# mvanveen/hyperopt

Measured on AMD Instinct MI355X. Metric: TPE candidate x component lpdf evals/sec (10k-trial history), higher is better.
Workload: dtype f32+f64

## Files before the change

hyperopt_amd/_lib.py:

```python
import ctypes
import os

HERE = os.path.dirname(os.path.abspath(__file__))
LIB_PATH = os.path.join(HERE, 'libhyperopt_tpe.so')
HEADER = os.path.join(os.path.dirname(HERE), 'include', 'hyperopt_tpe.h')

ABI_VERSION = 4

TPE_OK = 0
TPE_ERR_VALUE = -1
TPE_ERR_TYPE = -2
TPE_ERR_ARG = -3
TPE_STATUS_VALUE_ONLY = 1
TPE_ERR_HIP = -4
TPE_ERR_SAMPLE = -5

TPE_F64 = 0
TPE_F32 = 1

TPE_GMM1 = 0
TPE_LGMM1 = 1
TPE_CATEGORICAL = 2

TPE_HAS_LOW = 1
TPE_HAS_HIGH = 2
TPE_HAS_Q = 4
TPE_HAS_STREAM = 8

TPE_OPT_SCREEN = 1
TPE_OPT_SPLITK = 2
TPE_OPT_DEDUP = 3
TPE_OPT_CHUNKS = 4
TPE_OPT_WHOLE_N = 5
TPE_OPT_WHOLE_ROUNDS = 6
TPE_OPT_TIMING = 7
TPE_OPT_WINDOW = 8
TPE_OPT_WIN_T = 9
TPE_OPT_WIN_GROUPS = 10
TPE_OPT_EXPAND = 11
TPE_OPT_HOT = 12
TPE_OPT_EARLY = 13
TPE_OPT_HOT_DIV = 14
TPE_OPT_ZERO_WIN = 15
TPE_OPT_VALUE_ONLY = 16
TPE_OPT_RESCORE_CAP = 17
TPE_OPT_MODE_MASK = 18
TPE_OPT_AUX_FAMILIES = 19
TPE_OPT_BX_SPLIT = 21
TPE_OPT_BX_T = 22
TPE_OPT_PK_SLICED = 23
TPE_OPT_DEFER_REPORT = 24
TPE_OPT_LABEL_SHARDS = 25

TPE_JOINT_STREAM = 0x7FFFFFFF

TPE_OBS_IDENTITY = 0
TPE_OBS_LOG = 1
TPE_OBS_LOG_FLOOR = 2


class LabelDesc(ctypes.Structure):
    _fields_ = [('kind', ctypes.c_int32), ('flags', ctypes.c_int32),
                ('low', ctypes.c_double), ('high', ctypes.c_double), ('q', ctypes.c_double),
                ('below_off', ctypes.c_int64), ('above_off', ctypes.c_int64),
                ('n_below', ctypes.c_int32), ('n_above', ctypes.c_int32)]


class LabelSpec(ctypes.Structure):
    _fields_ = [('kind', ctypes.c_int32), ('flags', ctypes.c_int32),
                ('low', ctypes.c_double), ('high', ctypes.c_double), ('q', ctypes.c_double),
                ('prior_mu', ctypes.c_double), ('prior_sigma', ctypes.c_double),
                ('upper', ctypes.c_int32), ('randint', ctypes.c_int32), ('p_off', ctypes.c_int64),
                ('stream', ctypes.c_int32), ('reserved', ctypes.c_int32)]


class LabelResult(ctypes.Structure):
    _fields_ = [('value', ctypes.c_double), ('score', ctypes.c_double),
                ('lpdf_below', ctypes.c_double), ('lpdf_above', ctypes.c_double),
                ('index', ctypes.c_int64), ('label', ctypes.c_int32), ('status', ctypes.c_int32)]


class JointDim(ctypes.Structure):
    _fields_ = [('kind', ctypes.c_int32), ('flags', ctypes.c_int32),
                ('low', ctypes.c_double), ('high', ctypes.c_double),
                ('stream', ctypes.c_int32)]


assert ctypes.sizeof(JointDim) == 32
assert ctypes.sizeof(LabelDesc) == 56
assert ctypes.sizeof(LabelResult) == 48
assert ctypes.sizeof(LabelSpec) == 72

_P = ctypes.c_void_p
_I32, _I64, _U32, _U64, _D = (ctypes.c_int32, ctypes.c_int64, ctypes.c_uint32,
                              ctypes.c_uint64, ctypes.c_double)
_PD = ctypes.POINTER(ctypes.c_double)

SIGNATURES = {
    'tpe_abi_version': (ctypes.c_int, []),
    'tpe_source_hash': (ctypes.c_char_p, []),
    'tpe_ctx_create': (ctypes.c_int, [ctypes.c_int, ctypes.c_int, ctypes.POINTER(_P)]),
    'tpe_ctx_create_multi': (ctypes.c_int, [_P, _I32, ctypes.c_int, ctypes.POINTER(_P)]),
    'tpe_ctx_devices': (ctypes.c_int32, [_P, _P, _I32]),
    'tpe_label_device': (ctypes.c_int32, [_P, _I32]),
    'tpe_ctx_destroy': (None, [_P]),
    'tpe_last_error': (ctypes.c_char_p, [_P]),
    'tpe_gmm1_lpdf': (ctypes.c_int, [_P, _P, _I64, _P, _P, _P, _I32, _I32, _D, _D, _D, _P]),
    'tpe_lgmm1_lpdf': (ctypes.c_int, [_P, _P, _I64, _P, _P, _P, _I32, _I32, _D, _D, _D, _P]),
    'tpe_categorical_lpdf': (ctypes.c_int, [_P, _P, _I64, _P, _I32, _P]),
    'tpe_broadcast_best': (ctypes.c_int, [_P, _P, _P, _I64, _P]),
    'tpe_gmm1_sample': (ctypes.c_int, [_P, _P, _P, _P, _I32, _I32, _D, _D, _D, _U64, _U32, _U32,
                                       _I64, _I64, _P]),
    'tpe_lgmm1_sample': (ctypes.c_int, [_P, _P, _P, _P, _I32, _I32, _D, _D, _D, _U64, _U32, _U32,
                                        _I64, _I64, _P]),
    'tpe_categorical_sample': (ctypes.c_int, [_P, _P, _I32, _U64, _U32, _U32, _I64, _I64, _P]),
    'tpe_set_posterior': (ctypes.c_int, [_P, _P, _I32, _P, _P, _P, _I64]),
    'tpe_suggest': (ctypes.c_int, [_P, _U64, _U32, _I64, _I64, _P]),
    'tpe_suggest_batch': (ctypes.c_int, [_P, _U64, _P, _I32, _I64, _I64, _P]),
    'tpe_score': (ctypes.c_int, [_P, _I32, _P, _I64, _P, _P, _P]),
    'tpe_merge_results': (ctypes.c_int, [_P, _I32, _I32, _P]),
    'tpe_suggest_batch_device': (ctypes.c_int, [_P, _U64, _P, _I32, _I64, _I64, _P, _P]),
    'tpe_merge_results_device': (ctypes.c_int, [_P, _P, _I32, _I32, _P]),
    'tpe_last_timing': (ctypes.c_int, [_P, ctypes.POINTER(ctypes.c_float),
                                       ctypes.POINTER(ctypes.c_float)]),
    'tpe_last_evals': (ctypes.c_int64, [_P]),
    'tpe_last_mode_stats': (ctypes.c_int, [_P, _P, _P]),
    'tpe_build_posterior': (ctypes.c_int, [_P, _P, _I32, _P, _I64, _P, _I64, _P, _P, _P, _D, _D,
                                           _I32, _P]),
    'tpe_get_mixture': (ctypes.c_int, [_P, _I32, _I32, _P, _P, _P, _I32, _P]),
    'tpe_resident_labels': (ctypes.c_int32, [_P]),
    'tpe_history_reset': (ctypes.c_int, [_P, _P, _I32, _P, _I64]),
    'tpe_history_append': (ctypes.c_int, [_P, _P, _P, _P]),
    'tpe_build_posterior_resident': (ctypes.c_int, [_P, _P, _I64, _I64, _D, _D, _I32, _P]),
    'tpe_build_posterior_resident_ordered': (ctypes.c_int, [_P, _P, _I64, _I64, _D, _D, _I32, _P, _P, _P,
                                                            _P, _P]),
    'tpe_rebuild_labels': (ctypes.c_int, [_P, _P, _I64, _I64, _D, _D, _I32, _P, _P, _P, _I32, _P, _P]),
    'tpe_last_build_ms': (ctypes.c_int, [_P, ctypes.POINTER(ctypes.c_float)]),
    'tpe_build_report': (ctypes.c_int, [_P, ctypes.POINTER(ctypes.c_int32), ctypes.c_void_p]),
    'tpe_last_screen': (ctypes.c_int, [_P, _P, _P, ctypes.POINTER(ctypes.c_float)]),
    'tpe_set_option': (ctypes.c_int, [_P, _I32, _I64]),
    'tpe_last_screen_terms': (ctypes.c_int, [_P, _P]),
    'tpe_last_rescore_terms': (ctypes.c_int, [_P, _P]),
    'tpe_last_drawn': (ctypes.c_int, [_P, _P, _P]),
    'tpe_device_bytes': (ctypes.c_int64, []),
    'tpe_prepare': (ctypes.c_int, [_P, ctypes.c_int64, ctypes.c_int32]),
    'tpe_arm_prepare': (ctypes.c_int, [_P, ctypes.c_int64, ctypes.c_int32]),
    'tpe_last_screen_mode': (ctypes.c_int32, [_P]),
    'tpe_last_hot': (ctypes.c_int, [_P, _P, _P]),
    'tpe_last_prepare': (ctypes.c_int, [_P, _P]),
    'tpe_hot_probe': (ctypes.c_int, [_P, ctypes.c_int32, _P, ctypes.c_int64, _P, _P, _P]),
    'tpe_screen_probe': (ctypes.c_int, [_P, _I32, _P, _I64, _P, _P]),
    'tpe_export_posterior': (ctypes.c_int, [_P, _P, _I64, _P]),
    'tpe_import_posterior': (ctypes.c_int, [_P, _P, _I64, _P, _I32, _P, _P]),
    'tpe_joint_set_posterior': (ctypes.c_int, [_P, _P, _I32, _I32, _P, _P, _P, _I32, _P, _P, _P]),
    'tpe_joint_draw': (ctypes.c_int, [_P, _U64, _U32, _I64, _I64, _P, _P]),
    'tpe_joint_score': (ctypes.c_int, [_P, _P, _I64, _P, _P]),
    'tpe_joint_suggest': (ctypes.c_int, [_P, _U64, _U32, _I64, _P, _P, _PD, _PD]),
}

_lib = None


def load():
    global _lib
    if _lib is not None:
        return _lib
    try:
        import torch
    except Exception:
        pass
    variant = os.environ.get('HYPEROPT_AMD_VARIANT')
    path = LIB_PATH
    if variant:
        import sys
        path = os.path.abspath(variant)
        sys.stderr.write('hyperopt_amd: loading the experiment variant %s, not the product '
                         'library\n' % path)
    if not os.path.exists(path):
        raise OSError('hyperopt_amd native library not built: %s (run '
                      '`python -m hyperopt_amd._build` or __graft_entry__.build())' % path)
    lib = ctypes.CDLL(path)
    for name, (res, args) in SIGNATURES.items():
        if variant and not hasattr(lib, name):
            continue
        fn = getattr(lib, name)
        fn.restype = res
        fn.argtypes = args
    if lib.tpe_abi_version() != ABI_VERSION:
        raise OSError('ABI version mismatch')
    if variant:
        if not lib.tpe_source_hash().decode().startswith('v:'):
            raise OSError('%s is not a variant build (tools/build_variant.py)' % path)
    else:
        check_stamp(lib)
    _lib = lib
    return lib


def check_stamp(lib):
    from . import _build
    want = _build.source_hash()
    got = lib.tpe_source_hash().decode()
    if got != want:
        raise OSError('hyperopt_amd native library %s is stale: built from sources %s, tree '
                      'has %s (run `python -m hyperopt_amd._build`)' % (LIB_PATH, got, want))


def header_functions(path=HEADER):
    import re
    txt = open(path).read()
    txt = re.sub(r'/\*.*?\*/', '', txt, flags=re.S)
    return sorted(set(re.findall(r'\b(tpe_[a-z0-9_]+)\s*\(', txt)))
```

hyperopt_amd/csrc/tpe_build.hip:

```cpp
#include <hip/hip_runtime.h>

#include <hipcub/hipcub.hpp>

#include <cmath>
#include <cstring>
#include <string>
#include <vector>

#include "../../include/hyperopt_tpe.h"
#include "tpe_ctx.h"
#include "tpe_device.h"

using namespace tpe;
using namespace tpe_rt;

namespace {

constexpr int kSplitBlock = 1024;
constexpr int kPartBlock = 1024;
constexpr int kPartU = 4;
constexpr int kParzenBlock = 1024;
constexpr int kFoldU = 4;
constexpr int kMaxLF = 64;
constexpr int kCatChunk = 8192;
// ... 1304 lines not shown
        for (int32_t l = 0; l < L; ++l) mx = std::max(mx, B.cnt_h[l]);
        if (mx > 0 && B.pool_cap > 0)
            hipLaunchKernelGGL(k_hist_regrow, dim3((unsigned)std::min<int64_t>((mx + kBlock - 1) / kBlock, 1024), L),
                               dim3(kBlock), 0, sm, B.p_off.p, o2.p, B.cnt.p, B.p_trial.p, B.p_val.p,
                               B.s_key.p, B.s_idx.p, t2.p, v2.p, k2.p, i2.p);
        HIPCHK(ctx, hipGetLastError());
        HIPCHK(ctx, hipStreamSynchronize(sm));
        std::swap(B.p_trial, t2);
        std::swap(B.p_val, v2);
        std::swap(B.s_key, k2);
        std::swap(B.s_idx, i2);
        std::swap(B.p_off, o2);
        t2.release();
        v2.release();
        k2.release();
        i2.release();
        o2.release();
        HIPCHK(ctx, B.s_key2.reserve(pc));
        HIPCHK(ctx, B.s_idx2.reserve(pc));
        HIPCHK(ctx, B.arank.reserve(pc));
        HIPCHK(ctx, B.keys.reserve(pc));
        HIPCHK(ctx, B.idx.reserve(pc));
        B.cap_h = cap;
        B.off_h = off;
        B.pool_cap = pc;
    }
    HIPCHK(ctx, B.st_off.reserve(L + 1));
    HIPCHK(ctx, B.st_trial.reserve(total));
    HIPCHK(ctx, B.st_val.reserve(total));
    HIPCHK(ctx, B.st_idx.reserve(total));
    HIPCHK(ctx, B.st_idx_sorted.reserve(total));
    HIPCHK(ctx, B.st_key_sorted.reserve(total));
    HIPCHK(ctx, B.seg_begin.reserve(L));
    HIPCHK(ctx, B.seg_end.reserve(L));
    auto al = [](int64_t v) { return (v + 15) / 16 * 16; };
    const int64_t o_off = 0, o_val = al((L + 1) * 8), o_trial = o_val + al(total * 8),
                  o_seg = o_trial + al(total * 4), o_cnt = o_seg + al(2 * (int64_t)L * 4),
                  o_end = o_cnt + al((int64_t)L * 4);
    HIPCHK(ctx, B.h_stage.resize(o_end));
    HIPCHK(ctx, B.d_stage.reserve(o_end));
    uint8_t* hs = B.h_stage.data();
    std::memcpy(hs + o_off, st.data(), (L + 1) * sizeof(int64_t));
    int32_t* seg = (int32_t*)(hs + o_seg);
    for (int32_t l = 0; l < L; ++l) {
        seg[l] = (int32_t)st[l];
        seg[L + l] = (int32_t)(B.specs_h[l].kind == TPE_CATEGORICAL ? st[l] : st[l + 1]);
    }
    std::memcpy(hs + o_trial, obs_trial, total * sizeof(int32_t));
    std::memcpy(hs + o_val, obs_val, total * sizeof(double));
    int32_t* cnt_new = (int32_t*)(hs + o_cnt);
    for (int32_t l = 0; l < L; ++l) cnt_new[l] = B.cnt_h[l] + (int32_t)n_new[l];
    HIPCHK(ctx, hipMemcpyAsync(B.d_stage.p, hs, o_end, hipMemcpyHostToDevice, sm));
    {
        const uint8_t* ds = B.d_stage.p;
        const CopySpec cs[5] = {{B.st_off.p, ds + o_off, (L + 1) * 8},
                                {B.st_trial.p, ds + o_trial, total * 4},
                                {B.st_val.p, ds + o_val, total * 8},
                                {B.seg_begin.p, ds + o_seg, (int64_t)L * 4},
                                {B.seg_end.p, ds + o_seg + (int64_t)L * 4, (int64_t)L * 4}};
        const int rc = tpe_rt::copy_batch(ctx, sm, cs, 5);
        if (rc) return rc;
    }
    int64_t mx_new = 0, mx_all = 0;
    for (int32_t l = 0; l < L; ++l) {
        mx_new = std::max(mx_new, n_new[l]);
        mx_all = std::max<int64_t>(mx_all, B.cnt_h[l] + n_new[l]);
    }
    hipLaunchKernelGGL(k_hist_append, dim3((unsigned)std::min<int64_t>((mx_new + kBlock - 1) / kBlock, 1024), L),
                       dim3(kBlock), 0, sm, B.st_off.p, B.st_trial.p, B.st_val.p, B.p_off.p, B.cnt.p,
                       B.p_trial.p, B.p_val.p, B.st_idx.p);
    HIPCHK(ctx, hipGetLastError());
    if (total >= kGlobalSortMin) {
        HIPCHK(ctx, B.gs_a.reserve(total));
        HIPCHK(ctx, B.gs_b.reserve(total));
        HIPCHK(ctx, B.gs_lab.reserve(total));
        HIPCHK(ctx, B.gs_lab2.reserve(total));
        int lab_bits = 1;
        while ((1LL << lab_bits) < (int64_t)L) ++lab_bits;
        const unsigned gb = (unsigned)std::min<int64_t>((total + kBlock - 1) / kBlock, 2048);
        hipLaunchKernelGGL(k_iota, dim3(gb), dim3(kBlock), 0, sm, B.gs_a.p, total);
        HIPCHK(ctx, hipGetLastError());
        size_t b1 = 0, b2 = 0;
        HIPCHK(ctx, hipcub::DeviceRadixSort::SortPairs(nullptr, b1, B.st_val.p, B.st_key_sorted.p, B.gs_a.p,
                                                         B.gs_b.p, (int)total, 0, 64, sm));
        HIPCHK(ctx, hipcub::DeviceRadixSort::SortPairs(nullptr, b2, B.gs_lab.p, B.gs_lab2.p, B.gs_b.p,
                                                         B.gs_a.p, (int)total, 0, lab_bits, sm));
        HIPCHK(ctx, B.sort_tmp.reserve(std::max<size_t>(std::max(b1, b2), 1)));
        HIPCHK(ctx, hipcub::DeviceRadixSort::SortPairs(B.sort_tmp.p, b1, B.st_val.p, B.st_key_sorted.p,
                                                         B.gs_a.p, B.gs_b.p, (int)total, 0, 64, sm));
        hipLaunchKernelGGL(k_label_of, dim3(gb), dim3(kBlock), 0, sm, B.st_off.p, L, B.gs_b.p, B.gs_lab.p, total);
        HIPCHK(ctx, hipGetLastError());
        HIPCHK(ctx, hipcub::DeviceRadixSort::SortPairs(B.sort_tmp.p, b2, B.gs_lab.p, B.gs_lab2.p, B.gs_b.p,
                                                         B.gs_a.p, (int)total, 0, lab_bits, sm));
        hipLaunchKernelGGL(k_sorted_gather, dim3(gb), dim3(kBlock), 0, sm, B.gs_a.p, B.st_val.p, B.st_idx.p,
                           B.st_key_sorted.p, B.st_idx_sorted.p, total);
        HIPCHK(ctx, hipGetLastError());
    } else {
        size_t bytes = 0;
        HIPCHK(ctx, hipcub::DeviceSegmentedRadixSort::SortPairs(
                        nullptr, bytes, B.st_val.p, B.st_key_sorted.p, B.st_idx.p, B.st_idx_sorted.p,
                        (int)total, L, B.seg_begin.p, B.seg_end.p, 0, 64, sm));
        HIPCHK(ctx, B.sort_tmp.reserve(std::max<size_t>(bytes, 1)));
        HIPCHK(ctx, hipcub::DeviceSegmentedRadixSort::SortPairs(
                        B.sort_tmp.p, bytes, B.st_val.p, B.st_key_sorted.p, B.st_idx.p, B.st_idx_sorted.p,
                        (int)total, L, B.seg_begin.p, B.seg_end.p, 0, 64, sm));
    }
    hipLaunchKernelGGL(k_hist_merge, dim3((unsigned)std::min<int64_t>((mx_all + kBlock - 1) / kBlock, 1024), L),
                       dim3(kBlock), 0, sm, B.specs.p, B.p_off.p, B.cnt.p, B.st_off.p, B.s_key.p,
                       B.s_idx.p, B.st_key_sorted.p, B.st_idx_sorted.p, B.s_key2.p, B.s_idx2.p);
    HIPCHK(ctx, hipGetLastError());
    std::swap(B.s_key, B.s_key2);
    std::swap(B.s_idx, B.s_idx2);
    for (int32_t l = 0; l < L; ++l) B.cnt_h[l] += (int32_t)n_new[l];
    {
        const CopySpec cs{B.cnt.p, B.d_stage.p + o_cnt, (int64_t)L * 4};
        const int rc = tpe_rt::copy_batch(ctx, sm, &cs, 1);
        if (rc) return rc;
    }
    HIPCHK(ctx, hipEventRecord(B.ev_staged, sm));
    B.staged_pending = true;
    return TPE_OK;
}

constexpr int32_t kGammaCap = 25;

uint64_t loss_fingerprint(const double* losses, int64_t n) {
    uint64_t h = 0x9e3779b97f4a7c15ull ^ (uint64_t)n;
    for (int64_t t = 0; t < n; ++t) {
        uint64_t v;
        std::memcpy(&v, losses + t, sizeof(v));
        h = (h ^ v) * 0xff51afd7ed558ccdull;
        h ^= h >> 29;
    }
    return h;
}

int finish_build(tpe_ctx* ctx, BuildTail& t, int32_t* ties_out, int32_t* n_below_out) {
    auto& B = ctx->build;
    Posterior& P = ctx->resident;
    const int32_t n_labels = t.n_labels;
    const int64_t rep_dl = t.rep_dl;
    std::vector<DLabel>& dl = t.dl;
    const std::vector<int32_t>* grp = t.grp;
    const bool beside = t.beside, subset = t.subset;
    HIPCHK(ctx, hipStreamSynchronize(t.st));
    P.qc_ready = false;
    int32_t errh;
    std::memcpy(&errh, B.h_rep.data() + rep_dl, sizeof(int32_t));
    std::memcpy(dl.data(), B.h_rep.data(), rep_dl);
    B.last_ties.resize(n_labels + 1);
    std::memcpy(B.last_ties.data(), B.h_rep.data() + rep_dl + 16, (n_labels + 1) * sizeof(int32_t));
    B.last_n_below = t.n_below;
    if (ties_out) std::memcpy(ties_out, B.last_ties.data(), (n_labels + 1) * sizeof(int32_t));
    if (t.deferred) ctx->build_ms = -1.f;
    else HIPCHK(ctx, hipEventElapsedTime(&ctx->build_ms, ctx->ev0, ctx->ev1));
    if (errh & 1) return ctx->fail(TPE_ERR_ARG, "observation trial position out of range");
    if (errh & 2) return ctx->fail(TPE_ERR_ARG, "more below observations than the below set (duplicate trial in a label?)");
    if (errh & 4) return ctx->fail(TPE_ERR_VALUE, "below weights sum to zero");
    if (errh & 8) return ctx->fail(TPE_ERR_ARG, "supplied observation order does not fit the above set");

    std::vector<int32_t> cat;
    for (int m = 0; m < kNumModes; ++m) {
        P.group_off[m] = (int32_t)cat.size();
        cat.insert(cat.end(), grp[m].begin(), grp[m].end());
        P.h_group[m] = grp[m];
    }
    const bool groups_changed = cat != P.groups_h || !P.groups.p;
    if (groups_changed) {
        HIPCHK(ctx, P.groups.reserve(std::max<size_t>(cat.size(), 1)));
        HIPCHK(ctx, hipMemcpy(P.groups.p, cat.data(), cat.size() * sizeof(int32_t), hipMemcpyHostToDevice));
        P.groups_h = cat;
    }
    P.h_labels = dl;
    P.win_ready = false;
    P.zw_ready = false;
    P.qc_ready = t.qc_queued;
    if (!beside) P.bx_ready = tpe_rt::bx_keep_after(ctx, groups_changed);
    P.n_labels = n_labels;
    B.n_labels = n_labels;
    B.mix_h = t.mix;
    B.built_ok = true;
    B.built_gen = B.hist_gen;
    B.built_T = t.n_trials;
    B.built_valid = t.n_valid;
    B.built_gamma = t.gamma;
    B.built_pw = t.pw;
    B.built_lf = t.lf;
    if (!subset) B.built_loss_hash = t.loss_hash;
    if (n_below_out) *n_below_out = t.n_below;
    P.bx_prescan_ok = t.prescan && !P.bx_ready;
    if (t.arm_c > 0) return tpe1_prepare(ctx, t.arm_c, t.arm_r);
    return TPE_OK;
}

int build_resident(tpe_ctx* ctx, const double* losses, int64_t n_trials, int64_t n_valid,
                   double gamma, double prior_weight, int32_t lf, int32_t* n_below_out,
                   const uint8_t* below_h = nullptr, const int64_t* order_off_h = nullptr,
                   const int32_t* order_h = nullptr, int32_t* ties_out = nullptr,
                   const int32_t* only_h = nullptr, int32_t n_only = 0) {
    auto& B = ctx->build;
    const bool defer_report = B.defer;
    B.defer = false;
    if (!B.hist_ready) return ctx->fail(TPE_ERR_ARG, "no resident history (tpe_history_reset)");
    const bool subset = only_h != nullptr && n_only > 0;
    const int64_t arm_c = subset ? 0 : ctx->arm_c;
    const int32_t arm_r = subset ? 0 : ctx->arm_r;
    if (!subset) ctx->arm_c = ctx->arm_r = 0;
    if (subset) {
        if (below_h)
            return ctx->fail(TPE_ERR_ARG, "a label-subset rebuild keeps the previous build's below set");
        if (!B.built_ok || B.built_gen != B.hist_gen || B.built_T != n_trials || B.built_valid != n_valid ||
            B.built_gamma != gamma || B.built_pw != prior_weight || B.built_lf != lf ||
            B.n_labels != (int32_t)B.specs_h.size())
            return ctx->fail(TPE_ERR_ARG, "a label-subset rebuild must follow a build of the same history");
        if (n_trials > 0 && !losses) return ctx->fail(TPE_ERR_ARG, "tpe_build_posterior: bad trial arguments");
        if (loss_fingerprint(losses, n_trials) != B.built_loss_hash)
            return ctx->fail(TPE_ERR_ARG, "a label-subset rebuild must be given the previous build's losses");
        for (int32_t i = 0; i < n_only; ++i)
            if (only_h[i] < 0 || only_h[i] >= B.n_labels || (i && only_h[i] <= only_h[i - 1]))
                return ctx->fail(TPE_ERR_ARG, "subset labels must be increasing label indices");
    }
    B.built_ok = false;
    ctx->resident.bx_prescan_ok = false;
    if (lf < 1 || lf >= kMaxLF) return ctx->fail(TPE_ERR_ARG, "linear forgetting must be in [1, 63]");
    if (n_trials < 0 || n_trials >= INT32_MAX || (n_trials > 0 && !losses) || n_valid < 0 ||
        n_valid > n_trials)
        return ctx->fail(TPE_ERR_ARG, "tpe_build_posterior: bad trial arguments");
    HIPCHK(ctx, hipSetDevice(ctx->device));
    const int32_t n_labels = (int32_t)B.specs_h.size();
    Posterior& P = ctx->resident;
    ctx->P = &ctx->resident;
    bool beside = subset;
    for (int32_t i = 0; beside && i < n_only; ++i) {
        const tpe_label_spec& s = B.specs_h[only_h[i]];
        beside = s.kind == TPE_CATEGORICAL || (s.flags & TPE_HAS_Q) != 0;
    }
    hipStream_t st = beside ? ctx->aux : ctx->stream;

    const double nbd = std::ceil(gamma * std::sqrt((double)n_valid));
    const int32_t n_below = (int32_t)std::min<double>(nbd, (double)kGammaCap);
    if (below_h) {
        int64_t nb = 0;
        for (int64_t t = 0; t < n_trials; ++t)
            if (below_h[t]) {
                if (!(losses[t] == losses[t])) return ctx->fail(TPE_ERR_ARG, "below set holds a trial without a loss");
                ++nb;
            }
        if (nb != n_below) return ctx->fail(TPE_ERR_ARG, "below set size differs from n_below");
    }

    std::vector<DLabel> dl(n_labels);
    std::vector<int64_t> mix(2 * (size_t)n_labels);
    std::vector<int32_t> grp[kNumModes];
    int64_t total = 0, samp_total = 0, max_cap = 1;
    for (int32_t l = 0; l < n_labels; ++l) {
        const tpe_label_spec& s = B.specs_h[l];
        DLabel& o = dl[l];
        std::memset(&o, 0, sizeof(o));
        const bool quant = (s.flags & TPE_HAS_Q) != 0;
        int64_t cap_b, cap_a;
        if (s.kind == TPE_CATEGORICAL) {
            o.mode = CAT;
            cap_b = cap_a = s.upper;
        } else {
            o.mode = s.kind == TPE_GMM1 ? (quant ? QUANT_GMM : DENSE_GMM) : (quant ? QUANT_LGMM : DENSE_LGMM);
            cap_b = lf + 1;
            cap_a = (int64_t)B.cnt_h[l] + 1;
        }
        o.flags = s.kind == TPE_CATEGORICAL ? 0 : (s.flags & (TPE_HAS_LOW | TPE_HAS_HIGH | TPE_HAS_Q));
        o.low = s.low;
        o.high = s.high;
        o.q = s.q;
        o.exp_low = std::exp(s.low);
        o.exp_high = std::exp(s.high);
        o.stream = (s.flags & TPE_HAS_STREAM) ? s.stream : l;
        o.comp_b = mix[2 * l] = total;
        total += cap_b;
        o.comp_a = mix[2 * l + 1] = total;
        total += cap_a;
        max_cap = std::max(max_cap, std::max(cap_b, cap_a));
        o.samp_off = samp_total;
        samp_total += cap_b;
        grp[o.mode].push_back(l);
    }
    const int64_t T = n_trials;
    HIPCHK(ctx, B.losses.reserve(std::max<int64_t>(T, 1)));
    HIPCHK(ctx, B.below.reserve(std::max<int64_t>(T, 1)));
    HIPCHK(ctx, B.below_val.reserve((size_t)n_labels * kMaxLF));
    HIPCHK(ctx, B.counts.reserve(2 * (size_t)n_labels));
    HIPCHK(ctx, B.kcount.reserve(2 * (size_t)n_labels));
    HIPCHK(ctx, B.keys.reserve(std::max<int64_t>(B.pool_cap, 1)));
    HIPCHK(ctx, B.idx.reserve(std::max<int64_t>(B.pool_cap, 1)));
    HIPCHK(ctx, B.arank.reserve(std::max<int64_t>(B.pool_cap, 1)));
    HIPCHK(ctx, B.w.reserve(total));
    HIPCHK(ctx, B.mu.reserve(total));
    HIPCHK(ctx, B.sigma.reserve(total));
    HIPCHK(ctx, B.mix_off.reserve(2 * (size_t)n_labels));
    HIPCHK(ctx, B.scratch.reserve(4 * (size_t)total));
    HIPCHK(ctx, P.labels.reserve(n_labels));
    HIPCHK(ctx, P.comps64.reserve(total));
    HIPCHK(ctx, P.comps32.reserve(total));
    HIPCHK(ctx, P.samp.reserve(samp_total));
    HIPCHK(ctx, ctx->build_err.reserve(1));
    HIPCHK(ctx, B.ties.reserve(n_labels + 1));
    const int64_t* order_off_d = nullptr;
    const int32_t* order_d = nullptr;
    std::vector<UpTask> up;
    std::vector<const void*> up_src;
    auto put = [&](const void* src, int64_t bytes, void* dst) {
        if (bytes <= 0) return;
        up.push_back(UpTask{0, (uint8_t*)dst, bytes, 0});
        up_src.push_back(src);
    };
    put(nullptr, (n_labels + 1) * (int64_t)sizeof(int32_t), B.ties.p);
    if (order_off_h && order_h && order_off_h[n_labels] > 0) {
        for (int32_t l = 0; l < n_labels; ++l)
            if (order_off_h[l + 1] < order_off_h[l] || order_off_h[l] < 0)
                return ctx->fail(TPE_ERR_ARG, "order offsets must not decrease");
        HIPCHK(ctx, B.order_off.reserve(n_labels + 1));
        HIPCHK(ctx, B.order.reserve(order_off_h[n_labels]));
        put(order_off_h, (n_labels + 1) * (int64_t)sizeof(int64_t), B.order_off.p);
        put(order_h, order_off_h[n_labels] * (int64_t)sizeof(int32_t), B.order.p);
        order_off_d = B.order_off.p;
        order_d = B.order.p;
    }
    const int32_t* only_d = nullptr;
    const int32_t nl_run = subset ? n_only : n_labels;
    if (subset) {
        HIPCHK(ctx, B.only.reserve(n_only));
        put(only_h, n_only * (int64_t)sizeof(int32_t), B.only.p);
        only_d = B.only.p;
    } else {
        put(losses, T * (int64_t)sizeof(double), B.losses.p);
        if (below_h) put(below_h, T, B.below.p);
        put(mix.data(), (int64_t)mix.size() * (int64_t)sizeof(int64_t), B.mix_off.p);
        put(dl.data(), n_labels * (int64_t)sizeof(DLabel), P.labels.p);
    }
    put(nullptr, sizeof(int32_t), ctx->build_err.p);
    {
        const int64_t head = ((int64_t)up.size() * (int64_t)sizeof(UpTask) + 255) / 256 * 256;
        int64_t o = head;
        for (UpTask& u : up) {
            u.src = up_src[&u - up.data()] ? o : -1;
            if (u.src >= 0) o += (u.bytes + 15) / 16 * 16;
        }
        if (B.up_pending) {
            HIPCHK(ctx, hipEventSynchronize(B.ev_up));
            B.up_pending = false;
        }
        HIPCHK(ctx, B.h_up.resize(o));
        HIPCHK(ctx, B.d_up.reserve(o));
        std::memcpy(B.h_up.data(), up.data(), up.size() * sizeof(UpTask));
        for (size_t i = 0; i < up.size(); ++i)
            if (up[i].src >= 0) std::memcpy(B.h_up.data() + up[i].src, up_src[i], up[i].bytes);
        HIPCHK(ctx, hipMemcpyAsync(B.d_up.p, B.h_up.data(), o, hipMemcpyHostToDevice, st));
        if (!B.ev_up) HIPCHK(ctx, hipEventCreateWithFlags(&B.ev_up, hipEventDisableTiming));
        HIPCHK(ctx, hipEventRecord(B.ev_up, st));
        B.up_pending = true;
        int64_t mx = 1;
        for (const UpTask& u : up) mx = std::max(mx, u.bytes);
        hipLaunchKernelGGL(k_build_inputs, dim3((unsigned)std::min<int64_t>((mx + 4 * kUpBlock - 1) / (4 * kUpBlock), 32),
                                                (unsigned)up.size()),
                           dim3(kUpBlock), 0, st, (const UpTask*)B.d_up.p, B.d_up.p);
        HIPCHK(ctx, hipGetLastError());
    }

    HIPCHK(ctx, hipEventRecord(ctx->ev0, st));
    if (T > 0 && !below_h && !subset) {
        const int rc = launch_split(ctx, st, B.losses.p, T, n_below, B.below.p, B.ties.p + n_labels);
        if (rc) return rc;
    }
    hipLaunchKernelGGL(k_partition, dim3(nl_run), dim3(kPartBlock), 0, st, B.specs.p, B.p_off.p, B.cnt.p,
                       B.p_trial.p, B.p_val.p, B.s_key.p, B.s_idx.p, B.below.p, B.losses.p, T,
                       B.below_val.p, B.arank.p, B.keys.p, B.idx.p, B.counts.p, ctx->build_err.p, only_d);
    hipLaunchKernelGGL(k_parzen, dim3(nl_run, 2), dim3(kParzenBlock), 0, st, B.specs.p, B.cat_p.p,
                       B.p_off.p, B.counts.p, B.below_val.p, B.keys.p, B.keys.p, B.idx.p, B.mix_off.p,
                       prior_weight, lf, B.w.p, B.mu.p, B.sigma.p, B.kcount.p, B.scratch.p + total, order_off_d,
                       order_d, B.ties.p, ctx->build_err.p, only_d);
    hipLaunchKernelGGL(k_fold_terms, dim3((unsigned)((max_cap + kTermBlock - 1) / kTermBlock), nl_run, 2),
                       dim3(kTermBlock), 0, st, P.labels.p, B.kcount.p, B.mix_off.p, B.w.p, B.mu.p,
                       B.sigma.p, B.scratch.p, B.scratch.p + 2 * total, B.scratch.p + 3 * total, only_d);
    hipLaunchKernelGGL(k_fold, dim3(nl_run), dim3(kParzenBlock), 0, st, P.labels.p, B.kcount.p,
                       B.mix_off.p, B.w.p, B.mu.p, B.sigma.p, P.comps64.p, P.comps32.p, P.samp.p,
                       B.scratch.p, B.scratch.p + 2 * total, B.scratch.p + 3 * total, B.scratch.p + total,
                       ctx->build_err.p, only_d);
    HIPCHK(ctx, hipGetLastError());
    HIPCHK(ctx, hipEventRecord(ctx->ev1, st));
    const int64_t rep_dl = (int64_t)n_labels * (int64_t)sizeof(DLabel);
    const int64_t rep_bytes = rep_dl + 16 + (int64_t)(n_labels + 1) * (int64_t)sizeof(int32_t);
    HIPCHK(ctx, B.d_rep.reserve(rep_bytes));
    HIPCHK(ctx, B.h_rep.resize(rep_bytes));
    hipLaunchKernelGGL(k_build_report, dim3(1), dim3(kUpBlock), 0, st, (const uint32_t*)P.labels.p,
                       (int32_t)(rep_dl / 4), ctx->build_err.p, B.ties.p, n_labels + 1, (uint32_t*)B.d_rep.p);
    HIPCHK(ctx, hipGetLastError());
    HIPCHK(ctx, hipMemcpyAsync(B.h_rep.data(), B.d_rep.p, rep_bytes, hipMemcpyDeviceToHost, st));
    if (!beside) {
        const int rc = tpe_rt::bx_keep_check(ctx);
        if (rc) return rc;
    }
    bool prescan = false;
    if (!subset && arm_c > 0 && P.groups.p) {
        std::vector<int32_t> cat_now;
        for (int m = 0; m < kNumModes; ++m) cat_now.insert(cat_now.end(), grp[m].begin(), grp[m].end());
        bool same = cat_now == P.groups_h;
        for (int m = 0; same && m < kNumModes; ++m) same = grp[m] == P.h_group[m];
        if (same) {
            const int rc = tpe_rt::bx_prescan(ctx, st, &prescan);
            if (rc) return rc;
        }
    }
    bool qc_queued = false;
    if (beside && P.groups.p) {
        std::vector<int32_t> cat_now;
        for (int m = 0; m < kNumModes; ++m) cat_now.insert(cat_now.end(), grp[m].begin(), grp[m].end());
        if (cat_now == P.groups_h) {
            const int rc = tpe_rt::qc_launch(ctx, st);
            if (rc) return rc;
            qc_queued = true;
        }
    }
    BuildTail t;
    t.st = st;
    t.rep_dl = rep_dl;
    t.n_labels = n_labels;
    t.lf = lf;
    t.n_below = n_below;
    t.dl = std::move(dl);
    for (int m = 0; m < kNumModes; ++m) t.grp[m] = std::move(grp[m]);
    t.mix = std::move(mix);
    t.beside = beside;
    t.qc_queued = qc_queued;
    t.subset = subset;
    t.n_trials = n_trials;
    t.n_valid = n_valid;
    t.arm_c = arm_c;
    t.arm_r = arm_r;
    t.prescan = prescan;
    t.gamma = gamma;
    t.pw = prior_weight;
    if (!subset) t.loss_hash = loss_fingerprint(losses, n_trials);
    if (beside && subset && qc_queued && defer_report) {
        t.deferred = true;
        B.pending.reset(new BuildTail(std::move(t)));
        if (ties_out) std::memset(ties_out, 0, (n_labels + 1) * sizeof(int32_t));
        if (n_below_out) *n_below_out = n_below;
        return TPE_OK;
    }
    return finish_build(ctx, t, ties_out, n_below_out);
}

}

int tpe_rt::settle_build(tpe_ctx* ctx) {
    if (!ctx) return TPE_OK;
    auto& B = ctx->build;
    if (!B.pending) return TPE_OK;
    std::unique_ptr<BuildTail> t = std::move(B.pending);
    return finish_build(ctx, *t, nullptr, nullptr);
}

extern "C" {

TPE_DEV int tpe1_history_reset(tpe_ctx* ctx, const tpe_label_spec* specs, int32_t n_labels,
                      const double* cat_p, int64_t n_cat_p) {
    if (!ctx) return TPE_ERR_ARG;
    TPE_SETTLE(ctx);
    return history_reset(ctx, specs, n_labels, cat_p, n_cat_p);
}

TPE_DEV int tpe1_history_append(tpe_ctx* ctx, const int64_t* n_new, const int32_t* obs_trial,
                       const double* obs_val) {
    if (!ctx || !n_new) return TPE_ERR_ARG;
    TPE_SETTLE(ctx);
    return history_append(ctx, n_new, obs_trial, obs_val);
}

TPE_DEV int tpe1_build_posterior_resident(tpe_ctx* ctx, const double* losses, int64_t n_trials,
                                 int64_t n_valid, double gamma, double prior_weight, int32_t lf,
                                 int32_t* n_below_out) {
    if (!ctx) return TPE_ERR_ARG;
    TPE_SETTLE(ctx);
    return build_resident(ctx, losses, n_trials, n_valid, gamma, prior_weight, lf, n_below_out);
}

TPE_DEV int tpe1_build_posterior_resident_ordered(tpe_ctx* ctx, const double* losses, int64_t n_trials,
                                                  int64_t n_valid, double gamma, double prior_weight,
                                                  int32_t lf, const uint8_t* below, const int64_t* order_off,
                                                  const int32_t* order, int32_t* n_below_out, int32_t* ties) {
    if (!ctx) return TPE_ERR_ARG;
    TPE_SETTLE(ctx);
    return build_resident(ctx, losses, n_trials, n_valid, gamma, prior_weight, lf, n_below_out, below,
                          order_off, order, ties);
}

TPE_DEV int tpe1_rebuild_labels(tpe_ctx* ctx, const double* losses, int64_t n_trials, int64_t n_valid,
                                double gamma, double prior_weight, int32_t lf, const int64_t* order_off,
                                const int32_t* order, const int32_t* labels, int32_t n_only,
                                int32_t* n_below_out, int32_t* ties) {
    if (!ctx) return TPE_ERR_ARG;
    TPE_SETTLE(ctx);
    if (!labels || n_only <= 0) return ctx->fail(TPE_ERR_ARG, "tpe_rebuild_labels: no labels");
    return build_resident(ctx, losses, n_trials, n_valid, gamma, prior_weight, lf, n_below_out, nullptr,
                          order_off, order, ties, labels, n_only);
}

TPE_DEV int tpe1_build_posterior(tpe_ctx* ctx, const tpe_label_spec* specs, int32_t n_labels,
                        const double* cat_p, int64_t n_cat_p, const double* losses,
                        int64_t n_trials, const int64_t* obs_off, const int32_t* obs_trial,
                        const double* obs_val, double gamma, double prior_weight, int32_t lf,
                        int32_t* n_below_out) {
    if (!ctx) return TPE_ERR_ARG;
    TPE_SETTLE(ctx);
    if (n_labels <= 0 || !specs || !obs_off || n_trials < 0 || (n_trials > 0 && !losses))
        return ctx->fail(TPE_ERR_ARG, "tpe_build_posterior: bad arguments");
    if (obs_off[0] != 0 || obs_off[n_labels] < 0 || obs_off[n_labels] >= INT32_MAX)
        return ctx->fail(TPE_ERR_ARG, "observation offsets");
    std::vector<int64_t> n_new(n_labels);
    for (int32_t l = 0; l < n_labels; ++l) {
        n_new[l] = obs_off[l + 1] - obs_off[l];
        if (n_new[l] < 0) return ctx->fail(TPE_ERR_ARG, "observation offsets must not decrease");
    }
    int64_t n_valid = 0;
    for (int64_t t = 0; t < n_trials; ++t) n_valid += losses[t] == losses[t];
    int rc = history_reset(ctx, specs, n_labels, cat_p, n_cat_p);
    if (!rc) rc = history_append(ctx, n_new.data(), obs_trial, obs_val);
    if (!rc) rc = build_resident(ctx, losses, n_trials, n_valid, gamma, prior_weight, lf, n_below_out);
    if (rc) ctx->build.hist_ready = false;
    return rc;
}

TPE_DEV int tpe1_get_mixture(tpe_ctx* ctx, int32_t label, int32_t side, double* weights, double* mus,
                             double* sigmas, int32_t cap, int32_t* n) {
    if (!ctx) return TPE_ERR_ARG;
    TPE_SETTLE(ctx);
    auto& B = ctx->build;
    if (label < 0 || label >= B.n_labels || side < 0 || side > 1 || ctx->resident.n_labels != B.n_labels)
        return ctx->fail(TPE_ERR_ARG, "tpe_get_mixture: no such built mixture");
    const DLabel& d = ctx->resident.h_labels[label];
    const int32_t K = side ? d.na : d.nb;
    if (n) *n = K;
    const int32_t m = std::min(K, std::max(cap, 0));
    const int64_t o = B.mix_h[2 * (size_t)label + side];
    HIPCHK(ctx, hipSetDevice(ctx->device));
    if (m > 0) {
        if (weights) HIPCHK(ctx, hipMemcpy(weights, B.w.p + o, m * sizeof(double), hipMemcpyDeviceToHost));
        if (mus) HIPCHK(ctx, hipMemcpy(mus, B.mu.p + o, m * sizeof(double), hipMemcpyDeviceToHost));
        if (sigmas) HIPCHK(ctx, hipMemcpy(sigmas, B.sigma.p + o, m * sizeof(double), hipMemcpyDeviceToHost));
    }
    return TPE_OK;
}

TPE_DEV int32_t tpe1_resident_labels(const tpe_ctx* ctx) { return ctx ? ctx->resident.n_labels : 0; }

TPE_DEV int tpe1_last_build_ms(const tpe_ctx* ctx, float* ms) {
    if (!ctx || !ms) return TPE_ERR_ARG;
    TPE_SETTLE(const_cast<tpe_ctx*>(ctx));
    *ms = ctx->build_ms;
    return TPE_OK;
}

TPE_DEV int tpe1_build_report(tpe_ctx* ctx, int32_t* n_below, int32_t* ties) {
    if (!ctx) return TPE_ERR_ARG;
    TPE_SETTLE(ctx);
    if (n_below) *n_below = ctx->build.last_n_below;
    if (ties) {
        const auto& t = ctx->build.last_ties;
        if (t.empty()) return ctx->fail(TPE_ERR_ARG, "tpe_build_report: no build");
        std::memcpy(ties, t.data(), t.size() * sizeof(int32_t));
    }
    return TPE_OK;
}

}
```

hyperopt_amd/csrc/tpe_ctx.h:

```cpp
#pragma once

#include <hip/hip_runtime.h>
#include <stdint.h>

#include <algorithm>
#include <atomic>
#include <memory>
#include <string>
#include <vector>

#include "../../include/hyperopt_tpe.h"
#include "tpe_device.h"

struct tpe_ctx;

namespace tpe_rt {

struct RescoreChunkH {
    int32_t cell, j;
};
struct RescorePlanH {
    int64_t total;
    int32_t ne, sliced, overflow, pad;
};
// ... 86 lines not shown
            if (e != hipSuccess) {
                p = nullptr;
                return e;
            }
            cap = c;
        }
        n = m;
        return hipSuccess;
    }
    T* data() { return p; }
    const T* data() const { return p; }
    size_t size() const { return n; }
    T& operator[](size_t i) { return p[i]; }
    const T& operator[](size_t i) const { return p[i]; }
    PinVec() = default;
    PinVec(const PinVec&) = delete;
    PinVec& operator=(const PinVec&) = delete;
    ~PinVec() {
        if (p) (void)hipHostFree(p);
    }
};

struct PinScalars {
    int32_t err = 0, hot_flag = 0, bx_diff = 1, pad = 0;
    unsigned long long screen_exec = 0, xdrawn[2] = {0, 0};
    RescorePlanH plan{};
};

struct Posterior {
    std::vector<DLabel> h_labels;
    std::vector<int32_t> h_group[kNumModes];
    int32_t n_labels = 0;
    DevBuf<DLabel> labels;
    DevBuf<Comp<double>> comps64;
    DevBuf<Comp<float>> comps32;
    DevBuf<SampRec> samp;
    DevBuf<int32_t> groups;
    std::vector<int32_t> groups_h;
    int32_t group_off[kNumModes] = {};
    bool win_ready = false;
    bool zw_ready = false;
    DevBuf<double> zw_hi, zw_lo;
    DevBuf<int32_t> zw_wide, zw_n;
    bool qc_ready = false;
    DevBuf<Comp<double>> qcomp;
    DevBuf<int32_t> qc_n;
    int32_t win_t = 0;
    DevBuf<tpe::WinLabel> win;
    DevBuf<double> win_p, win_q;
    DevBuf<Comp<float>> win_wide;
    DevBuf<int2> win_bins;
    DevBuf<double> win_seg;
    DevBuf<int32_t> win_hist;
    DevBuf<uint8_t> win_flag;
    DevBuf<double> win_skip;
    DevBuf<double> win_skip_part;
    bool bx_ready = false, bx_ok = false;
    bool bx_prescan_ok = false;
    PinVec<double> bx_scan_h;
    DevBuf<tpe::BxLabel> bx;
    std::vector<tpe::BxLabel> bx_h;
    PinVec<tpe::BxLabel> bx_up_h;
    DevBuf<double> bx_tab;
    DevBuf<int32_t> bx_nc;
    DevBuf<tpe::BxTerm> bx_terms;
    DevBuf<int32_t> bx_loff;
    DevBuf<int32_t> bx_list;
    DevBuf<double> bx_scan;
    DevBuf<float2> bx_sb;
    DevBuf<float> bx_sbp;
    DevBuf<double> bx_part;
    DevBuf<int2> bx_blocks;
    PinVec<int2> bx_blocks_h;
    int64_t bx_sb_max = 0;
    uint64_t bx_gen = 0;
    DevBuf<tpe::DLabel> bx_snap_l;
    DevBuf<tpe::Comp<double>> bx_snap_c;
    DevBuf<tpe::SampRec> bx_snap_s;
    DevBuf<int32_t> bx_snap_g;
    DevBuf<int32_t> bx_diff;
    int32_t bx_snap_nl = 0;
    void release() {
        labels.release();
        comps64.release();
        comps32.release();
        samp.release();
        groups.release();
        groups_h.clear();
        win.release();
        win_p.release();
        win_q.release();
        win_wide.release();
        win_bins.release();
        win_seg.release();
        win_hist.release();
        win_flag.release();
        win_skip.release();
        win_skip_part.release();
        win_ready = false;
        zw_ready = false;
        qc_ready = false;
        qcomp.release();
        qc_n.release();
        zw_hi.release();
        zw_lo.release();
        zw_wide.release();
        zw_n.release();
        bx.release();
        bx_h.clear();
        bx_tab.release();
        bx_nc.release();
        bx_terms.release();
        bx_loff.release();
        bx_list.release();
        bx_scan.release();
        bx_sb.release();
        bx_sbp.release();
        bx_part.release();
        bx_blocks.release();
        bx_snap_l.release();
        bx_snap_c.release();
        bx_snap_s.release();
        bx_snap_g.release();
        bx_diff.release();
        bx_snap_nl = 0;
        bx_ready = bx_ok = false;
        n_labels = 0;
    }
};

struct CopySpec {
    void* dst;
    const void* src;
    int64_t bytes;
};
constexpr int kCopyBatch = 8;
int copy_batch(tpe_ctx* ctx, hipStream_t st, const CopySpec* specs, int n);

struct UpTask {
    int64_t src;
    uint8_t* dst;
    int64_t bytes;
    int64_t pad;
};

struct BuildTail {
    hipStream_t st = nullptr;
    int64_t rep_dl = 0;
    int32_t n_labels = 0, lf = 0, n_below = 0;
    std::vector<DLabel> dl;
    std::vector<int32_t> grp[kNumModes];
    std::vector<int64_t> mix;
    bool beside = false, qc_queued = false, subset = false, deferred = false;
    int64_t n_trials = 0, n_valid = 0, arm_c = 0;
    int32_t arm_r = 0;
    bool prescan = false;
    double gamma = 0.0, pw = 0.0;
    uint64_t loss_hash = 0;
};
int settle_build(tpe_ctx* ctx);

struct BuildBufs {
    std::vector<tpe_label_spec> specs_h;
    std::vector<int64_t> cap_h, off_h;
    std::vector<int32_t> cnt_h;
    int64_t pool_cap = 0;
    bool hist_ready = false;
    DevBuf<tpe_label_spec> specs;
    DevBuf<double> cat_p;
    DevBuf<int64_t> p_off;
    DevBuf<int32_t> cnt;
    DevBuf<int32_t> p_trial;
    DevBuf<double> p_val;
    DevBuf<double> s_key, s_key2;
    DevBuf<int32_t> s_idx, s_idx2;
    DevBuf<int32_t> arank;
    DevBuf<int64_t> st_off;
    DevBuf<int32_t> st_trial, st_idx, st_idx_sorted;
    DevBuf<double> st_val, st_key_sorted;
    DevBuf<int32_t> seg_begin, seg_end;
    DevBuf<uint8_t> sort_tmp;
    DevBuf<int32_t> gs_a, gs_b;
    DevBuf<uint32_t> gs_lab, gs_lab2;
    PinVec<uint8_t> h_stage;
    DevBuf<uint8_t> d_stage;
    hipEvent_t ev_staged = nullptr;
    bool staged_pending = false;
    DevBuf<double> losses;
    DevBuf<uint8_t> below;
    DevBuf<double> keys;
    DevBuf<int32_t> idx;
    DevBuf<double> below_val;
    DevBuf<int32_t> counts;
    DevBuf<int32_t> kcount;
    DevBuf<double> w, mu, sigma;
    DevBuf<int64_t> mix_off;
    DevBuf<double> scratch;
    DevBuf<int32_t> ties;
    DevBuf<int64_t> order_off;
    DevBuf<int32_t> order;
    int32_t n_labels = 0;
    std::vector<int64_t> mix_h;
    uint64_t hist_gen = 0, built_gen = 0;
    bool built_ok = false;
    int64_t built_T = -1, built_valid = -1;
    double built_gamma = 0.0, built_pw = 0.0;
    int32_t built_lf = 0;
    uint64_t built_loss_hash = 0;
    DevBuf<int32_t> only;
    DevBuf<uint64_t> split_key;
    DevBuf<int64_t> split_pos;
    bool defer = false;
    std::unique_ptr<BuildTail> pending;
    std::vector<int32_t> last_ties;
    int32_t last_n_below = 0;
    PinVec<uint8_t> h_up, h_rep;
    DevBuf<uint8_t> d_up, d_rep;
    hipEvent_t ev_up = nullptr;
    bool up_pending = false;
    void release() {
        specs.release(); cat_p.release(); p_off.release(); cnt.release(); p_trial.release();
        p_val.release(); s_key.release(); s_key2.release(); s_idx.release(); s_idx2.release();
        arank.release(); st_off.release(); st_trial.release(); st_idx.release();
        st_idx_sorted.release(); st_val.release(); st_key_sorted.release(); seg_begin.release();
        seg_end.release(); sort_tmp.release(); gs_a.release(); gs_b.release(); gs_lab.release();
        gs_lab2.release(); losses.release(); below.release(); keys.release();
        idx.release(); below_val.release(); counts.release(); kcount.release(); w.release();
        mu.release(); sigma.release(); mix_off.release(); scratch.release(); ties.release();
        order_off.release(); order.release(); only.release(); split_key.release(); split_pos.release();
        d_up.release(); d_rep.release(); d_stage.release();
        if (ev_up) (void)hipEventDestroy(ev_up);
        ev_up = nullptr;
        up_pending = false;
        if (ev_staged) (void)hipEventDestroy(ev_staged);
        ev_staged = nullptr;
        staged_pending = false;
        built_ok = false;
        n_labels = 0;
        hist_ready = false;
        pool_cap = 0;
    }
};

double np_pairwise_sum(const double* a, size_t n);

struct QExchange {
    virtual int exchange(tpe_ctx* ctx, std::vector<unsigned long long>& mm) = 0;
    virtual ~QExchange() {}
};

}

struct tpe_ctx {
    using Partial = tpe::Partial;
    using QInfo = tpe_rt::QInfo;
    template <typename T>
    using DevBuf = tpe_rt::DevBuf<T>;
    using Posterior = tpe_rt::Posterior;
    static constexpr int kNumModes = tpe_rt::kNumModes;

    int device = 0;
    int precision = TPE_F64;
    hipStream_t stream = nullptr;
    hipEvent_t ev0 = nullptr, ev1 = nullptr, ev2 = nullptr;
    hipEvent_t evm[kNumModes][2] = {};
    bool mode_ran[kNumModes] = {};
    float mode_ms[kNumModes] = {};
    int64_t mode_evals[kNumModes] = {};
    std::string err;
    float score_ms = 0.f, round_ms = 0.f;
    int64_t evals = 0;
    bool dedup = true;
    bool timing = true;

    Posterior resident, single;
    Posterior* P = &resident;

    DevBuf<Partial> partials;
    DevBuf<tpe_label_result> results;
    DevBuf<uint32_t> rounds;
    DevBuf<int32_t> errflag;
    DevBuf<int32_t> build_err;
    DevBuf<double> cand, out_lb, out_la;
    DevBuf<int32_t> one_group;
    DevBuf<int64_t> qj;
    DevBuf<unsigned long long> qmm;
    DevBuf<QInfo> qinfo;
    DevBuf<double2> qtab;
    DevBuf<unsigned long long> qkmax;
    DevBuf<int64_t> xfound;
    DevBuf<unsigned long long> xdrawn;
    unsigned long long xdrawn_h[2] = {0, 0};
    bool cat_early = false;
    DevBuf<double> xs, slice_part;
    bool splitk = true;
    DevBuf<double> chunk_part;
    int32_t chunks_forced = 0;
    bool screen = true;
    DevBuf<float> scr_hi;
    DevBuf<double> scr_hid;
    DevBuf<double2> bx_lohi;
    bool expand = true;
    int32_t hot = 1;
    bool early = true;
    bool zero_win = true;
    bool zw_pending = false;
    double hot_cap_div = 16.0;
    DevBuf<double> hot_x;
    DevBuf<uint32_t> rs_done;
    bool dense_one = false;
    DevBuf<int32_t> hot_pc;
    DevBuf<uint32_t> hot_ucell;
    DevBuf<uint4> samp_img;
    int32_t bx_split = 0;
    int64_t pk_sliced = 8192;
    int32_t bx_t_force = 0;
    double bx_t_next = 64.0;
    DevBuf<int32_t> hot_i, hot_cnt;
    DevBuf<int32_t> hot_mi, hot_mcnt;
    DevBuf<unsigned long long> hot_t, hot_tau0;
    DevBuf<uint32_t> hot_bits;
    DevBuf<int32_t> hot_flag;
    DevBuf<int32_t> hot_items;
    tpe_rt::PinVec<int32_t> hot_cnt_h;
    int64_t hot_listed = 0;
    int32_t hot_fallback = 0;
    bool hot_ran = false;
    int64_t hot_cells = 0;
    bool hot_redo = false;
    DevBuf<int64_t> rs_plan;
    bool value_only = false;
    int32_t mode_mask = 31;
    int64_t pk_cap = 1 << 16;
    bool pk_plan_pending = false;
    bool pk_redo = false;
    tpe_label_result* dev_out = nullptr;
    float prep_ms = 0.f;
    hipEvent_t ev_prep[2] = {};
    bool prep_pending = false;
    uint64_t hot_tau0_gen = 0;
    int64_t hot_tau0_n = 0;
    int64_t arm_c = 0;
    int32_t arm_r = 0;
    DevBuf<int32_t> scr_idx;
    DevBuf<unsigned long long> scr_lb;
    DevBuf<int32_t> scr_cnt;
    tpe_rt::PinVec<int32_t> scr_cnt_h;
    tpe_rt::PinVec<tpe_rt::PinScalars> pin;
    struct RepTask {
        const void* src;
        void* dst;
        int64_t bytes;
    };
    std::vector<RepTask> rep;
    tpe_rt::DevBuf<uint8_t> rep_d;
    tpe_rt::PinVec<uint8_t> rep_h;
    tpe_rt::PinVec<tpe_label_result> res_h;
    static constexpr int kResPieces = 4;
    hipEvent_t ev_res[kResPieces] = {};
    tpe_rt::PinVec<tpe::DLabel> dl_h;
    tpe_rt::PinVec<int32_t> ties_h;
    DevBuf<int64_t> scr_chunks;
    DevBuf<int64_t> scr_list;
    DevBuf<Partial> scr_res;
    DevBuf<int64_t> scr_rsel;
    DevBuf<int64_t> scr_off;
    DevBuf<int64_t> scr_range;
    DevBuf<double> scr_planes;
    DevBuf<double> rs_x, rs_part;
    DevBuf<int32_t> rs_win;
    DevBuf<int64_t> rs_g;
    std::vector<tpe_rt::RescoreChunkH> scr_chunks_h;
    int64_t screen_total = 0, screen_rescored = 0;
    int32_t screen_mode = 0;
    bool screen_pending = false;
    bool window = true;
    int32_t win_t = tpe::kWinTDefault;
    int32_t win_groups = 0;
    DevBuf<uint32_t> win_keys[2], win_keys2[2];
    DevBuf<uint8_t> win_keys8[2], win_keys8b[2];
    DevBuf<uint64_t> win_vals[2], win_vals2[2];
    DevBuf<uint8_t> win_tmp[2];
    hipStream_t aux = nullptr;
    hipEvent_t ev_fork = nullptr, ev_sorted[2] = {}, ev_done[2] = {};
    hipEvent_t ev_cat[2] = {};
    bool aux_families = false;
    std::vector<hipEvent_t> evw;
    int32_t evw_used = 0;
    DevBuf<unsigned long long> win_evals;
    DevBuf<float2> win_lohi;
    int64_t screen_exec = 0;
    int64_t screen_rescore_terms = 0;
    bool screen_exec_pending = false;
    unsigned long long screen_exec_h = 0;
    hipEvent_t evs[2] = {};
    float screen_ms = 0.f;
    tpe_rt::BuildBufs build;
    int64_t built_n_trials = 0;
    int32_t built_n_below = 0;
    float build_ms = 0.f;

    std::vector<tpe_ctx*> peers;
    std::shared_ptr<void> workers;
    std::shared_ptr<void> share;
    int64_t hint_n = 0;
    int32_t hint_rounds = 0;
    int64_t opt_whole_n = 0;
    int32_t opt_whole_rounds = 0;
    tpe_rt::QExchange* qx = nullptr;
    int32_t shard_id = 0;
    std::vector<std::vector<int32_t>> lsh_ids;
    std::vector<int32_t> lsh_dev, lsh_local;
    int32_t lsh_L = 0;
    bool lsh_enable = true;

    std::shared_ptr<void> joint;

    int fail(int code, const std::string& m) {
        err = m;
        return code;
    }
    int hip(hipError_t e, const char* what) {
        if (e == hipSuccess) return TPE_OK;
        err = std::string(what) + ": " + hipGetErrorString(e);
        return TPE_ERR_HIP;
    }
};

namespace tpe_rt {
struct WinScreenArgs {
    const int32_t* grp;
    int32_t nl;
    int64_t n, cand_offset;
    uint64_t seed;
    int32_t z0, nz;
    const double* cand_in;
    float* hi;
    unsigned long long* lbkey;
    double *s_out, *e_out;
    int32_t cpack = 0;
    float2* lohi = nullptr;
    int32_t y0 = 0, nl_all = 0;
    int slot = 0;
};
int win_prepare(tpe_ctx* ctx);
int win_screen(tpe_ctx* ctx, const WinScreenArgs& a, const uint64_t** sorted_vals);
int win_reserve(tpe_ctx* ctx, size_t total, int64_t cells, int nslots);
int win_sort(tpe_ctx* ctx, const WinScreenArgs& a, hipStream_t st, const uint64_t** sorted);
int win_tiles(tpe_ctx* ctx, const WinScreenArgs& a, const uint64_t* sorted, hipStream_t st);
int64_t win_rounds_per_batch(int64_t n, int32_t nl);

int bx_prepare(tpe_ctx* ctx);
uint64_t next_bx_gen();
int bx_build(tpe_ctx* ctx);
int bx_keep_check(tpe_ctx* ctx);
bool bx_keep_after(tpe_ctx* ctx, bool groups_changed);
int bx_prescan(tpe_ctx* ctx, hipStream_t st, bool* queued);
int qc_launch(tpe_ctx* ctx, hipStream_t st);
}

#define TPE_SETTLE(ctx)                                   \
    do {                                                  \
        const int settle_rc_ = tpe_rt::settle_build(ctx); \
        if (settle_rc_) return settle_rc_;                \
    } while (0)

#define TPE_DEV __attribute__((visibility("hidden")))
extern "C" {
TPE_DEV int tpe1_set_posterior(tpe_ctx* ctx, const tpe_label_desc* labels, int32_t n_labels,
                               const double* weights, const double* mus, const double* sigmas,
                               int64_t n_components);
TPE_DEV int tpe1_suggest(tpe_ctx* ctx, uint64_t seed, uint32_t round, int64_t n_candidates,
                         int64_t cand_offset, tpe_label_result* out);
TPE_DEV int tpe1_suggest_batch(tpe_ctx* ctx, uint64_t seed, const uint32_t* rounds,
                               int32_t n_rounds, int64_t n_candidates, int64_t cand_offset,
                               tpe_label_result* out);
TPE_DEV int tpe1_set_option(tpe_ctx* ctx, int32_t option, int64_t value);
TPE_DEV int tpe1_prepare(tpe_ctx* ctx, int64_t n_candidates, int32_t n_rounds);
TPE_DEV int tpe1_arm_prepare(tpe_ctx* ctx, int64_t n_candidates, int32_t n_rounds);
TPE_DEV int tpe1_history_reset(tpe_ctx* ctx, const tpe_label_spec* specs, int32_t n_labels,
                               const double* cat_p, int64_t n_cat_p);
TPE_DEV int tpe1_history_append(tpe_ctx* ctx, const int64_t* n_new, const int32_t* obs_trial,
                                const double* obs_val);
TPE_DEV int tpe1_build_posterior_resident(tpe_ctx* ctx, const double* losses, int64_t n_trials,
                                          int64_t n_valid, double gamma, double prior_weight,
                                          int32_t lf, int32_t* n_below_out);
TPE_DEV int tpe1_build_posterior_resident_ordered(tpe_ctx* ctx, const double* losses, int64_t n_trials,
                                                  int64_t n_valid, double gamma, double prior_weight,
                                                  int32_t lf, const uint8_t* below, const int64_t* order_off,
                                                  const int32_t* order, int32_t* n_below_out, int32_t* ties);
TPE_DEV int tpe1_rebuild_labels(tpe_ctx* ctx, const double* losses, int64_t n_trials, int64_t n_valid,
                                double gamma, double prior_weight, int32_t lf, const int64_t* order_off,
                                const int32_t* order, const int32_t* labels, int32_t n_only,
                                int32_t* n_below_out, int32_t* ties);
TPE_DEV int tpe1_build_posterior(tpe_ctx* ctx, const tpe_label_spec* specs, int32_t n_labels,
                                 const double* cat_p, int64_t n_cat_p, const double* losses,
                                 int64_t n_trials, const int64_t* obs_off, const int32_t* obs_trial,
                                 const double* obs_val, double gamma, double prior_weight,
                                 int32_t lf, int32_t* n_below_out);
TPE_DEV void tpe1_ctx_destroy(tpe_ctx* ctx);
TPE_DEV int tpe1_get_mixture(tpe_ctx* ctx, int32_t label, int32_t side, double* weights, double* mus,
                             double* sigmas, int32_t cap, int32_t* n);
TPE_DEV int32_t tpe1_resident_labels(const tpe_ctx* ctx);
TPE_DEV int tpe1_last_build_ms(const tpe_ctx* ctx, float* ms);
TPE_DEV int tpe1_build_report(tpe_ctx* ctx, int32_t* n_below, int32_t* ties);
TPE_DEV int tpe1_score(tpe_ctx* ctx, int32_t label, const double* cand, int64_t n, double* lpdf_below,
                       double* lpdf_above, tpe_label_result* out);
}

#define TPE_NOT_LSHARD(ctx)                                                                        \
    do {                                                                                         \
        if (!(ctx)->lsh_ids.empty())                                                             \
            return (ctx)->fail(TPE_ERR_ARG, "not available on a label-sharded multi-device context"); \
    } while (0)

#define HIPCHK(ctx, call)                                  \
    do {                                                   \
        int _rc = (ctx)->hip((call), #call);               \
        if (_rc != TPE_OK) return _rc;                     \
    } while (0)
```

hyperopt_amd/csrc/tpe_engine.hip:

```cpp
#include <hip/hip_runtime.h>

#include <algorithm>
#include <type_traits>
#include <cmath>
#include <cstdio>
#include <cstring>
#include <string>
#include <thread>
#include <vector>

#include "../../include/hyperopt_tpe.h"
#include "tpe_ctx.h"
#include "tpe_device.h"

using namespace tpe;
using namespace tpe_rt;

namespace {

constexpr int kR = 4;
constexpr int kRGroup = 3;
constexpr int kTile = kBlock * kR;

thread_local std::string g_create_error;
// ... 3838 lines not shown
                       a.cand_offset, a.seed, ctx->rounds.p, qbase, ctx->P->n_labels, a.tiles,          \
                       ctx->partials.p, ctx->errflag.p, a.S)
                const unsigned qgx = (unsigned)std::max<int64_t>(
                    1, std::min<int64_t>({(int64_t)a.gx, (a.n + kQR * kBlock - 1) / (kQR * kBlock),
                                          kHotWgs / std::max<int64_t>(1, (int64_t)cnt * a.gz)}));
#define TPE_QTILES(M)                                                                                   \
    do {                                                                                                \
    for (const EarlyPhase& ph : early_phases(a, (int64_t)kQR * kBlock, qgx, found != nullptr,           \
                                             (int64_t)cnt * a.gz))                                     \
        hipLaunchKernelGGL((k_qfused_tiles<M, kQR>), dim3(ph.grid, cnt, a.gz), dim3(kBlock), 0,         \
                           ctx->stream, ctx->P->labels.p, g.dev[mode], ctx->P->comps64.p, ctx->P->samp.p, \
                           ctx->qinfo.p, ctx->qtab.p, ph.n, a.cand_offset, a.seed, ctx->rounds.p, qbase,  \
                           ctx->P->n_labels, a.tiles, ctx->partials.p, ctx->errflag.p, ctx->qkmax.p, found, \
                           ph.i0, ph.slot_base, ph.empty_from, nullptr);                                \
    launch_early_drawn(ctx, g.dev[mode], cnt, a, found, (int64_t)kQR * kBlock, ctx->xdrawn.p);          \
    } while (0)
                if (fam) {
                    if (a.S.cpack == 0) TPE_QTILES(QUANT_LGMM);
                    else if (narrow(a.S)) TPE_QFUSED(QUANT_LGMM, kRGroup);
                    else TPE_QFUSED(QUANT_LGMM, kR);
                } else {
                    if (a.S.cpack == 0) TPE_QTILES(QUANT_GMM);
                    else if (narrow(a.S)) TPE_QFUSED(QUANT_GMM, kRGroup);
                    else TPE_QFUSED(QUANT_GMM, kR);
                }
#undef TPE_QTILES
#undef TPE_QFUSED
                bracket(ctx, mode, 1);
            }
            return ctx->hip(hipGetLastError(), "fused quantized launch");
        }
        evals_q[0] = evals_q[1] = 0;
    }
    const size_t slots = (size_t)a.n_rounds * nq;
    HIPCHK(ctx, ctx->qj.reserve(slots * (size_t)a.n));
    HIPCHK(ctx, ctx->qmm.reserve(2 * (size_t)nq));
    HIPCHK(ctx, ctx->qinfo.reserve(nq));
    const int first_mode = nqg ? QUANT_GMM : QUANT_LGMM;
    bracket(ctx, first_mode, 0);
    HIPCHK(ctx, hipMemsetAsync(ctx->qmm.p, 0xFF, nq * sizeof(unsigned long long), ctx->stream));
    HIPCHK(ctx, hipMemsetAsync(ctx->qmm.p + nq, 0, nq * sizeof(unsigned long long), ctx->stream));
#define TPE_QSAMPLE(M, CNT, BASE, RR)                                                         \
    hipLaunchKernelGGL((k_qsample<M, RR>), dim3(a.gx, CNT, a.gz), dim3(kBlock), 0, ctx->stream, \
                       ctx->P->labels.p, g.dev[M], ctx->P->samp.p, a.n, a.cand_offset, a.seed,      \
                       ctx->rounds.p, nq, BASE, ctx->qj.p, ctx->qmm.p, ctx->qmm.p + nq,        \
                       ctx->errflag.p, a.S)
    if (nqg) {
        if (narrow(a.S)) TPE_QSAMPLE(QUANT_GMM, nqg, 0, kRGroup);
        else TPE_QSAMPLE(QUANT_GMM, nqg, 0, kR);
    }
    if (nql) {
        if (narrow(a.S)) TPE_QSAMPLE(QUANT_LGMM, nql, nqg, kRGroup);
        else TPE_QSAMPLE(QUANT_LGMM, nql, nqg, kR);
    }
#undef TPE_QSAMPLE
    HIPCHK(ctx, hipGetLastError());
    std::vector<unsigned long long> mm(2 * (size_t)nq);
    HIPCHK(ctx, hipMemcpyAsync(mm.data(), ctx->qmm.p, 2 * nq * sizeof(unsigned long long),
                               hipMemcpyDeviceToHost, ctx->stream));
    HIPCHK(ctx, hipStreamSynchronize(ctx->stream));
    if (ctx->qx) {
        int rc = ctx->qx->exchange(ctx, mm);
        if (rc) return rc;
    }
    std::vector<QInfo> qi(nq);
    int64_t tab = 0, maxG = 0;
    const int64_t total = a.total_slots;
    for (int qpos = 0; qpos < nq; ++qpos) {
        const int64_t jmin = (int64_t)(mm[qpos] ^ 0x8000000000000000ull);
        const int64_t jmax = (int64_t)(mm[nq + qpos] ^ 0x8000000000000000ull);
        const int64_t G = (mm[qpos] <= mm[nq + qpos]) ? jmax - jmin + 1 : 0;
        qi[qpos] = QInfo{jmin, (ctx->dedup && G > 0 && 2 * G <= total) ? G : 0, tab, 1, 0, 0};
        tab += qi[qpos].G;
        maxG = std::max(maxG, qi[qpos].G);
        const int li = qpos < nqg ? ctx->P->h_group[QUANT_GMM][qpos] : ctx->P->h_group[QUANT_LGMM][qpos - nqg];
        const DLabel& d = ctx->P->h_labels[li];
        evals_q[qpos < nqg ? 0 : 1] += (qi[qpos].G ? qi[qpos].G : total) * (int64_t)(d.nb + d.na);
    }
    HIPCHK(ctx, ctx->qtab.reserve(std::max<int64_t>(tab, 1)));
    HIPCHK(ctx, hipMemcpyAsync(ctx->qinfo.p, qi.data(), nq * sizeof(QInfo),
                               hipMemcpyHostToDevice, ctx->stream));
    for (int fam = 0; fam < 2; ++fam) {
        const int mode = fam ? QUANT_LGMM : QUANT_GMM;
        const int cnt = fam ? nql : nqg;
        const int qbase = fam ? nqg : 0;
        if (!cnt) continue;
        if (mode != first_mode) bracket(ctx, mode, 0);
        if (maxG > 0) {
            dim3 tg((unsigned)maxG, cnt, 1);
            if (fam)
                hipLaunchKernelGGL(k_qtable<QUANT_LGMM>, tg, dim3(kBlock), 0, ctx->stream,
                                   ctx->P->labels.p, g.dev[mode], ctx->P->comps64.p, ctx->qinfo.p, nq,
                                   qbase, ctx->qtab.p, nullptr, ctx->P->qcomp.p, ctx->P->qc_n.p);
            else
                hipLaunchKernelGGL(k_qtable<QUANT_GMM>, tg, dim3(kBlock), 0, ctx->stream,
                                   ctx->P->labels.p, g.dev[mode], ctx->P->comps64.p, ctx->qinfo.p, nq,
                                   qbase, ctx->qtab.p, nullptr, ctx->P->qcomp.p, ctx->P->qc_n.p);
        }
        dim3 sg(a.gx, cnt, a.gz);
#define TPE_QSCAN(M, RR)                                                                      \
    hipLaunchKernelGGL((k_qscan<M, RR>), sg, dim3(kBlock), 0, ctx->stream, ctx->P->labels.p,     \
                       g.dev[mode], ctx->P->comps64.p, ctx->qj.p, ctx->qinfo.p, ctx->qtab.p, a.n, \
                       a.cand_offset, nq, qbase, ctx->P->n_labels, a.tiles, ctx->partials.p, a.S)
        if (fam) {
            if (narrow(a.S)) TPE_QSCAN(QUANT_LGMM, kRGroup);
            else TPE_QSCAN(QUANT_LGMM, kR);
        } else {
            if (narrow(a.S)) TPE_QSCAN(QUANT_GMM, kRGroup);
            else TPE_QSCAN(QUANT_GMM, kR);
        }
#undef TPE_QSCAN
        bracket(ctx, mode, 1);
    }
    HIPCHK(ctx, hipGetLastError());
    return TPE_OK;
}

constexpr int64_t kSplitKMaxSlots = 2048;

inline int slices_of(const DLabel& d) {
    const int S = slice_len(d.mode);
    return (d.nb + S - 1) / S + (d.na + S - 1) / S;
}

template <typename T, int MODE>
int launch_splitk(tpe_ctx* ctx, const Groups& g, const RoundArgs& a, int32_t s_max) {
    constexpr bool kAny = MODE == DENSE_ANY;
    const int nl = kAny ? g.count[DENSE_GMM] + g.count[DENSE_LGMM] : g.count[MODE];
    if (nl == 0) return TPE_OK;
    const int32_t* grp = kAny ? ctx->P->groups.p + ctx->P->group_off[DENSE_GMM] : g.dev[MODE];
    int32_t s_mode = 0;
    for (int m : {kAny ? DENSE_GMM : MODE, kAny ? DENSE_LGMM : MODE})
        for (int li : ctx->P->h_group[m]) s_mode = std::max(s_mode, slices_of(ctx->P->h_labels[li]));
    const Comp<T>* comps;
    if constexpr (sizeof(T) == 8) comps = ctx->P->comps64.p; else comps = ctx->P->comps32.p;
    const int32_t L = ctx->P->n_labels;
    const int slot = kAny ? DENSE_GMM : MODE;
    bracket(ctx, slot, 0);
    const unsigned sb = (unsigned)((a.n * a.n_rounds + kBlock - 1) / kBlock);
    hipLaunchKernelGGL(k_sample_small<MODE>, dim3(sb, nl), dim3(kBlock), 0, ctx->stream,
                       ctx->P->labels.p, grp, ctx->P->samp.p, a.n, a.cand_offset, a.seed,
                       ctx->rounds.p, a.n_rounds, L, ctx->xs.p, ctx->errflag.p);
    hipLaunchKernelGGL((k_score_slices<T, MODE>),
                       dim3((unsigned)((s_mode + kSliceWaves - 1) / kSliceWaves), nl, a.n_rounds),
                       dim3(kBlock), 0, ctx->stream, ctx->P->labels.p, grp, comps,
                       ctx->P->comps64.p, a.n, L, s_max, ctx->xs.p, ctx->slice_part.p);
    hipLaunchKernelGGL((k_finish_slices<T, MODE>), dim3(nl, a.n_rounds), dim3(kBlock), 0,
                       ctx->stream, ctx->P->labels.p, grp, comps, a.n, a.cand_offset, L, s_max,
                       ctx->xs.p, ctx->slice_part.p, ctx->partials.p, ctx->errflag.p);
    bracket(ctx, slot, 1);
    return ctx->hip(hipGetLastError(), "split-K launch");
}

int run_round(tpe_ctx* ctx, uint64_t seed, const uint32_t* rounds_h, int32_t n_rounds, int64_t n,
              int64_t cand_offset, const double* cand_in_dev, double* olb, double* ola,
              tpe_label_result* out, int32_t only_label) {
    if (ctx->P->n_labels == 0) return ctx->fail(TPE_ERR_ARG, "no posterior set (tpe_set_posterior)");
    if (n < 0 || n_rounds <= 0) return ctx->fail(TPE_ERR_ARG, "bad candidate/round count");
    if (cand_offset < 0 || cand_offset + n > (int64_t)UINT32_MAX)
        return ctx->fail(TPE_ERR_ARG, "candidate indices must stay below 2^32");
    if (!(ctx->build.pending && only_label < 0 && cand_in_dev == nullptr && n > 0 && ctx->aux_families &&
          ctx->aux && !ctx->qx))
        TPE_SETTLE(ctx);
    Slots S{0, 0, n_rounds};
    int32_t tiles;
    uint32_t gx, gz;
    if (n > 0 && n < kTile) {
        const int per_block = n <= kBlock * kRGroup ? kBlock * kRGroup : kTile;
        S.cpack = (int32_t)n;
        S.rpb = per_block / (int32_t)n;
        tiles = 1;
        gx = (uint32_t)((n_rounds + S.rpb - 1) / S.rpb);
        gz = 1;
    } else {
        tiles = (int32_t)((n + kTile - 1) / kTile);
        gx = (uint32_t)tiles;
        gz = (uint32_t)n_rounds;
    }
    const int32_t L = ctx->P->n_labels;
    ctx->rep.clear();
    HIPCHK(ctx, ctx->partials.reserve((size_t)n_rounds * L * std::max(tiles, 1)));
    HIPCHK(ctx, ctx->results.reserve((size_t)n_rounds * L));
    HIPCHK(ctx, ctx->rounds.reserve(n_rounds));
    HIPCHK(ctx, ctx->errflag.reserve(1));
    HIPCHK(ctx, hipMemcpyAsync(ctx->rounds.p, rounds_h, n_rounds * sizeof(uint32_t),
                               hipMemcpyHostToDevice, ctx->stream));
    HIPCHK(ctx, ctx->xdrawn.reserve(2));
    {
        FillSet f{};
        add_fill(f, ctx->errflag.p, sizeof(int32_t), 0);
        add_fill(f, ctx->xdrawn.p, 2 * sizeof(unsigned long long), 0);
        if (ctx->early && S.cpack == 0 && cand_in_dev == nullptr) {
            HIPCHK(ctx, ctx->xfound.reserve((size_t)n_rounds * L));
            add_fill(f, ctx->xfound.p, (size_t)n_rounds * L * sizeof(int64_t), 0x7f7f7f7fu);
        }
        const int rc = run_fills(ctx, f);
        if (rc) return rc;
    }
    const int32_t fam = only_label >= 0 ? 31 : ctx->mode_mask;
    const bool dense_on = (fam & 3) != 0;
    Groups g;
    for (int m = 0; m < kNumModes; ++m) {
        g.dev[m] = ctx->P->groups.p + ctx->P->group_off[m];
        g.count[m] = (fam >> m) & 1 ? (int32_t)ctx->P->h_group[m].size() : 0;
        if (!((fam >> m) & 1)) continue;
        ctx->mode_ran[m] = false;
        ctx->mode_ms[m] = 0.f;
        ctx->mode_evals[m] = 0;
    }
    if (only_label >= 0) {
        HIPCHK(ctx, ctx->one_group.reserve(1));
        HIPCHK(ctx, hipMemcpyAsync(ctx->one_group.p, &only_label, sizeof(int32_t),
                                   hipMemcpyHostToDevice, ctx->stream));
        for (int m = 0; m < kNumModes; ++m) g.count[m] = 0;
        const int m = ctx->P->h_labels[only_label].mode;
        g.dev[m] = ctx->one_group.p;
        g.count[m] = 1;
    }
    const int64_t n_whole =
        ctx->hint_n > 0 ? ctx->hint_n : (ctx->opt_whole_n > 0 ? ctx->opt_whole_n : n);
    const int32_t rounds_whole = ctx->hint_rounds > 0
                                     ? ctx->hint_rounds
                                     : (ctx->opt_whole_rounds > 0 ? ctx->opt_whole_rounds : n_rounds);
    const uint32_t gx_whole =
        S.cpack ? (uint32_t)((rounds_whole + S.rpb - 1) / S.rpb) : gx;
    RoundArgs a{n, cand_offset, seed, n_rounds, tiles, cand_in_dev, olb, ola, S, gx, gz,
                n_whole * rounds_whole, gx_whole};
    if (dense_on) {
        ctx->screen_total = ctx->screen_rescored = 0;
        ctx->hot_ran = false;
        ctx->hot_listed = 0;
        ctx->hot_fallback = 0;
        ctx->screen_mode = 0;
        ctx->screen_exec = 0;
        ctx->screen_rescore_terms = 0;
    }
    if (fam & (1 << CAT)) ctx->cat_early = false;
    ctx->dense_one = false;
    ctx->pk_plan_pending = false;
    ctx->zw_pending = false;
    ctx->evw_used = 0;
    ctx->screen_pending = false;
    ctx->screen_exec_pending = false;
    const bool sample = cand_in_dev == nullptr;
    int64_t evals_q[2] = {0, 0};
    if (ctx->timing) HIPCHK(ctx, hipEventRecord(ctx->ev0, ctx->stream));
    const bool splitk = sample && ctx->splitk && n > 0 && S.cpack != 0 &&
                        a.total_slots <= kSplitKMaxSlots;
    if (splitk) {
        TPE_SETTLE(ctx);
        int32_t s_max = 1;
        for (int m = 0; m < CAT; ++m)
            for (int li : ctx->P->h_group[m]) s_max = std::max(s_max, slices_of(ctx->P->h_labels[li]));
        HIPCHK(ctx, ctx->xs.reserve((size_t)n_rounds * L * n));
        HIPCHK(ctx, ctx->slice_part.reserve((size_t)n_rounds * L * s_max * n));
        int rc;
        if (ctx->precision == TPE_F32) {
            if ((rc = launch_splitk<float, DENSE_ANY>(ctx, g, a, s_max))) return rc;
        } else {
            if ((rc = launch_splitk<double, DENSE_ANY>(ctx, g, a, s_max))) return rc;
        }
        if ((rc = launch_splitk<double, QUANT_GMM>(ctx, g, a, s_max))) return rc;
        if ((rc = launch_splitk<double, QUANT_LGMM>(ctx, g, a, s_max))) return rc;
        for (int q = 0; q < 2; ++q)
            for (int li : ctx->P->h_group[q ? QUANT_LGMM : QUANT_GMM]) {
                const DLabel& d = ctx->P->h_labels[li];
                evals_q[q] += n * (int64_t)n_rounds * (d.nb + d.na);
            }
        launch_round<double, CAT, true>(ctx, g, a);
    } else if (sample) {
        const bool side = ctx->aux_families && ctx->aux && !ctx->qx && a.tiles > 0 &&
                          g.count[CAT] + g.count[QUANT_GMM] + g.count[QUANT_LGMM] > 0;
        int rc = TPE_OK;
        bool dense_done = false;
        if (side) {
            HIPCHK(ctx, hipEventRecord(ctx->ev_cat[0], ctx->stream));
            if (ctx->build.pending) {
                rc = ctx->precision == TPE_F32 ? launch_dense<float>(ctx, g, a) : launch_dense<double>(ctx, g, a);
                if (rc) return rc;
                dense_done = true;
                TPE_SETTLE(ctx);
            }
            HIPCHK(ctx, hipStreamWaitEvent(ctx->aux, ctx->ev_cat[0], 0));
            std::swap(ctx->stream, ctx->aux);
            rc = launch_quantized(ctx, g, a, evals_q);
            if (rc == TPE_OK) launch_round<double, CAT, true>(ctx, g, a);
            std::swap(ctx->stream, ctx->aux);
            const hipError_t e = hipEventRecord(ctx->ev_cat[1], ctx->aux);
            if (rc == TPE_OK && e != hipSuccess) rc = ctx->hip(e, "second-stream join");
        } else {
            TPE_SETTLE(ctx);
            rc = launch_quantized(ctx, g, a, evals_q);
        }
        if (rc == TPE_OK && !dense_done)
            rc = ctx->precision == TPE_F32 ? launch_dense<float>(ctx, g, a) : launch_dense<double>(ctx, g, a);
        if (side) HIPCHK(ctx, hipStreamWaitEvent(ctx->stream, ctx->ev_cat[1], 0));
        if (rc) return rc;
        if (!side) launch_round<double, CAT, true>(ctx, g, a);
    } else {
        launch_round<double, QUANT_GMM, false>(ctx, g, a);
        launch_round<double, QUANT_LGMM, false>(ctx, g, a);
        if (ctx->precision == TPE_F32) {
            launch_round<float, DENSE_GMM, false>(ctx, g, a);
            launch_round<float, DENSE_LGMM, false>(ctx, g, a);
        } else {
            launch_round<double, DENSE_GMM, false>(ctx, g, a);
            launch_round<double, DENSE_LGMM, false>(ctx, g, a);
        }
        launch_round<double, CAT, false>(ctx, g, a);
    }
    HIPCHK(ctx, hipGetLastError());
    TPE_SETTLE(ctx);
    if (ctx->timing) HIPCHK(ctx, hipEventRecord(ctx->ev1, ctx->stream));
    if (tiles == 1) {
        const int64_t nr = (int64_t)n_rounds * L;
        hipLaunchKernelGGL(k_emit, dim3((unsigned)((nr + kBlock - 1) / kBlock)), dim3(kBlock), 0,
                           ctx->stream, ctx->partials.p, nr, L, ctx->results.p);
        HIPCHK(ctx, hipGetLastError());
    } else if (tiles > 1) {
        hipLaunchKernelGGL(k_reduce, dim3(L, n_rounds), dim3(kReduceBlock), 0, ctx->stream,
                           ctx->partials.p, tiles, L, ctx->results.p, ctx->P->labels.p, ctx->dense_one ? 1 : 0);
        HIPCHK(ctx, hipGetLastError());
    }
    if (ctx->timing) HIPCHK(ctx, hipEventRecord(ctx->ev2, ctx->stream));
    PinScalars& pin = ctx->pin[0];
    const size_t n_res = (size_t)n_rounds * L;
    if (tiles > 0 && ctx->dev_out)
        HIPCHK(ctx, hipMemcpyAsync(ctx->dev_out, ctx->results.p, n_res * sizeof(tpe_label_result),
                                   hipMemcpyDeviceToDevice, ctx->stream));
    const size_t res_bytes = n_res * sizeof(tpe_label_result);
    const int pieces = (tiles > 0 && out && res_bytes >= ((size_t)8 << 20)) ? tpe_ctx::kResPieces : 0;
    const size_t piece = ((res_bytes + std::max(pieces, 1) - 1) / std::max(pieces, 1) + 4095) & ~(size_t)4095;
    {
        int rc = defer_read(ctx, &pin.err, ctx->errflag.p, sizeof(int32_t));
        if (!rc) rc = defer_read(ctx, pin.xdrawn, ctx->xdrawn.p, 2 * sizeof(unsigned long long));
        if (!rc && tiles > 0 && out) HIPCHK(ctx, ctx->res_h.resize(n_res));
        if (!rc && pieces) {
            for (int k = 0; k < pieces; ++k) {
                const size_t a0 = std::min(res_bytes, k * piece), a1 = std::min(res_bytes, a0 + piece);
                if (!ctx->ev_res[k])
                    HIPCHK(ctx, hipEventCreateWithFlags(&ctx->ev_res[k], hipEventDisableTiming));
                if (a1 > a0)
                    HIPCHK(ctx, hipMemcpyAsync((char*)ctx->res_h.data() + a0, (const char*)ctx->results.p + a0,
                                               a1 - a0, hipMemcpyDeviceToHost, ctx->stream));
                HIPCHK(ctx, hipEventRecord(ctx->ev_res[k], ctx->stream));
            }
        } else if (!rc && tiles > 0 && out) {
            rc = defer_read(ctx, ctx->res_h.data(), ctx->results.p, res_bytes);
        }
        if (!rc) rc = flush_reads(ctx);
        if (rc) return rc;
    }
    for (int k = 0; k < pieces; ++k) {
        const size_t a0 = std::min(res_bytes, k * piece), a1 = std::min(res_bytes, a0 + piece);
        HIPCHK(ctx, hipEventSynchronize(ctx->ev_res[k]));
        if (a1 > a0) copy_out((char*)out + a0, (const char*)ctx->res_h.data() + a0, a1 - a0);
    }
    HIPCHK(ctx, hipStreamSynchronize(ctx->stream));
    unpack_reads(ctx);
    if (tiles > 0 && out && !pieces) copy_out(out, ctx->res_h.data(), res_bytes);
    if (tiles == 0 && out) std::memset(out, 0, res_bytes);
    if (ctx->zw_pending) {
        ctx->P->zw_ready = pin.plan.total > 0 && !pin.plan.sliced;
        ctx->zw_pending = false;
    }
    if (ctx->pk_plan_pending && pin.plan.overflow && !ctx->pk_redo) {
        ctx->pk_cap = pin.plan.total + pin.plan.total / 4 + 1024;
        ctx->pk_redo = true;
        const int rc = run_round(ctx, seed, rounds_h, n_rounds, n, cand_offset, cand_in_dev, olb, ola, out,
                                 only_label);
        ctx->pk_redo = false;
        return rc;
    }
    const int32_t errh = pin.err;
    ctx->xdrawn_h[0] = pin.xdrawn[0];
    ctx->xdrawn_h[1] = pin.xdrawn[1];
    if (dense_on) ctx->screen_ms = 0.f;
    if (ctx->screen_exec_pending) {
        ctx->screen_exec += (int64_t)ctx->pin[0].screen_exec;
        ctx->screen_exec_pending = false;
    }
    if (ctx->screen_pending) {
        const std::vector<int32_t>& gg = ctx->P->h_group[DENSE_GMM];
        const std::vector<int32_t>& gl = ctx->P->h_group[DENSE_LGMM];
        const size_t nld = gg.size() + gl.size();
        for (size_t c = 0; c < ctx->scr_cnt_h.size(); ++c) {
            const int32_t cnt = ctx->scr_cnt_h[c];
            const size_t y = c % nld;
            const DLabel& d = ctx->P->h_labels[y < gg.size() ? gg[y] : gl[y - gg.size()]];
            ctx->screen_rescored += cnt;
            ctx->screen_rescore_terms += (int64_t)cnt * (d.nb + d.na);
        }
        ctx->screen_pending = false;
        if (ctx->timing && ctx->evw_used > 0) {
            for (int32_t u = 0; u < ctx->evw_used; ++u) {
                float ms = 0.f;
                HIPCHK(ctx, hipEventElapsedTime(&ms, ctx->evw[2 * u], ctx->evw[2 * u + 1]));
                ctx->screen_ms += ms;
            }
        } else if (ctx->timing) {
            HIPCHK(ctx, hipEventElapsedTime(&ctx->screen_ms, ctx->evs[0], ctx->evs[1]));
        }
    }
    if (ctx->timing) {
        HIPCHK(ctx, hipEventElapsedTime(&ctx->score_ms, ctx->ev0, ctx->ev1));
        HIPCHK(ctx, hipEventElapsedTime(&ctx->round_ms, ctx->ev0, ctx->ev2));
    } else {
        ctx->score_ms = ctx->round_ms = 0.f;
    }
    for (int m = 0; m < kNumModes; ++m)
        if (ctx->mode_ran[m])
            if (ctx->timing)
                HIPCHK(ctx, hipEventElapsedTime(&ctx->mode_ms[m], ctx->evm[m][0], ctx->evm[m][1]));
    int64_t evals = 0;
    for (int32_t l = 0; l < L; ++l) {
        if (only_label >= 0 && l != only_label) continue;
        const DLabel& d = ctx->P->h_labels[l];
        if (!((fam >> d.mode) & 1)) continue;
        if (sample && (d.mode == QUANT_GMM || d.mode == QUANT_LGMM)) continue;
        if (d.mode == CAT && ctx->cat_early) continue;
        const int64_t e = ((d.mode == CAT) ? 2 * n : n * (int64_t)(d.nb + d.na)) * n_rounds;
        evals += e;
        const bool merged = sample && d.mode == DENSE_LGMM;
        ctx->mode_evals[merged ? DENSE_GMM : d.mode] += e;
    }
    ctx->mode_evals[QUANT_GMM] += evals_q[0];
    ctx->mode_evals[QUANT_LGMM] += evals_q[1];
    if (ctx->cat_early) {
        ctx->mode_evals[CAT] += 2 * (int64_t)ctx->xdrawn_h[1];
        evals += 2 * (int64_t)ctx->xdrawn_h[1];
    }
    ctx->evals = evals + evals_q[0] + evals_q[1];
    if (tiles == 0 && out) {
        for (int32_t j = 0; j < n_rounds * L; ++j)
            out[j] = tpe_label_result{NAN, NAN, NAN, NAN, -1, j % L, 0};
    }
    if (dense_on && ctx->hot_ran) {
        for (int64_t c = 0; c < ctx->hot_cells; ++c) ctx->hot_listed += ctx->hot_cnt_h[c];
        const int32_t hf = pin.hot_flag;
        if (hf && !ctx->hot_redo && errh == 0) {
            if ((hf & 2) && ctx->hot_cap_div > 1.0) ctx->hot_cap_div = std::max(1.0, ctx->hot_cap_div / 4.0);
            const int64_t listed = ctx->hot_listed;
            int64_t side_evals = 0;
            for (int m = QUANT_GMM; m <= CAT; ++m)
                if ((fam >> m) & 1) side_evals += ctx->mode_evals[m];
            const unsigned long long drawn0 = ctx->xdrawn_h[0], drawn1 = ctx->xdrawn_h[1];
            const bool cat_early = ctx->cat_early;
            const int32_t mask = ctx->mode_mask;
            ctx->mode_mask = fam & ((1 << DENSE_GMM) | (1 << DENSE_LGMM));
            ctx->hot_redo = true;
            const int rc = run_round(ctx, seed, rounds_h, n_rounds, n, cand_offset, cand_in_dev, olb, ola, out,
                                     only_label);
            ctx->hot_redo = false;
            ctx->mode_mask = mask;
            ctx->hot_ran = true;
            ctx->hot_fallback = hf;
            ctx->hot_listed = listed;
            ctx->evals += side_evals;
            ctx->xdrawn_h[0] = drawn0;
            ctx->xdrawn_h[1] = drawn1;
            ctx->cat_early = cat_early;
            return rc;
        }
    }
    if (errh & 1) return ctx->fail(TPE_ERR_SAMPLE, "truncated sampler: interval [low, high) not reached");
    if (errh & 2) return ctx->fail(TPE_ERR_VALUE, "negative arg to lognormal_cdf");
    if (errh & 4) return ctx->fail(TPE_ERR_VALUE, "categorical sample out of range");
    if (errh & 8) return ctx->fail(TPE_ERR_VALUE, "quantized sample beyond 2^52 grid steps");
    return TPE_OK;
}

__global__ __launch_bounds__(64) void k_samp_fold(const DLabel* __restrict__ labels, SampRec* __restrict__ samp) {
    const DLabel L = labels[blockIdx.x];
    (void)samp_fold_block(L, samp + L.samp_off, L.ns);
}

void launch_sample_only(tpe_ctx* ctx, int mode, int64_t n, int64_t offset, uint64_t seed,
                        double* out) {
    const int blocks = (int)((n + kBlock - 1) / kBlock);
#define TPE_SO(M)                                                                             \
    hipLaunchKernelGGL(k_sample_only<M>, dim3(blocks), dim3(kBlock), 0, ctx->stream,         \
                       ctx->P->labels.p, ctx->P->samp.p, n, offset, seed, ctx->rounds.p, out,       \
                       ctx->errflag.p)
    switch (mode) {
        case DENSE_GMM: TPE_SO(DENSE_GMM); break;
        case DENSE_LGMM: TPE_SO(DENSE_LGMM); break;
        case QUANT_GMM: TPE_SO(QUANT_GMM); break;
        case QUANT_LGMM: TPE_SO(QUANT_LGMM); break;
        default: TPE_SO(CAT); break;
    }
#undef TPE_SO
}

int set_posterior_impl(tpe_ctx* ctx, const tpe_label_desc* labels, int32_t n_labels,
                       const double* weights, const double* mus, const double* sigmas,
                       int64_t n_components, bool sampler_checks) {
    if (!ctx) return TPE_ERR_ARG;
    if (ctx->P == &ctx->resident) ctx->build.n_labels = 0;
    ctx->P->bx_prescan_ok = false;
    if (n_labels <= 0 || !labels || !weights) return ctx->fail(TPE_ERR_ARG, "empty posterior");
    HIPCHK(ctx, hipSetDevice(ctx->device));
    std::vector<DLabel> dl(n_labels);
    std::vector<Comp<double>> c64;
    std::vector<Comp<float>> c32;
    std::vector<SampRec> sr;
    std::vector<int32_t> grp[kNumModes];
    for (int32_t l = 0; l < n_labels; ++l) {
        const tpe_label_desc& d = labels[l];
        DLabel& o = dl[l];
        std::memset(&o, 0, sizeof(o));
        const bool quant = (d.flags & TPE_HAS_Q) != 0;
        if (d.kind == TPE_CATEGORICAL) o.mode = CAT;
        else if (d.kind == TPE_GMM1) o.mode = quant ? QUANT_GMM : DENSE_GMM;
        else if (d.kind == TPE_LGMM1) o.mode = quant ? QUANT_LGMM : DENSE_LGMM;
        else return ctx->fail(TPE_ERR_ARG, "label " + std::to_string(l) + ": unknown kind");
        if (d.n_below <= 0 || d.n_above <= 0 || d.below_off < 0 || d.above_off < 0 ||
            d.below_off + d.n_below > n_components || d.above_off + d.n_above > n_components)
            return ctx->fail(TPE_ERR_ARG, "label " + std::to_string(l) + ": component range");
        if (d.kind == TPE_CATEGORICAL && d.n_below != d.n_above)
            return ctx->fail(TPE_ERR_ARG, "categorical: below/above sizes differ");
        if (d.kind != TPE_CATEGORICAL) {
            if (!mus || !sigmas) return ctx->fail(TPE_ERR_ARG, "mus/sigmas required");
            int rc = validate_mixture(ctx, d.n_below, d.flags, d.low, d.high, sampler_checks);
            if (rc) return rc;
            if (quant && !(d.q > 0) && !(d.q < 0)) return ctx->fail(TPE_ERR_VALUE, "q must be non-zero");
        }
        o.flags = d.flags;
        o.low = d.low;
        o.high = d.high;
        o.q = d.q;
        o.exp_low = std::exp(d.low);
        o.exp_high = std::exp(d.high);
        o.nb = d.n_below;
        o.na = d.n_above;
        o.stream = l;
        if (d.kind != TPE_CATEGORICAL && !quant) {
            double lo = INFINITY, hi = -INFINITY;
            for (int side = 0; side < 2; ++side) {
                const int64_t off = side ? d.above_off : d.below_off;
                const int32_t n = side ? d.n_above : d.n_below;
                for (int k = 0; k < n; ++k) {
                    lo = std::min(lo, mus[off + k]);
                    hi = std::max(hi, mus[off + k]);
                }
            }
            o.centre = (std::isfinite(lo) && std::isfinite(hi)) ? 0.5 * lo + 0.5 * hi : 0.0;
        }
        for (int side = 0; side < 2; ++side) {
            const int64_t off = side ? d.above_off : d.below_off;
            const int32_t n = side ? d.n_above : d.n_below;
            const int64_t at = (int64_t)c64.size();
            c64.resize(at + n);
            c32.resize(at + n);
            if (d.kind == TPE_CATEGORICAL) {
                for (int k = 0; k < n; ++k) {
                    const double lp = std::log(weights[off + k]);
                    c64[at + k] = Comp<double>{0.0, 0.0, lp, weights[off + k]};
                    c32[at + k] = Comp<float>{0.f, 0.f, (float)lp, (float)weights[off + k]};
                }
            } else {
                Folded f = fold_mixture(d.kind, quant, d.flags, d.low, d.high, o.centre, weights + off,
                                        mus + off, sigmas + off, n, c64.data() + at, c32.data() + at);
                (side ? o.shift_a : o.shift_b) = f.shift;
                (side ? o.logpacc_a : o.logpacc_b) = f.logpacc;
                (side ? o.amax_a : o.amax_b) = (float)f.amax;
            }
            (side ? o.comp_a : o.comp_b) = at;
        }
        o.samp_off = (int64_t)sr.size();
        o.ns = d.n_below;
        double tot = 0.0;
        for (int k = 0; k < d.n_below; ++k) tot += weights[d.below_off + k];
        if (!(tot > 0) && sampler_checks) return ctx->fail(TPE_ERR_VALUE, "below weights sum to zero");
        for (int k = 0; k < d.n_below; ++k) {
            SampRec s{};
            s.mu = d.kind == TPE_CATEGORICAL ? 0.0 : mus[d.below_off + k];
            s.sigma = d.kind == TPE_CATEGORICAL ? 0.0 : sigmas[d.below_off + k];
            s.wd = weights[d.below_off + k];
            sr.push_back(s);
        }
        grp[o.mode].push_back(l);
    }
    std::vector<int32_t> cat;
    for (int m = 0; m < kNumModes; ++m) {
        ctx->P->group_off[m] = (int32_t)cat.size();
        cat.insert(cat.end(), grp[m].begin(), grp[m].end());
        ctx->P->h_group[m] = grp[m];
    }
    HIPCHK(ctx, ctx->P->labels.reserve(n_labels));
    HIPCHK(ctx, ctx->P->comps64.reserve(c64.size()));
    HIPCHK(ctx, ctx->P->comps32.reserve(c32.size()));
    HIPCHK(ctx, ctx->P->samp.reserve(sr.size()));
    HIPCHK(ctx, ctx->P->groups.reserve(cat.size()));
    HIPCHK(ctx, hipMemcpy(ctx->P->labels.p, dl.data(), dl.size() * sizeof(DLabel), hipMemcpyHostToDevice));
    HIPCHK(ctx, hipMemcpy(ctx->P->comps64.p, c64.data(), c64.size() * sizeof(Comp<double>), hipMemcpyHostToDevice));
    HIPCHK(ctx, hipMemcpy(ctx->P->comps32.p, c32.data(), c32.size() * sizeof(Comp<float>), hipMemcpyHostToDevice));
    HIPCHK(ctx, hipMemcpy(ctx->P->samp.p, sr.data(), sr.size() * sizeof(SampRec), hipMemcpyHostToDevice));
    HIPCHK(ctx, hipMemcpy(ctx->P->groups.p, cat.data(), cat.size() * sizeof(int32_t), hipMemcpyHostToDevice));
    hipLaunchKernelGGL(k_samp_fold, dim3((unsigned)n_labels), dim3(64), 0, ctx->stream, ctx->P->labels.p,
                       ctx->P->samp.p);
    HIPCHK(ctx, hipGetLastError());
    HIPCHK(ctx, hipStreamSynchronize(ctx->stream));
    ctx->P->groups_h = cat;
    ctx->P->h_labels = dl;
    ctx->P->win_ready = false;
    ctx->P->zw_ready = false;
    ctx->P->qc_ready = false;
    ctx->P->bx_ready = false;
    ctx->P->n_labels = n_labels;
    return TPE_OK;
}

}

double tpe_rt::np_pairwise_sum(const double* a, size_t n) {
    double r = 0.0;
    for (size_t c = 0; c < n; c += 8192) r += np_pairwise_sum_impl(a + c, std::min<size_t>(8192, n - c));
    return r;
}

int tpe_rt::qc_launch(tpe_ctx* ctx, hipStream_t st) {
    tpe_rt::Posterior& P = *ctx->P;
    const int nall = (int)(P.h_group[QUANT_GMM].size() + P.h_group[QUANT_LGMM].size());
    if (nall > 0) {
        HIPCHK(ctx, P.qcomp.reserve(P.comps64.cap));
        HIPCHK(ctx, P.qc_n.reserve(std::max(P.n_labels, 1)));
        hipLaunchKernelGGL(k_qcompress, dim3((unsigned)nall), dim3(kQcBlock), 0, st, P.labels.p,
                           P.groups.p + P.group_off[QUANT_GMM], P.comps64.p, P.qcomp.p, P.qc_n.p);
        HIPCHK(ctx, hipGetLastError());
    }
    P.qc_ready = true;
    return TPE_OK;
}

namespace {
__global__ __launch_bounds__(kBlock) void k_merge_results(const tpe_label_result* __restrict__ parts,
                                                          int32_t n_parts, int32_t n,
                                                          tpe_label_result* __restrict__ out,
                                                          int32_t* __restrict__ err) {
    const int32_t j = blockIdx.x * kBlock + threadIdx.x;
    if (j >= n) return;
    for (int32_t p = 0; p < n_parts; ++p) {
        const tpe_label_result* c = parts + (size_t)p * n + j;
        if (c->index >= 0 && c->status == TPE_STATUS_VALUE_ONLY) *err = 1;
    }
    int32_t bp = 0;
    int64_t bi = parts[j].index;
    uint64_t bk = order_key(parts[j].score);
    for (int32_t p = 1; p < n_parts; ++p) {
        const tpe_label_result* c = parts + (size_t)p * n + j;
        const int64_t ci = c->index;
        if (ci < 0) continue;
        const uint64_t ck = order_key(c->score);
        if (bi < 0 || better(ck, ci, bk, bi)) {
            bp = p;
            bi = ci;
            bk = ck;
        }
    }
    out[j] = parts[(size_t)bp * n + j];
}

}

extern "C" {

int tpe_abi_version(void) { return TPE_ABI_VERSION; }

#ifndef TPE_SOURCE_HASH
#define TPE_SOURCE_HASH "unstamped000000"
#endif
static const char kSourceStamp[] __attribute__((used)) = "TPE_SOURCE_HASH=" TPE_SOURCE_HASH;
const char* tpe_source_hash(void) { return kSourceStamp + 16; }

int tpe_ctx_create(int device, int precision, tpe_ctx** out) {
    if (!out) return TPE_ERR_ARG;
    *out = nullptr;
    if (precision != TPE_F64 && precision != TPE_F32) {
        g_create_error = "precision must be TPE_F64 or TPE_F32";
        return TPE_ERR_ARG;
    }
    int ndev = 0;
    hipError_t e = hipGetDeviceCount(&ndev);
    if (e != hipSuccess || device < 0 || device >= ndev) {
        g_create_error = std::string("no HIP device ") + std::to_string(device) + " (" +
                         (e == hipSuccess ? "count " + std::to_string(ndev) : hipGetErrorString(e)) + ")";
        return TPE_ERR_HIP;
    }
    e = hipSetDevice(device);
    if (e != hipSuccess) {
        g_create_error = hipGetErrorString(e);
        return TPE_ERR_HIP;
    }
    tpe_ctx* c = new tpe_ctx();
    c->device = device;
    c->precision = precision;
    bool ok = hipStreamCreateWithFlags(&c->stream, hipStreamNonBlocking) == hipSuccess &&
              hipEventCreate(&c->ev0) == hipSuccess && hipEventCreate(&c->ev1) == hipSuccess &&
              hipEventCreate(&c->ev2) == hipSuccess;
    for (int m = 0; m < kNumModes; ++m)
        ok = ok && hipEventCreate(&c->evm[m][0]) == hipSuccess &&
             hipEventCreate(&c->evm[m][1]) == hipSuccess;
    ok = ok && hipEventCreate(&c->evs[0]) == hipSuccess && hipEventCreate(&c->evs[1]) == hipSuccess;
    ok = ok && hipEventCreate(&c->ev_prep[0]) == hipSuccess && hipEventCreate(&c->ev_prep[1]) == hipSuccess;
    int prio_lo = 0, prio_hi = 0;
    (void)hipDeviceGetStreamPriorityRange(&prio_lo, &prio_hi);
    ok = ok && hipStreamCreateWithPriority(&c->aux, hipStreamNonBlocking, prio_hi) == hipSuccess &&
         hipEventCreateWithFlags(&c->ev_fork, hipEventDisableTiming) == hipSuccess &&
         hipEventCreateWithFlags(&c->ev_cat[0], hipEventDisableTiming) == hipSuccess &&
         hipEventCreateWithFlags(&c->ev_cat[1], hipEventDisableTiming) == hipSuccess;
    for (int j = 0; j < 2; ++j)
        ok = ok && hipEventCreateWithFlags(&c->ev_sorted[j], hipEventDisableTiming) == hipSuccess &&
             hipEventCreateWithFlags(&c->ev_done[j], hipEventDisableTiming) == hipSuccess;
    ok = ok && c->pin.resize(1) == hipSuccess;
    if (ok) c->pin[0] = PinScalars{};
    if (!ok) {
        g_create_error = "stream/event creation failed";
        tpe_ctx_destroy(c);
        return TPE_ERR_HIP;
    }
    *out = c;
    return TPE_OK;
}

TPE_DEV void tpe1_ctx_destroy(tpe_ctx* c) {
    if (!c) return;
    (void)hipSetDevice(c->device);
    if (c->stream) (void)hipStreamSynchronize(c->stream);
    if (c->aux) (void)hipStreamSynchronize(c->aux);
    c->resident.release();
    c->single.release();
    c->partials.release();
    c->results.release();
    c->rounds.release();
    c->errflag.release();
    c->build_err.release();
    c->cand.release();
    c->out_lb.release();
    c->out_la.release();
    c->one_group.release();
    c->qj.release();
    c->qmm.release();
    c->qinfo.release();
    c->qtab.release();
    c->xs.release();
    c->slice_part.release();
    c->build.release();
    if (c->ev0) (void)hipEventDestroy(c->ev0);
    if (c->ev1) (void)hipEventDestroy(c->ev1);
    if (c->ev2) (void)hipEventDestroy(c->ev2);
    for (int m = 0; m < kNumModes; ++m)
        for (int j = 0; j < 2; ++j)
            if (c->evm[m][j]) (void)hipEventDestroy(c->evm[m][j]);
    for (int j = 0; j < 2; ++j) {
        if (c->evs[j]) (void)hipEventDestroy(c->evs[j]);
        if (c->ev_prep[j]) (void)hipEventDestroy(c->ev_prep[j]);
    }
    for (hipEvent_t& e : c->ev_res)
        if (e) (void)hipEventDestroy(e);
    c->scr_hi.release();
    c->scr_idx.release();
    c->scr_range.release();
    c->rs_plan.release();
    c->scr_lb.release();
    c->scr_cnt.release();
    c->scr_chunks.release();
    c->scr_list.release();
    c->scr_res.release();
    c->scr_rsel.release();
    c->scr_off.release();
    c->scr_planes.release();
    c->chunk_part.release();
    for (int j = 0; j < 2; ++j) {
        c->win_keys[j].release();
        c->win_keys2[j].release();
        c->win_keys8[j].release();
        c->win_keys8b[j].release();
        c->win_vals[j].release();
        c->win_vals2[j].release();
        c->win_tmp[j].release();
        if (c->ev_sorted[j]) (void)hipEventDestroy(c->ev_sorted[j]);
        if (c->ev_done[j]) (void)hipEventDestroy(c->ev_done[j]);
    }
    c->win_evals.release();
    c->win_lohi.release();
    for (hipEvent_t e : c->evw) (void)hipEventDestroy(e);
    if (c->ev_fork) (void)hipEventDestroy(c->ev_fork);
    for (hipEvent_t e : c->ev_cat)
        if (e) (void)hipEventDestroy(e);
    if (c->aux) (void)hipStreamDestroy(c->aux);
    if (c->stream) (void)hipStreamDestroy(c->stream);
    delete c;
}

const char* tpe_last_error(const tpe_ctx* c) {
    return c ? c->err.c_str() : g_create_error.c_str();
}

TPE_DEV int tpe1_set_posterior(tpe_ctx* ctx, const tpe_label_desc* labels, int32_t n_labels,
                      const double* weights, const double* mus, const double* sigmas,
                      int64_t n_components) {
    TPE_SETTLE(ctx);
    return set_posterior_impl(ctx, labels, n_labels, weights, mus, sigmas, n_components, true);
}

TPE_DEV int tpe1_suggest(tpe_ctx* ctx, uint64_t seed, uint32_t round, int64_t n_candidates,
                int64_t cand_offset, tpe_label_result* out) {
    if (!ctx || !out) return TPE_ERR_ARG;
    HIPCHK(ctx, hipSetDevice(ctx->device));
    return run_round(ctx, seed, &round, 1, n_candidates, cand_offset, nullptr, nullptr, nullptr,
                     out, -1);
}

TPE_DEV int tpe1_suggest_batch(tpe_ctx* ctx, uint64_t seed, const uint32_t* rounds, int32_t n_rounds,
                      int64_t n_candidates, int64_t cand_offset, tpe_label_result* out) {
    if (!ctx || !out || !rounds) return TPE_ERR_ARG;
    HIPCHK(ctx, hipSetDevice(ctx->device));
    return run_round(ctx, seed, rounds, n_rounds, n_candidates, cand_offset, nullptr, nullptr,
                     nullptr, out, -1);
}

TPE_DEV int tpe1_score(tpe_ctx* ctx, int32_t label, const double* cand, int64_t n, double* lpdf_below,
                       double* lpdf_above, tpe_label_result* out) {
    if (!ctx || (!cand && n > 0)) return TPE_ERR_ARG;
    TPE_SETTLE(ctx);
    if (label < 0 || label >= ctx->P->n_labels) return ctx->fail(TPE_ERR_ARG, "label out of range");
    HIPCHK(ctx, hipSetDevice(ctx->device));
    const DLabel& d = ctx->P->h_labels[label];
    if (d.mode == QUANT_LGMM) {
        for (int64_t i = 0; i < n; ++i) {
            double ub = cand[i] + d.q / 2.0;
            if ((d.flags & 2) && ub > d.exp_high) ub = d.exp_high;
            if (ub < 0) return ctx->fail(TPE_ERR_VALUE, "negative arg to lognormal_cdf");
        }
    }
    if (d.mode == CAT) {
        for (int64_t i = 0; i < n; ++i)
            if (!(cand[i] >= 0 && cand[i] < d.nb) || cand[i] != std::floor(cand[i]))
                return ctx->fail(TPE_ERR_VALUE, "categorical sample out of range");
    }
    const size_t rows = (size_t)ctx->P->n_labels * std::max<int64_t>(n, 1);
    HIPCHK(ctx, ctx->cand.reserve(std::max<int64_t>(n, 1)));
    HIPCHK(ctx, ctx->out_lb.reserve(rows));
    HIPCHK(ctx, ctx->out_la.reserve(rows));
    if (n > 0)
        HIPCHK(ctx, hipMemcpyAsync(ctx->cand.p, cand, n * sizeof(double), hipMemcpyHostToDevice,
                                   ctx->stream));
    std::vector<tpe_label_result> all(ctx->P->n_labels);
    uint32_t round = 0;
    int rc = run_round(ctx, 0, &round, 1, n, 0, ctx->cand.p, ctx->out_lb.p, ctx->out_la.p,
                       all.data(), label);
    if (rc) return rc;
    const size_t row = (size_t)label * n;
    if (lpdf_below && n > 0)
        HIPCHK(ctx, hipMemcpy(lpdf_below, ctx->out_lb.p + row, n * sizeof(double), hipMemcpyDeviceToHost));
    if (lpdf_above && n > 0)
        HIPCHK(ctx, hipMemcpy(lpdf_above, ctx->out_la.p + row, n * sizeof(double), hipMemcpyDeviceToHost));
    if (out) {
        *out = all[label];
        if (n == 0) *out = tpe_label_result{NAN, NAN, NAN, NAN, -1, label, 0};
    }
    return TPE_OK;
}

int tpe_hot_probe(tpe_ctx* ctx, int32_t label, const double* cand, int64_t n, double* upper, double* lower,
                  double* mass) {
    if (!ctx || (n > 0 && (!cand || !upper || !lower || !mass))) return TPE_ERR_ARG;
    TPE_NOT_LSHARD(ctx);
    TPE_SETTLE(ctx);
    if (label < 0 || label >= ctx->P->n_labels) return ctx->fail(TPE_ERR_ARG, "label out of range");
    const DLabel& d = ctx->P->h_labels[label];
    if (d.mode != DENSE_GMM && d.mode != DENSE_LGMM)
        return ctx->fail(TPE_ERR_ARG, "hot probe: label is not a dense GMM1/LGMM1 label");
    HIPCHK(ctx, hipSetDevice(ctx->device));
    ctx->bx_t_next = kBxTTile;
    int rc = tpe_rt::bx_prepare(ctx);
    if (rc) return rc;
    tpe_rt::Posterior& P = *ctx->P;
    if (!P.bx_ok) return ctx->fail(TPE_ERR_ARG, "hot probe: the posterior has no expansion index");
    if (n == 0) return TPE_OK;
    HIPCHK(ctx, ctx->cand.reserve(n));
    HIPCHK(ctx, ctx->out_lb.reserve(n));
    HIPCHK(ctx, ctx->out_la.reserve(n));
    HIPCHK(ctx, ctx->xs.reserve(n));
    HIPCHK(ctx, hipMemcpyAsync(ctx->cand.p, cand, n * sizeof(double), hipMemcpyHostToDevice, ctx->stream));
    hipLaunchKernelGGL(k_hot_probe, dim3((unsigned)((n + kBlock - 1) / kBlock)), dim3(kBlock), 0, ctx->stream,
                       P.labels.p, P.bx.p, P.bx_sb.p, P.bx_sbp.p, label, ctx->cand.p, n, ctx->out_lb.p,
                       ctx->out_la.p, ctx->xs.p);
    HIPCHK(ctx, hipGetLastError());
    HIPCHK(ctx, hipMemcpyAsync(upper, ctx->out_lb.p, n * sizeof(double), hipMemcpyDeviceToHost, ctx->stream));
    HIPCHK(ctx, hipMemcpyAsync(lower, ctx->out_la.p, n * sizeof(double), hipMemcpyDeviceToHost, ctx->stream));
    HIPCHK(ctx, hipMemcpyAsync(mass, ctx->xs.p, n * sizeof(double), hipMemcpyDeviceToHost, ctx->stream));
    HIPCHK(ctx, hipStreamSynchronize(ctx->stream));
    return TPE_OK;
}

int tpe_screen_probe(tpe_ctx* ctx, int32_t label, const double* cand, int64_t n, double* score32,
                     double* err_bound) {
    if (!ctx || (n > 0 && (!cand || !score32 || !err_bound))) return TPE_ERR_ARG;
    TPE_NOT_LSHARD(ctx);
    TPE_SETTLE(ctx);
    if (label < 0 || label >= ctx->P->n_labels) return ctx->fail(TPE_ERR_ARG, "label out of range");
    const DLabel& d = ctx->P->h_labels[label];
    if (d.mode != DENSE_GMM && d.mode != DENSE_LGMM)
        return ctx->fail(TPE_ERR_ARG, "screen probe: label is not a dense GMM1/LGMM1 label");
    if (n == 0) return TPE_OK;
    HIPCHK(ctx, hipSetDevice(ctx->device));
    HIPCHK(ctx, ctx->cand.reserve(n));
    HIPCHK(ctx, ctx->out_lb.reserve(n));
    HIPCHK(ctx, ctx->out_la.reserve(n));
    HIPCHK(ctx, ctx->one_group.reserve(1));
    HIPCHK(ctx, ctx->rounds.reserve(1));
    HIPCHK(ctx, ctx->errflag.reserve(1));
    HIPCHK(ctx, hipMemcpyAsync(ctx->one_group.p, &label, sizeof(int32_t), hipMemcpyHostToDevice, ctx->stream));
    HIPCHK(ctx, hipMemcpyAsync(ctx->cand.p, cand, n * sizeof(double), hipMemcpyHostToDevice, ctx->stream));
    bool use_bx = false;
    if (ctx->expand && n >= 2048) {
        ctx->bx_t_next = kBxTTile;
        int rc = tpe_rt::bx_prepare(ctx);
        if (rc) return rc;
        use_bx = ctx->P->bx_ok;
    }
    if (use_bx) {
        tpe_rt::Posterior& P = *ctx->P;
        const unsigned bgx = (unsigned)((n + kBxR * kBlock - 1) / (kBxR * kBlock));
        hipLaunchKernelGGL((k_screen_bx<kBxR, false>), dim3(bgx, 1, 1), dim3(kBlock), 0, ctx->stream,
                           P.labels.p, ctx->one_group.p, P.comps64.p, P.samp.p, P.bx.p, P.bx_tab.p,
                           P.bx_loff.p, P.bx_list.p, n, 0, 0, ctx->rounds.p, 1, nullptr, nullptr, nullptr,
                           nullptr, nullptr, ctx->errflag.p, Slots{0, 0, 1}, ctx->cand.p, ctx->out_lb.p,
                           ctx->out_la.p, nullptr, (int64_t)0);
    } else if (ctx->window && n >= 2048) {
        int rc = tpe_rt::win_prepare(ctx);
        if (rc) return rc;
        if (n > ((int64_t)1 << 30)) return ctx->fail(TPE_ERR_ARG, "screen probe: too many candidates");
        const uint64_t* sorted = nullptr;
        tpe_rt::WinScreenArgs wa{ctx->one_group.p, 1, n, 0, 0, 0, 1, ctx->cand.p,
                                 nullptr, nullptr, ctx->out_lb.p, ctx->out_la.p};
        if ((rc = tpe_rt::win_screen(ctx, wa, &sorted))) return rc;
    } else {
        const uint32_t tiles = (uint32_t)((n + kTile - 1) / kTile);
        hipLaunchKernelGGL((k_screen<kR, false>), dim3(tiles, 1, 1), dim3(kBlock), 0, ctx->stream,
                           ctx->P->labels.p, ctx->one_group.p, ctx->P->comps32.p, ctx->P->samp.p, n, 0,
                           0, ctx->rounds.p, 1, nullptr, nullptr, ctx->errflag.p, Slots{0, 0, 1},
                           ctx->cand.p, ctx->out_lb.p, ctx->out_la.p);
    }
    HIPCHK(ctx, hipGetLastError());
    HIPCHK(ctx, hipMemcpyAsync(score32, ctx->out_lb.p, n * sizeof(double), hipMemcpyDeviceToHost, ctx->stream));
    HIPCHK(ctx, hipMemcpyAsync(err_bound, ctx->out_la.p, n * sizeof(double), hipMemcpyDeviceToHost, ctx->stream));
    HIPCHK(ctx, hipStreamSynchronize(ctx->stream));
    return TPE_OK;
}

int tpe_suggest_batch_device(tpe_ctx* ctx, uint64_t seed, const uint32_t* rounds, int32_t n_rounds,
                             int64_t n_candidates, int64_t cand_offset, tpe_label_result* d_out,
                             tpe_label_result* out) {
    if (!ctx || !d_out || !rounds) return TPE_ERR_ARG;
    TPE_NOT_LSHARD(ctx);
    if (!ctx->peers.empty()) return ctx->fail(TPE_ERR_ARG, "device results: single-device contexts only");
    HIPCHK(ctx, hipSetDevice(ctx->device));
    if (n_candidates <= 0) return ctx->fail(TPE_ERR_ARG, "device results need candidates");
    ctx->dev_out = d_out;
    const int rc = run_round(ctx, seed, rounds, n_rounds, n_candidates, cand_offset, nullptr, nullptr, nullptr, out,
                             -1);
    ctx->dev_out = nullptr;
    return rc;
}

int tpe_merge_results_device(tpe_ctx* ctx, const tpe_label_result* d_parts, int32_t n_parts, int32_t n,
                             tpe_label_result* d_out) {
    if (!ctx || !d_parts || !d_out || n_parts <= 0 || n < 0) return TPE_ERR_ARG;
    TPE_SETTLE(ctx);
    HIPCHK(ctx, hipSetDevice(ctx->device));
    if (n == 0) return TPE_OK;
    HIPCHK(ctx, ctx->errflag.reserve(1));
    HIPCHK(ctx, ctx->pin.resize(1));
    ctx->pin[0].err = 0;
    HIPCHK(ctx, hipMemsetAsync(ctx->errflag.p, 0, sizeof(int32_t), ctx->stream));
    hipLaunchKernelGGL(k_merge_results, dim3((unsigned)((n + kBlock - 1) / kBlock)), dim3(kBlock), 0, ctx->stream,
                       d_parts, n_parts, n, d_out, ctx->errflag.p);
    HIPCHK(ctx, hipGetLastError());
    HIPCHK(ctx, hipMemcpyAsync(&ctx->pin[0].err, ctx->errflag.p, sizeof(int32_t), hipMemcpyDeviceToHost,
                               ctx->stream));
    HIPCHK(ctx, hipStreamSynchronize(ctx->stream));
    if (ctx->pin[0].err)
        return ctx->fail(TPE_ERR_ARG, "tpe_merge_results_device: a part holds a value-only record "
                                      "(TPE_OPT_VALUE_ONLY): it has no score to merge by");
    return TPE_OK;
}

int tpe_merge_results(const tpe_label_result* parts, int32_t n_parts, int32_t n,
                      tpe_label_result* out) {
    if (!parts || !out || n_parts <= 0 || n < 0) return TPE_ERR_ARG;
    for (int64_t j = 0; j < (int64_t)n_parts * n; ++j)
        if (parts[j].index >= 0 && parts[j].status == TPE_STATUS_VALUE_ONLY) return TPE_ERR_ARG;
    for (int32_t j = 0; j < n; ++j) {
        tpe_label_result best = parts[j];
        for (int32_t p = 1; p < n_parts; ++p) {
            const tpe_label_result& c = parts[(size_t)p * n + j];
            if (c.index < 0) continue;
            if (best.index < 0 ||
                host_better(order_key(c.score), c.index, order_key(best.score), best.index))
                best = c;
        }
        out[j] = best;
    }
    return TPE_OK;
}

int tpe_last_timing(const tpe_ctx* ctx, float* score_ms, float* round_ms) {
    if (!ctx) return TPE_ERR_ARG;
    if (score_ms) *score_ms = ctx->score_ms;
    if (round_ms) *round_ms = ctx->round_ms;
    return TPE_OK;
}

int64_t tpe_last_evals(const tpe_ctx* ctx) { return ctx ? ctx->evals : -1; }

int tpe_last_screen(const tpe_ctx* ctx, int64_t* screened, int64_t* rescored, float* screen_ms) {
    if (!ctx) return TPE_ERR_ARG;
    if (screened) *screened = ctx->screen_total;
    if (rescored) *rescored = ctx->screen_rescored;
    if (screen_ms) *screen_ms = ctx->screen_ms;
    return TPE_OK;
}

int tpe_last_screen_terms(const tpe_ctx* ctx, int64_t* terms) {
    if (!ctx) return TPE_ERR_ARG;
    if (terms) *terms = ctx->screen_exec;
    return TPE_OK;
}

int32_t tpe_last_screen_mode(const tpe_ctx* ctx) { return ctx ? ctx->screen_mode : -1; }

int tpe_last_prepare(tpe_ctx* ctx, float* ms) {
    if (!ctx) return TPE_ERR_ARG;
    if (ctx->prep_pending) {
        HIPCHK(ctx, hipEventSynchronize(ctx->ev_prep[1]));
        HIPCHK(ctx, hipEventElapsedTime(&ctx->prep_ms, ctx->ev_prep[0], ctx->ev_prep[1]));
        ctx->prep_pending = false;
    }
    if (ms) *ms = ctx->prep_ms;
    return TPE_OK;
}

int tpe_last_hot(const tpe_ctx* ctx, int64_t* listed, int32_t* fallback) {
    if (!ctx) return TPE_ERR_ARG;
    if (listed) *listed = ctx->hot_ran ? ctx->hot_listed : -1;
    if (fallback) *fallback = ctx->hot_fallback;
    return TPE_OK;
}

int tpe_last_drawn(const tpe_ctx* ctx, int64_t* quantized, int64_t* categorical) {
    if (!ctx) return TPE_ERR_ARG;
    if (quantized) *quantized = (int64_t)ctx->xdrawn_h[0];
    if (categorical) *categorical = (int64_t)ctx->xdrawn_h[1];
    return TPE_OK;
}

int64_t tpe_device_bytes(void) { return tpe_rt::device_bytes_held().load(std::memory_order_relaxed); }

int tpe_last_rescore_terms(const tpe_ctx* ctx, int64_t* terms) {
    if (!ctx) return TPE_ERR_ARG;
    if (terms) *terms = ctx->screen_rescore_terms;
    return TPE_OK;
}

TPE_DEV int tpe1_prepare(tpe_ctx* ctx, int64_t n_candidates, int32_t n_rounds) {
    if (!ctx) return TPE_ERR_ARG;
    TPE_SETTLE(ctx);
    if (!ctx->P || ctx->P->n_labels <= 0) return ctx->fail(TPE_ERR_ARG, "no resident posterior");
    if (n_candidates < 0 || n_rounds < 1) return ctx->fail(TPE_ERR_ARG, "bad candidate/round count");
    if (ctx->precision != TPE_F64 || !ctx->screen || !ctx->expand || n_candidates * n_rounds < kWinMinN)
        return TPE_OK;
    HIPCHK(ctx, hipSetDevice(ctx->device));
    ctx->bx_t_next = n_candidates >= kTile ? kBxTTile : kBxT;
    int rc = tpe_rt::bx_prepare(ctx);
    if (rc == TPE_OK && ctx->hot && n_candidates >= kWinMinN) rc = hot_tau_prepare(ctx, n_candidates);
    return rc;
}

TPE_DEV int tpe1_arm_prepare(tpe_ctx* ctx, int64_t n_candidates, int32_t n_rounds) {
    if (!ctx) return TPE_ERR_ARG;
    TPE_SETTLE(ctx);
    if (n_candidates < 0 || (n_candidates > 0 && n_rounds < 1))
        return ctx->fail(TPE_ERR_ARG, "bad candidate/round count");
    ctx->arm_c = n_candidates;
    ctx->arm_r = n_candidates > 0 ? n_rounds : 0;
    return TPE_OK;
}

TPE_DEV int tpe1_set_option(tpe_ctx* ctx, int32_t option, int64_t value) {
    if (!ctx) return TPE_ERR_ARG;
    TPE_SETTLE(ctx);
    switch (option) {
        case TPE_OPT_SCREEN: ctx->screen = value != 0; break;
        case TPE_OPT_SPLITK: ctx->splitk = value != 0; break;
        case TPE_OPT_DEDUP: ctx->dedup = value != 0; break;
        case TPE_OPT_CHUNKS:
            if (value < 0 || value > 4096) return ctx->fail(TPE_ERR_ARG, "chunks must be in [0, 4096]");
            ctx->chunks_forced = (int32_t)value;
            break;
        case TPE_OPT_TIMING: ctx->timing = value != 0; break;
        case TPE_OPT_WINDOW: ctx->window = value != 0; break;
        case TPE_OPT_EXPAND: ctx->expand = value != 0; break;
        case TPE_OPT_EARLY: ctx->early = value != 0; break;
        case TPE_OPT_ZERO_WIN: ctx->zero_win = value != 0; break;
        case TPE_OPT_VALUE_ONLY: ctx->value_only = value != 0; break;
        case TPE_OPT_BX_T:
            if (value != 0 && (value < 32 || value > 128)) return ctx->fail(TPE_ERR_ARG, "index cut T must be 0 or in [32, 128]");
            ctx->bx_t_force = (int32_t)value;
            break;
        case TPE_OPT_PK_SLICED:
            if (value < 0 || value > kSlicedRescoreMax)
                return ctx->fail(TPE_ERR_ARG, "packed sliced re-score limit must be in [0, 65536]");
            ctx->pk_sliced = value;
            break;
        case TPE_OPT_DEFER_REPORT:
            if (!ctx->peers.empty() && value) return ctx->fail(TPE_ERR_ARG, "deferred reports: single-device contexts only");
            ctx->build.defer = value != 0;
            break;
        case TPE_OPT_BX_SPLIT:
            if (value < 0 || value > 8) return ctx->fail(TPE_ERR_ARG, "index window split must be in [0, 8]");
            ctx->bx_split = (int32_t)value;
            break;
        case TPE_OPT_MODE_MASK:
            if (value < 1 || value > 31) return ctx->fail(TPE_ERR_ARG, "family mask must be in [1, 31]");
            ctx->mode_mask = (int32_t)value;
            break;
        case TPE_OPT_AUX_FAMILIES: ctx->aux_families = value != 0; break;
        case TPE_OPT_RESCORE_CAP:
            if (value < 1) return ctx->fail(TPE_ERR_ARG, "re-score capacity must be positive");
            ctx->pk_cap = value;
            break;
        case TPE_OPT_HOT_DIV:
            if (value < 1 || value > (1 << 20)) return ctx->fail(TPE_ERR_ARG, "hot list divisor must be in [1, 2^20]");
            ctx->hot_cap_div = (double)value;
            break;
        case TPE_OPT_HOT:
            if (value < 0 || value > 2) return ctx->fail(TPE_ERR_ARG, "hot must be 0, 1 or 2");
            ctx->hot = (int32_t)value;
            break;
        case TPE_OPT_WIN_GROUPS:
            if (value < 0 || value > 64) return ctx->fail(TPE_ERR_ARG, "window groups must be in [0, 64]");
            ctx->win_groups = (int32_t)value;
            break;
        case TPE_OPT_WIN_T:
            if (value < 8 || value > 62) return ctx->fail(TPE_ERR_ARG, "window cut must be in [8, 62]");
            ctx->win_t = (int32_t)value;
            break;
        case TPE_OPT_WHOLE_N:
            if (value < 0) return ctx->fail(TPE_ERR_ARG, "whole candidate count must be >= 0");
            ctx->opt_whole_n = value;
            break;
        case TPE_OPT_WHOLE_ROUNDS:
            if (value < 0 || value > INT32_MAX) return ctx->fail(TPE_ERR_ARG, "whole round count");
            ctx->opt_whole_rounds = (int32_t)value;
            break;
        default: return ctx->fail(TPE_ERR_ARG, "unknown option " + std::to_string(option));
    }
    return TPE_OK;
}

int tpe_last_mode_stats(const tpe_ctx* ctx, float* ms, int64_t* evals) {
    if (!ctx) return TPE_ERR_ARG;
    for (int m = 0; m < kNumModes; ++m) {
        if (ms) ms[m] = ctx->mode_ms[m];
        if (evals) evals[m] = ctx->mode_evals[m];
    }
    return TPE_OK;
}


namespace {
struct SingleSlot {
    tpe_ctx* ctx;
    explicit SingleSlot(tpe_ctx* c) : ctx(c) { ctx->P = &ctx->single; }
    ~SingleSlot() { ctx->P = &ctx->resident; }
};
}

static int one_label_lpdf(tpe_ctx* ctx, int kind, const double* samples, int64_t n,
                          const double* w, const double* mu, const double* sg, int32_t k,
                          int32_t flags, double low, double high, double q, double* out) {
    if (!ctx) return TPE_ERR_ARG;
    SingleSlot slot(ctx);
    if (n == 0) return TPE_OK;
    if (!samples || !out || !w || !mu || !sg) return ctx->fail(TPE_ERR_ARG, "null pointer");
    tpe_label_desc d{};
    d.kind = kind;
    d.flags = flags;
    d.low = low;
    d.high = high;
    d.q = q;
    d.n_below = d.n_above = k;
    int rc = set_posterior_impl(ctx, &d, 1, w, mu, sg, k, false);
    if (rc) return rc;
    tpe_label_result r;
    return tpe_score(ctx, 0, samples, n, out, nullptr, &r);
}

int tpe_gmm1_lpdf(tpe_ctx* ctx, const double* samples, int64_t n, const double* weights,
                  const double* mus, const double* sigmas, int32_t k, int32_t flags, double low,
                  double high, double q, double* out) {
    TPE_SETTLE(ctx);
    return one_label_lpdf(ctx, TPE_GMM1, samples, n, weights, mus, sigmas, k, flags, low, high, q, out);
}

int tpe_lgmm1_lpdf(tpe_ctx* ctx, const double* samples, int64_t n, const double* weights,
                   const double* mus, const double* sigmas, int32_t k, int32_t flags, double low,
                   double high, double q, double* out) {
    TPE_SETTLE(ctx);
    return one_label_lpdf(ctx, TPE_LGMM1, samples, n, weights, mus, sigmas, k, flags, low, high, q, out);
}

int tpe_categorical_lpdf(tpe_ctx* ctx, const int64_t* samples, int64_t n, const double* p,
                         int32_t upper, double* out) {
    if (!ctx) return TPE_ERR_ARG;
    TPE_SETTLE(ctx);
    SingleSlot slot(ctx);
    if (n == 0) return TPE_OK;
    if (!samples || !p || !out || upper <= 0) return ctx->fail(TPE_ERR_ARG, "bad arguments");
    tpe_label_desc d{};
    d.kind = TPE_CATEGORICAL;
    d.n_below = d.n_above = upper;
    int rc = set_posterior_impl(ctx, &d, 1, p, nullptr, nullptr, upper, false);
    if (rc) return rc;
    std::vector<double> c(n);
    for (int64_t i = 0; i < n; ++i) c[i] = (double)samples[i];
    tpe_label_result r;
    return tpe_score(ctx, 0, c.data(), n, out, nullptr, &r);
}

int tpe_broadcast_best(tpe_ctx* ctx, const double* below, const double* above, int64_t n,
                       int64_t* best) {
    if (!ctx || !best) return TPE_ERR_ARG;
    if (n <= 0) {
        *best = -1;
        return TPE_OK;
    }
    HIPCHK(ctx, hipSetDevice(ctx->device));
    HIPCHK(ctx, ctx->out_lb.reserve(n));
    HIPCHK(ctx, ctx->out_la.reserve(n));
    const int blocks = (int)std::min<int64_t>((n + kBlock - 1) / kBlock, 1024);
    HIPCHK(ctx, ctx->partials.reserve(blocks));
    HIPCHK(ctx, hipMemcpyAsync(ctx->out_lb.p, below, n * sizeof(double), hipMemcpyHostToDevice, ctx->stream));
    HIPCHK(ctx, hipMemcpyAsync(ctx->out_la.p, above, n * sizeof(double), hipMemcpyHostToDevice, ctx->stream));
// ... 87 lines not shown
```

hyperopt_amd/csrc/tpe_multi.hip:

```cpp
#include <hip/hip_runtime.h>

#include <condition_variable>
#include <algorithm>
#include <functional>
#include <mutex>
#include <string>
#include <thread>
#include <vector>

#include "../../include/hyperopt_tpe.h"
#include "tpe_ctx.h"

namespace {

constexpr int64_t kMinShard = 1024;

int ndev(const tpe_ctx* c) { return 1 + (int)c->peers.size(); }

tpe_ctx* dev(tpe_ctx* c, int d) { return d == 0 ? c : c->peers[d - 1]; }

struct Workers {
    std::mutex mu;
    std::condition_variable cv_job, cv_done;
    const std::function<int(tpe_ctx*, int)>* job = nullptr;
// ... 476 lines not shown
        std::fill(ties, ties + L + 1, 0);
        for (int d = 0; d < nd; ++d) lsh_ties_merge(ctx->lsh_ids[d], td[d], L, ties);
    }
    return TPE_OK;
}

int tpe_rebuild_labels(tpe_ctx* ctx, const double* losses, int64_t n_trials, int64_t n_valid, double gamma,
                       double prior_weight, int32_t lf, const int64_t* order_off, const int32_t* order,
                       const int32_t* labels, int32_t n_only, int32_t* n_below_out, int32_t* ties) {
    if (!ctx) return TPE_ERR_ARG;
    if (!lsharded(ctx))
        return for_all(ctx, [&](tpe_ctx* x, int d) {
            return tpe1_rebuild_labels(x, losses, n_trials, n_valid, gamma, prior_weight, lf, order_off, order,
                                       labels, n_only, d == 0 ? n_below_out : nullptr, d == 0 ? ties : nullptr);
        });
    if (!labels || n_only <= 0 || !order_off) return ctx->fail(TPE_ERR_ARG, "tpe_rebuild_labels: no labels");
    const int nd = ndev(ctx);
    const int32_t L = ctx->lsh_L;
    std::vector<std::vector<int32_t>> td(nd);
    std::vector<int32_t> nbd(nd, -1);
    const int rc = for_all(ctx, [&](tpe_ctx* x, int d) {
        const std::vector<int32_t>& ids = ctx->lsh_ids[d];
        td[d].assign(ids.size() + 1, 0);
        std::vector<int32_t> mine;
        for (int32_t i = 0; i < n_only; ++i) {
            const int32_t g = labels[i];
            if (g < 0 || g >= L) return x->fail(TPE_ERR_ARG, "tpe_rebuild_labels: label out of range");
            if (ctx->lsh_dev[g] == d) mine.push_back(ctx->lsh_local[g]);
        }
        if (mine.empty()) return TPE_OK;
        std::vector<int64_t> off;
        std::vector<int32_t> ord;
        lsh_orders(ids, order_off, order, off, ord);
        return tpe1_rebuild_labels(x, losses, n_trials, n_valid, gamma, prior_weight, lf, off.data(), ord.data(),
                                   mine.data(), (int32_t)mine.size(), &nbd[d], td[d].data());
    });
    if (rc) return rc;
    if (n_below_out) {
        *n_below_out = 0;
        for (int d = 0; d < nd; ++d)
            if (nbd[d] >= 0) {
                *n_below_out = nbd[d];
                break;
            }
    }
    if (ties) {
        std::fill(ties, ties + L + 1, 0);
        for (int d = 0; d < nd; ++d) lsh_ties_merge(ctx->lsh_ids[d], td[d], L, ties);
    }
    return TPE_OK;
}

int tpe_build_report(tpe_ctx* ctx, int32_t* n_below, int32_t* ties) {
    if (!ctx) return TPE_ERR_ARG;
    if (!lsharded(ctx)) return tpe1_build_report(ctx, n_below, ties);
    const int nd = ndev(ctx);
    const int32_t L = ctx->lsh_L;
    std::vector<std::vector<int32_t>> td(nd);
    int32_t nb0 = 0;
    const int rc = for_all(ctx, [&](tpe_ctx* x, int d) {
        td[d].assign(ctx->lsh_ids[d].size() + 1, 0);
        return tpe1_build_report(x, d == 0 ? &nb0 : nullptr, td[d].data());
    });
    if (rc) return rc;
    if (n_below) *n_below = nb0;
    if (ties) {
        std::fill(ties, ties + L + 1, 0);
        for (int d = 0; d < nd; ++d) lsh_ties_merge(ctx->lsh_ids[d], td[d], L, ties);
    }
    return TPE_OK;
}

int tpe_get_mixture(tpe_ctx* ctx, int32_t label, int32_t side, double* weights, double* mus, double* sigmas,
                    int32_t cap, int32_t* n) {
    if (!ctx) return TPE_ERR_ARG;
    if (!lsharded(ctx)) return tpe1_get_mixture(ctx, label, side, weights, mus, sigmas, cap, n);
    if (label < 0 || label >= ctx->lsh_L) return ctx->fail(TPE_ERR_ARG, "tpe_get_mixture: no such built mixture");
    tpe_ctx* x = dev(ctx, ctx->lsh_dev[label]);
    HIPCHK(ctx, hipSetDevice(x->device));
    const int rc = tpe1_get_mixture(x, ctx->lsh_local[label], side, weights, mus, sigmas, cap, n);
    if (rc) ctx->err = x->err;
    return rc;
}

int32_t tpe_label_device(const tpe_ctx* ctx, int32_t label) {
    if (!ctx || !lsharded(ctx) || label < 0 || label >= ctx->lsh_L) return -1;
    return ctx->lsh_dev[label];
}

int32_t tpe_resident_labels(const tpe_ctx* ctx) {
    if (!ctx) return 0;
    return lsharded(ctx) ? ctx->lsh_L : tpe1_resident_labels(ctx);
}

int tpe_last_build_ms(const tpe_ctx* ctx, float* ms) {
    if (!ctx || !ms) return TPE_ERR_ARG;
    if (!lsharded(ctx)) return tpe1_last_build_ms(ctx, ms);
    float m = 0.f;
    for (int d = 0; d < ndev(const_cast<tpe_ctx*>(ctx)); ++d) {
        float v = 0.f;
        const int rc = tpe1_last_build_ms(dev(const_cast<tpe_ctx*>(ctx), d), &v);
        if (rc) return rc;
        m = std::max(m, v);
    }
    *ms = m;
    return TPE_OK;
}

int tpe_score(tpe_ctx* ctx, int32_t label, const double* cand, int64_t n, double* lpdf_below, double* lpdf_above,
              tpe_label_result* out) {
    if (!ctx) return TPE_ERR_ARG;
    if (!lsharded(ctx)) return tpe1_score(ctx, label, cand, n, lpdf_below, lpdf_above, out);
    if (label < 0 || label >= ctx->lsh_L) return ctx->fail(TPE_ERR_ARG, "tpe_score: label out of range");
    tpe_ctx* x = dev(ctx, ctx->lsh_dev[label]);
    HIPCHK(ctx, hipSetDevice(x->device));
    const int rc = tpe1_score(x, ctx->lsh_local[label], cand, n, lpdf_below, lpdf_above, out);
    if (rc) ctx->err = x->err;
    if (!rc && out) out->label = label;
    return rc;
}

int tpe_build_posterior(tpe_ctx* ctx, const tpe_label_spec* specs, int32_t n_labels,
                        const double* cat_p, int64_t n_cat_p, const double* losses,
                        int64_t n_trials, const int64_t* obs_off, const int32_t* obs_trial,
                        const double* obs_val, double gamma, double prior_weight, int32_t lf,
                        int32_t* n_below_out) {
    if (!ctx) return TPE_ERR_ARG;
    lsh_clear(ctx);
    return for_all(ctx, [&](tpe_ctx* x, int d) {
        return tpe1_build_posterior(x, specs, n_labels, cat_p, n_cat_p, losses, n_trials, obs_off,
                                    obs_trial, obs_val, gamma, prior_weight, lf,
                                    d == 0 ? n_below_out : nullptr);
    });
}

int tpe_suggest(tpe_ctx* ctx, uint64_t seed, uint32_t round, int64_t n_candidates,
                int64_t cand_offset, tpe_label_result* out) {
    if (!ctx || !out) return TPE_ERR_ARG;
    if (ctx->peers.empty()) return tpe1_suggest(ctx, seed, round, n_candidates, cand_offset, out);
    if (lsharded(ctx)) return lsh_round(ctx, seed, &round, 1, n_candidates, cand_offset, out);
    return sharded_round(ctx, seed, &round, 1, n_candidates, cand_offset, out);
}

int tpe_suggest_batch(tpe_ctx* ctx, uint64_t seed, const uint32_t* rounds, int32_t n_rounds,
                      int64_t n_candidates, int64_t cand_offset, tpe_label_result* out) {
    if (!ctx || !out || !rounds) return TPE_ERR_ARG;
    if (ctx->peers.empty())
        return tpe1_suggest_batch(ctx, seed, rounds, n_rounds, n_candidates, cand_offset, out);
    if (n_rounds <= 0) return ctx->fail(TPE_ERR_ARG, "bad candidate/round count");
    if (lsharded(ctx)) return lsh_round(ctx, seed, rounds, n_rounds, n_candidates, cand_offset, out);
    return sharded_round(ctx, seed, rounds, n_rounds, n_candidates, cand_offset, out);
}

}
```

hyperopt_amd/engine.py:

```python
import ctypes
import threading

import numpy as np

from . import _lib as L


class EngineError(RuntimeError):
    pass


def _raise(code, msg):
    msg = msg.decode() if isinstance(msg, bytes) else msg
    if code == L.TPE_ERR_VALUE:
        raise ValueError(msg)
    if code == L.TPE_ERR_TYPE:
        raise TypeError(msg)
    raise EngineError('%s (code %d)' % (msg, code))


def _ptr(a):
    return a.ctypes.data_as(ctypes.c_void_p) if a is not None else None


def _f64(a):
    return np.ascontiguousarray(np.asarray(a, dtype=np.float64))


RESULT_DTYPE = np.dtype([('value', '<f8'), ('score', '<f8'), ('lpdf_below', '<f8'),
                         ('lpdf_above', '<f8'), ('index', '<i8'), ('label', '<i4'),
                         ('status', '<i4')])
assert RESULT_DTYPE.itemsize == ctypes.sizeof(L.LabelResult)

DESC_DTYPE = np.dtype([('kind', '<i4'), ('flags', '<i4'), ('low', '<f8'), ('high', '<f8'),
                       ('q', '<f8'), ('below_off', '<i8'), ('above_off', '<i8'),
                       ('n_below', '<i4'), ('n_above', '<i4')])
assert DESC_DTYPE.itemsize == ctypes.sizeof(L.LabelDesc)


SPEC_DTYPE = np.dtype([('kind', '<i4'), ('flags', '<i4'), ('low', '<f8'), ('high', '<f8'),
                       ('q', '<f8'), ('prior_mu', '<f8'), ('prior_sigma', '<f8'),
                       ('upper', '<i4'), ('randint', '<i4'), ('p_off', '<i8'),
                       ('stream', '<i4'), ('reserved', '<i4')])
assert SPEC_DTYPE.itemsize == ctypes.sizeof(L.LabelSpec)


JOINT_DIM_DTYPE = np.dtype({'names': ['kind', 'flags', 'low', 'high', 'stream'],
                            'formats': ['<i4', '<i4', '<f8', '<f8', '<i4'],
                            'offsets': [0, 4, 8, 16, 24], 'itemsize': 32})
assert JOINT_DIM_DTYPE.itemsize == ctypes.sizeof(L.JointDim)


def bounds_flags(low, high, q):
    f = 0
    if low is not None:
        f |= L.TPE_HAS_LOW
    if high is not None:
        f |= L.TPE_HAS_HIGH
    if q is not None:
        f |= L.TPE_HAS_Q
    return f


DEFAULT_LF = 25


def _check_lf(lf):
    if int(lf) < DEFAULT_LF:
        raise ValueError('linear forgetting %d < gamma_cap %d: a below mixture would depend on '
                         'the order of its observations' % (int(lf), DEFAULT_LF))


def _devices(device):
    if isinstance(device, (list, tuple)):
        if not device:
            raise ValueError('devices must not be empty')
        return tuple(int(d) for d in device)
    return (int(device),)


class Engine(object):

    def __init__(self, device=0, precision='f64'):
        self.lib = L.load()
        self.precision = precision
        prec = {'f64': L.TPE_F64, 'f32': L.TPE_F32}[precision]
        devs = _devices(device)
        h = ctypes.c_void_p()
        if len(devs) == 1:
            rc = self.lib.tpe_ctx_create(devs[0], prec, ctypes.byref(h))
        else:
            arr = (ctypes.c_int * len(devs))(*devs)
            rc = self.lib.tpe_ctx_create_multi(arr, len(devs), prec, ctypes.byref(h))
        if rc != L.TPE_OK:
            raise EngineError('tpe_ctx_create(devices=%s): %s' % (
                list(devs), self.lib.tpe_last_error(None).decode()))
        self.h = h
        self.devices = devs
        self.device = devs[0]
        self.n_labels = 0
        self.history_generation = 0

    def close(self):
        if getattr(self, 'h', None):
            self.lib.tpe_ctx_destroy(self.h)
            self.h = None

    def __del__(self):
        try:
            self.close()
        except Exception:
            pass

    def _check(self, rc):
        if rc != L.TPE_OK:
            _raise(rc, self.lib.tpe_last_error(self.h))

    def set_posterior(self, descs, weights, mus, sigmas):
        descs = np.ascontiguousarray(descs, dtype=DESC_DTYPE)
        w, m, s = _f64(weights), _f64(mus), _f64(sigmas)
        self._check(self.lib.tpe_set_posterior(self.h, _ptr(descs), len(descs), _ptr(w),
                                               _ptr(m), _ptr(s), len(w)))
        self.n_labels = len(descs)

    def build_posterior(self, specs, cat_p, losses, obs_off, obs_trial, obs_val, gamma,
                        prior_weight, lf=25, tie_order='reference'):
        from . import posterior as _post
        _check_lf(lf)
        specs = np.ascontiguousarray(specs, dtype=SPEC_DTYPE)
        cat_p = _f64(cat_p)
        losses = _f64(losses)
        obs_off = np.ascontiguousarray(obs_off, dtype=np.int64)
        obs_trial = np.ascontiguousarray(obs_trial, dtype=np.int32)
        obs_val = _f64(obs_val)
        if tie_order == 'reference':
            self.history_reset(specs, cat_p)
            self.history_append(np.diff(obs_off), obs_trial, obs_val)
            n_valid = int(np.count_nonzero(losses == losses))
            nb, self.tie_labels = _post.build_reference_order(
                self, losses, n_valid, gamma, prior_weight, lf, _post._ObsOf(obs_off, obs_trial, obs_val))
            return nb
        if tie_order != 'position':
            raise ValueError("tie_order must be 'reference' or 'position'")
        nb = ctypes.c_int32()
        self.history_generation += 1
        self._check(self.lib.tpe_build_posterior(
            self.h, _ptr(specs), len(specs), _ptr(cat_p), len(cat_p), _ptr(losses), len(losses),
            _ptr(obs_off), _ptr(obs_trial), _ptr(obs_val), float(gamma), float(prior_weight),
            int(lf), ctypes.byref(nb)))
        self.n_labels = self.hist_labels = len(specs)
        return nb.value

    def history_reset(self, specs, cat_p):
        specs = np.ascontiguousarray(specs, dtype=SPEC_DTYPE)
        cat_p = _f64(cat_p)
        self.history_generation += 1
        self._check(self.lib.tpe_history_reset(self.h, _ptr(specs), len(specs), _ptr(cat_p),
                                               len(cat_p)))
        self.hist_labels = len(specs)

    def history_append(self, n_new, obs_trial, obs_val):
        n_new = np.ascontiguousarray(n_new, dtype=np.int64)
        obs_trial = np.ascontiguousarray(obs_trial, dtype=np.int32)
        obs_val = _f64(obs_val)
        self._check(self.lib.tpe_history_append(self.h, _ptr(n_new), _ptr(obs_trial),
                                                _ptr(obs_val)))

    def build_posterior_resident(self, losses, n_valid, gamma, prior_weight, lf=25):
        _check_lf(lf)
        losses = _f64(losses)
        nb = ctypes.c_int32()
        self._check(self.lib.tpe_build_posterior_resident(
            self.h, _ptr(losses), len(losses), int(n_valid), float(gamma), float(prior_weight),
            int(lf), ctypes.byref(nb)))
        self.n_labels = self.hist_labels
        return nb.value

    def build_posterior_ordered(self, losses, n_valid, gamma, prior_weight, lf=25, below=None,
                                order_off=None, order=None):
        _check_lf(lf)
        losses = _f64(losses)
        L_ = self.hist_labels
        if below is not None:
            below = np.ascontiguousarray(below, dtype=np.uint8)
            if len(below) != len(losses):
                raise ValueError('below mask must cover every trial position')
        if order_off is not None:
            order_off = np.ascontiguousarray(order_off, dtype=np.int64)
            order = np.ascontiguousarray(order, dtype=np.int32)
            if len(order_off) != L_ + 1 or order_off[-1] != len(order):
                raise ValueError('order offsets must be n_labels + 1 long and end at len(order)')
        nb = ctypes.c_int32()
        ties = np.zeros(L_ + 1, dtype=np.int32)
        self._check(self.lib.tpe_build_posterior_resident_ordered(
            self.h, _ptr(losses), len(losses), int(n_valid), float(gamma), float(prior_weight),
            int(lf), _ptr(below), _ptr(order_off), _ptr(order), ctypes.byref(nb), _ptr(ties)))
        self.n_labels = self.hist_labels
        return nb.value, ties

    def rebuild_labels(self, losses, n_valid, gamma, prior_weight, lf, order_off, order, labels,
                       defer=False):
        _check_lf(lf)
        losses = _f64(losses)
        L_ = self.hist_labels
        order_off = np.ascontiguousarray(order_off, dtype=np.int64)
        order = np.ascontiguousarray(order, dtype=np.int32)
        if len(order_off) != L_ + 1 or order_off[-1] != len(order):
            raise ValueError('order offsets must be n_labels + 1 long and end at len(order)')
        only = np.ascontiguousarray(sorted(int(l) for l in labels), dtype=np.int32)
        nb = ctypes.c_int32()
        ties = np.zeros(L_ + 1, dtype=np.int32)
        if defer:
            self.set_option('defer_report', 1)
        self._check(self.lib.tpe_rebuild_labels(
            self.h, _ptr(losses), len(losses), int(n_valid), float(gamma), float(prior_weight), int(lf),
            _ptr(order_off), _ptr(order), _ptr(only), len(only), ctypes.byref(nb), _ptr(ties)))
        return nb.value, ties

    def build_report(self):
        nb = ctypes.c_int32()
        ties = np.zeros(self.hist_labels + 1, dtype=np.int32)
        self._check(self.lib.tpe_build_report(self.h, ctypes.byref(nb), _ptr(ties)))
        return nb.value, ties

    def get_mixture(self, label, side):
        n = ctypes.c_int32()
        self._check(self.lib.tpe_get_mixture(self.h, int(label), int(side), None, None, None, 0,
                                             ctypes.byref(n)))
        w, m, s = np.empty(n.value), np.empty(n.value), np.empty(n.value)
        self._check(self.lib.tpe_get_mixture(self.h, int(label), int(side), _ptr(w), _ptr(m),
                                             _ptr(s), n.value, ctypes.byref(n)))
        return w, m, s

    def prepare(self, n_candidates, n_rounds=1):
        self._check(self.lib.tpe_prepare(self.h, int(n_candidates), int(n_rounds)))

    def arm_prepare(self, n_candidates, n_rounds=1):
        self._check(self.lib.tpe_arm_prepare(self.h, int(n_candidates), int(n_rounds)))

    def last_build_ms(self):
        ms = ctypes.c_float()
        self._check(self.lib.tpe_last_build_ms(self.h, ctypes.byref(ms)))
        return ms.value

    def _labels(self):
        self.n_labels = int(self.lib.tpe_resident_labels(self.h))
        return self.n_labels

    def suggest(self, seed, n_candidates, round=0, cand_offset=0):
        out = np.empty(self._labels(), dtype=RESULT_DTYPE)
        self._check(self.lib.tpe_suggest(self.h, int(seed) & 0xFFFFFFFFFFFFFFFF,
                                         int(round) & 0xFFFFFFFF, int(n_candidates),
                                         int(cand_offset), _ptr(out)))
        return out

    def suggest_batch(self, seed, rounds, n_candidates, cand_offset=0):
        rounds = np.ascontiguousarray(np.asarray(rounds, dtype=np.uint32))
        out = np.empty(len(rounds) * self._labels(), dtype=RESULT_DTYPE)
        self._check(self.lib.tpe_suggest_batch(self.h, int(seed) & 0xFFFFFFFFFFFFFFFF,
                                               _ptr(rounds), len(rounds), int(n_candidates),
                                               int(cand_offset), _ptr(out)))
        return out.reshape(len(rounds), self.n_labels)

    def suggest_batch_device(self, seed, rounds, n_candidates, d_out, cand_offset=0):
        rounds = np.ascontiguousarray(np.asarray(rounds, dtype=np.uint32))
        need = len(rounds) * self._labels() * RESULT_DTYPE.itemsize
        if not d_out.is_cuda or d_out.numel() * d_out.element_size() < need or not d_out.is_contiguous():
            raise ValueError('d_out must be a contiguous device tensor of %d bytes' % need)
        self._check_device(d_out, 'd_out')
        _torch_stream_done(d_out)
        self._check(self.lib.tpe_suggest_batch_device(
            self.h, int(seed) & 0xFFFFFFFFFFFFFFFF, _ptr(rounds), len(rounds), int(n_candidates),
            int(cand_offset), ctypes.c_void_p(d_out.data_ptr()), None))
        return d_out

    def _check_device(self, t, what):
        if len(self.devices) != 1 or t.device.index != self.device:
            raise ValueError('%s is on cuda:%s, this engine runs on cuda:%d%s'
                             % (what, t.device.index, self.device,
                                '' if len(self.devices) == 1 else ' (multi-device contexts take host buffers)'))

    def merge_results_device(self, d_parts, n_parts, n, d_out):
        rec = RESULT_DTYPE.itemsize
        for t, need, what in ((d_parts, n_parts * n * rec, 'd_parts'), (d_out, n * rec, 'd_out')):
            if not t.is_cuda or t.numel() * t.element_size() < need or not t.is_contiguous():
                raise ValueError('%s must be a contiguous device tensor of %d bytes' % (what, need))
            self._check_device(t, what)
        _torch_stream_done(d_parts)
        self._check(self.lib.tpe_merge_results_device(
            self.h, ctypes.c_void_p(d_parts.data_ptr()), int(n_parts), int(n),
            ctypes.c_void_p(d_out.data_ptr())))
        return d_out

    def export_size(self):
        n = ctypes.c_int64()
        self._check(self.lib.tpe_export_posterior(self.h, None, 0, ctypes.byref(n)))
        return int(n.value)

    def export_posterior(self, d_out):
        n = ctypes.c_int64()
        cap = d_out.numel() * d_out.element_size()
        if not d_out.is_cuda or not d_out.is_contiguous():
            raise ValueError('d_out must be a contiguous device tensor')
        self._check_device(d_out, 'd_out')
        _torch_stream_done(d_out)
        self._check(self.lib.tpe_export_posterior(self.h, ctypes.c_void_p(d_out.data_ptr()), cap,
                                                  ctypes.byref(n)))
        if n.value > cap:
            raise ValueError('d_out holds %d bytes, the posterior needs %d' % (cap, n.value))
        return int(n.value)

    def import_posterior(self, d_blobs, part_off, part_labels):
        if not d_blobs.is_cuda or not d_blobs.is_contiguous():
            raise ValueError('d_blobs must be a contiguous device tensor')
        self._check_device(d_blobs, 'd_blobs')
        off = np.ascontiguousarray(np.asarray(part_off, dtype=np.int64))
        counts = np.ascontiguousarray(np.asarray([len(p) for p in part_labels], dtype=np.int32))
        ids = np.ascontiguousarray(np.concatenate([np.asarray(p, dtype=np.int32) for p in part_labels]))
        if len(off) != len(counts):
            raise ValueError('one offset per part')
        _torch_stream_done(d_blobs)
        self._check(self.lib.tpe_import_posterior(
            self.h, ctypes.c_void_p(d_blobs.data_ptr()), d_blobs.numel() * d_blobs.element_size(),
            _ptr(off), len(off), _ptr(counts), _ptr(ids)))
        self._labels()

    def set_joint_posterior(self, dims, wb, mub, sigb, wa, mua, siga):
        dims = np.ascontiguousarray(dims, dtype=JOINT_DIM_DTYPE)
        D = len(dims)
        arrs = []
        for w, m, s in ((wb, mub, sigb), (wa, mua, siga)):
            w, m, s = _f64(w).ravel(), _f64(m), _f64(s)
            if m.shape != (len(w), D) or s.shape != (len(w), D):
                raise ValueError('joint means and sigmas must be [components, dimensions]')
            arrs.append((w, m, s))
        (wb, mub, sigb), (wa, mua, siga) = arrs
        rc = self.lib.tpe_joint_set_posterior(
            self.h, _ptr(dims), D, len(wb), _ptr(wb), _ptr(mub), _ptr(sigb), len(wa), _ptr(wa),
            _ptr(mua), _ptr(siga))
        self.joint_dims = D if rc in (L.TPE_OK, L.TPE_ERR_SAMPLE) else 0
        self._check(rc)

    def _joint_dims(self):
        D = getattr(self, 'joint_dims', 0)
        if not D:
            raise EngineError('no joint posterior set (Engine.set_joint_posterior)')
        return D

    def joint_draw(self, seed, n, round=0, cand_offset=0):
        D = self._joint_dims()
        values = np.empty((int(n), D))
        comp = np.empty(int(n), dtype=np.int32)
        self._check(self.lib.tpe_joint_draw(self.h, int(seed) & 0xFFFFFFFFFFFFFFFF, int(round) & 0xFFFFFFFF,
                                            int(n), int(cand_offset), _ptr(values), _ptr(comp)))
        return values, comp

    def joint_score(self, values):
        D = self._joint_dims()
        values = _f64(values)
        if values.ndim != 2 or values.shape[1] != D:
            raise ValueError('values must be [n, %d]' % D)
        ll, lg = np.empty(len(values)), np.empty(len(values))
        self._check(self.lib.tpe_joint_score(self.h, _ptr(values), len(values), _ptr(ll), _ptr(lg)))
        return ll, lg

    def joint_suggest(self, seed, n_candidates, round=0):
        D = self._joint_dims()
        values = np.empty(D)
        idx = ctypes.c_int64()
        ll, lg = ctypes.c_double(), ctypes.c_double()
        self._check(self.lib.tpe_joint_suggest(self.h, int(seed) & 0xFFFFFFFFFFFFFFFF,
                                               int(round) & 0xFFFFFFFF, int(n_candidates), _ptr(values),
                                               ctypes.byref(idx), ctypes.byref(ll), ctypes.byref(lg)))
        return values, int(idx.value), ll.value, lg.value

    def score(self, label, cand, want_lpdf=True):
        cand = _f64(cand).ravel()
        lb = np.empty(len(cand)) if want_lpdf else None
        la = np.empty(len(cand)) if want_lpdf else None
        out = np.zeros(1, dtype=RESULT_DTYPE)
        self._check(self.lib.tpe_score(self.h, int(label), _ptr(cand), len(cand), _ptr(lb),
                                       _ptr(la), _ptr(out)))
        return lb, la, out[0]

    def last_timing(self):
        a, b = ctypes.c_float(), ctypes.c_float()
        self._check(self.lib.tpe_last_timing(self.h, ctypes.byref(a), ctypes.byref(b)))
        return a.value, b.value

    def last_evals(self):
        return int(self.lib.tpe_last_evals(self.h))

    def last_screen(self, with_ms=False):
        a, b, ms = ctypes.c_int64(), ctypes.c_int64(), ctypes.c_float()
        self._check(self.lib.tpe_last_screen(self.h, ctypes.byref(a), ctypes.byref(b),
                                             ctypes.byref(ms)))
        return (a.value, b.value, ms.value) if with_ms else (a.value, b.value)

    def last_screen_terms(self):
        t = ctypes.c_int64()
        self._check(self.lib.tpe_last_screen_terms(self.h, ctypes.byref(t)))
        return t.value

    def last_screen_mode(self):
        return int(self.lib.tpe_last_screen_mode(self.h))

    def last_hot(self):
        a, b = ctypes.c_int64(), ctypes.c_int32()
        self._check(self.lib.tpe_last_hot(self.h, ctypes.byref(a), ctypes.byref(b)))
        return a.value, b.value
# ... 167 lines not shown
```

hyperopt_amd/posterior.py:

```python
import threading
import time
import weakref

import numpy as np

from . import _lib as L
from .engine import DESC_DTYPE

PHASES = None


def _phase(name, t0):
    t = time.perf_counter()
    if PHASES is not None:
        c = PHASES.setdefault(name, [0, 0.0])
        c[0] += 1
        c[1] += t - t0
    return t

EPS = 1e-12
DEFAULT_LF = 25

CONTINUOUS = ('uniform', 'quniform', 'loguniform', 'qloguniform',
              'normal', 'qnormal', 'lognormal', 'qlognormal')
# ... 212 lines not shown


def label_spec(kind, args):
    if kind in CATEGORICAL:
        upper = int(args['upper'])
        p = None if kind == 'randint' else np.asarray(args['p'], dtype=float)
        return dict(kind=L.TPE_CATEGORICAL, flags=0, upper=upper,
                    randint=1 if kind == 'randint' else 0), None, p
    if kind in ('uniform', 'quniform', 'loguniform', 'qloguniform'):
        low, high = float(args['low']), float(args['high'])
        spec = dict(low=low, high=high, prior_mu=0.5 * (high + low), prior_sigma=1.0 * (high - low),
                    flags=L.TPE_HAS_LOW | L.TPE_HAS_HIGH)
        if kind in ('quniform', 'qloguniform'):
            spec['q'] = float(args['q'])
            spec['flags'] |= L.TPE_HAS_Q
        if kind in ('uniform', 'quniform'):
            spec['kind'], tr = L.TPE_GMM1, None
        elif kind == 'loguniform':
            spec['kind'], tr = L.TPE_LGMM1, np.log
        else:
            floor = np.maximum(EPS, np.exp(low))
            spec['kind'], tr = L.TPE_LGMM1, (lambda o: np.log(np.maximum(o, floor)))
            tr.floor = float(floor)
        return spec, tr, None
    spec = dict(prior_mu=float(args['mu']), prior_sigma=float(args['sigma']), flags=0)
    if kind in ('qnormal', 'qlognormal'):
        spec['q'] = float(args['q'])
        spec['flags'] = L.TPE_HAS_Q
    if kind in ('normal', 'qnormal'):
        spec['kind'], tr = L.TPE_GMM1, None
    elif kind == 'lognormal':
        spec['kind'], tr = L.TPE_LGMM1, np.log
    elif kind == 'qlognormal':
        spec['kind'], tr = L.TPE_LGMM1, (lambda o: np.log(np.maximum(o, EPS)))
        tr.floor = float(EPS)
    else:
        raise ValueError('unknown distribution %r' % kind)
    return spec, tr, None


def spec_table(labels, streams=None):
    from .engine import SPEC_DTYPE
    specs = np.zeros(len(labels), dtype=SPEC_DTYPE)
    cat_p, p_len, trs = [], 0, []
    for i, (name, kind, args) in enumerate(labels):
        sp, tr, p = label_spec(kind, args)
        for k, v in sp.items():
            specs[i][k] = v
        if p is not None:
            specs[i]['p_off'] = p_len
            cat_p.append(p)
            p_len += len(p)
        if streams is not None:
            specs[i]['flags'] |= L.TPE_HAS_STREAM
            specs[i]['stream'] = int(streams[i])
        trs.append(tr)
    return specs, (np.concatenate(cat_p) if cat_p else np.zeros(0)), trs


def n_below_of(n_valid, gamma, gamma_cap=DEFAULT_LF):
    return int(min(np.ceil(gamma * np.sqrt(n_valid)), gamma_cap))


def reference_orders(losses, n_below, obs_of, labels):
    losses = np.asarray(losses, dtype=np.float64)
    T = len(losses)
    has = losses == losses
    valid = np.flatnonzero(has)
    lv = losses[valid]
    below = np.zeros(T, dtype=np.uint8)
    if 0 < n_below < len(lv):
        part = np.partition(lv, (n_below - 1, n_below))
        if part[n_below - 1] < part[n_below]:
            below[valid[lv <= part[n_below - 1]]] = 1
        else:
            below[valid[np.argsort(lv)[:n_below]]] = 1
    elif n_below > 0:
        below[valid] = 1
    above = has & (below == 0)
    n_labels = obs_of.n_labels
    off = np.zeros(n_labels + 1, dtype=np.int64)
    jobs = []
    n_above = None
    for l in range(n_labels):
        n = 0
        if l in labels:
            pos, val = obs_of(l)
            val = np.asarray(val, dtype=np.float64)
            if len(pos) == T and T and pos[0] == 0 and pos[-1] == T - 1:
                sel = above
                if n_above is None:
                    n_above = int(np.count_nonzero(above))
                n = n_above
            else:
                pos = np.asarray(pos, dtype=np.int64)
                ok = (pos >= 0) & (pos < T)
                sel = np.zeros(len(pos), dtype=bool)
                sel[ok] = above[pos[ok]]
                n = int(np.count_nonzero(sel))
            jobs.append((l, val, sel))
        off[l + 1] = off[l] + n
    order = np.empty(int(off[-1]), dtype=np.int32)

    def sort_one(job):
        l, val, sel = job
        order[off[l]:off[l + 1]] = np.argsort(val[sel])

    if jobs and off[-1] >= _POOL_MIN:
        for _ in _sort_pool().map(sort_one, jobs):
            pass
    else:
        for job in jobs:
            sort_one(job)
    return below, off, order


EARLY_ORDERS = True
_order_exec = None


def _order_thread():
    global _order_exec
    if _order_exec is None:
        with _pool_lock:
            if _order_exec is None:
                from concurrent.futures import ThreadPoolExecutor
                _order_exec = ThreadPoolExecutor(max_workers=1)
    return _order_exec


_POOL_MIN = 1 << 14
SORT_THREADS = 16
_pool = None
_pool_lock = threading.Lock()


def _sort_pool():
    global _pool
    if _pool is None:
        with _pool_lock:
            if _pool is None:
                import os
                from concurrent.futures import ThreadPoolExecutor
                try:
                    ncpu = len(os.sched_getaffinity(0))
                except (AttributeError, OSError):
                    ncpu = os.cpu_count() or 2
                _pool = ThreadPoolExecutor(max_workers=max(1, min(SORT_THREADS, ncpu)))
    return _pool


SUBSET_REBUILD = True
DEFER_REPORT = True


def build_reference_order(eng, losses, n_valid, gamma, prior_weight, lf, obs_of, known=(), prepare=None,
                          overlap=True, round_call=None, early=None):
    holder = {'early': early}
    try:
        return _build_reference_order(eng, losses, n_valid, gamma, prior_weight, lf, obs_of, known,
                                      prepare, overlap, round_call, holder)
    finally:
        if holder['early'] is not None:
            from concurrent.futures import wait
            wait([holder['early']])


def _build_reference_order(eng, losses, n_valid, gamma, prior_weight, lf, obs_of, known, prepare,
                           overlap, round_call, holder):
    early = holder['early']
    n_below = n_below_of(n_valid, gamma)
    known = set(known)
    t0 = time.perf_counter()
    if prepare and (overlap or not known):
        if known and EARLY_ORDERS and early is None:
            early = holder['early'] = _order_thread().submit(reference_orders, losses, n_below, obs_of,
                                                             known)
        eng.arm_prepare(*prepare)
        nb, ties = eng.build_posterior_ordered(losses, n_valid, gamma, prior_weight, lf)
        t0 = _phase('build', t0)
        eng.prepare(*prepare)
        t0 = _phase('prepare_enqueue', t0)
        have = set()
    elif known:
        below, off, order = reference_orders(losses, n_below, obs_of, known)
        t0 = _phase('argsorts', t0)
        if prepare:
            eng.arm_prepare(*prepare)
        nb, ties = eng.build_posterior_ordered(losses, n_valid, gamma, prior_weight, lf, below, off, order)
        t0 = _phase('build', t0)
        if prepare:
            eng.prepare(*prepare)
            t0 = _phase('prepare_enqueue', t0)
        have = known
    else:
        nb, ties = eng.build_posterior_ordered(losses, n_valid, gamma, prior_weight, lf)
        t0 = _phase('build', t0)
        have = set()
    if np.any(ties[:-1] & 1):
        raise AssertionError('below mixture depends on a tie order (lf < gamma_cap?)')
    need = have | set(np.flatnonzero(ties[:-1] & 2).tolist())
    res = None
    deferred = False
    if early is not None:
        orders = early.result()
        if need != have and need <= known:
            need = set(known)
            below, off, order = orders
        else:
            early = None
    if need != have or ties[-1]:
        if early is None:
            below, off, order = reference_orders(losses, n_below, obs_of, need)
        t0 = _phase('argsorts', t0)
        if SUBSET_REBUILD and not ties[-1] and len(need) < obs_of.n_labels:
            deferred = (DEFER_REPORT and round_call is not None and len(getattr(eng, 'devices', ())) == 1
                        and hasattr(eng, 'build_report'))
            nb, ties = eng.rebuild_labels(losses, n_valid, gamma, prior_weight, lf, off, order, need,
                                          defer=deferred)
        else:
            nb, ties = eng.build_posterior_ordered(losses, n_valid, gamma, prior_weight, lf, below, off,
                                                   order)
        t0 = _phase('rebuild', t0)
        if np.any(ties[:-1]):
            need |= set(np.flatnonzero(ties[:-1] & 2).tolist())
            below, off, order = reference_orders(losses, n_below, obs_of, need)
            nb, ties = eng.build_posterior_ordered(losses, n_valid, gamma, prior_weight, lf, below, off,
                                                   order)
            assert not np.any(ties[:-1])
    if round_call is not None:
        res = round_call()
        if deferred:
            nb, ties = eng.build_report()
            if np.any(ties[:-1]):
                need |= set(np.flatnonzero(ties[:-1] & 2).tolist())
                below, off, order = reference_orders(losses, n_below, obs_of, need)
                nb, ties = eng.build_posterior_ordered(losses, n_valid, gamma, prior_weight, lf, below, off,
                                                       order)
                assert not np.any(ties[:-1])
                res = round_call()
        _phase('round', t0)
        return nb, frozenset(need), res
    return nb, frozenset(need)


class _ObsOf(object):

    def __init__(self, obs_off, obs_trial, obs_val):
        self.off, self.trial, self.val = obs_off, obs_trial, obs_val
        self.n_labels = len(obs_off) - 1

    def __call__(self, l):
        a, b = int(self.off[l]), int(self.off[l + 1])
        return self.trial[a:b], self.val[a:b]


class NonFiniteObservation(ValueError):
    """A transformed observation is NaN (e.g. the log of a non-positive value
    of a log-scale label inserted through points_to_evaluate).  The
    reference's adaptive_parzen_normal then trips its `sigma > 0` assertion
    (tpe.py:469) in the host build; the device builder cannot order NaN
    keys, so it refuses them (tpe.suggest falls back to the host builder)."""


def _check_finite(label, vals):
    if np.isnan(vals).any():
        raise NonFiniteObservation('label %r: NaN observation value' % (label,))


class DeviceHistoryUploader(object):

    def __init__(self):
        self.key = None
        self.owner = None

    def build(self, eng, labels, view, gamma, prior_weight, lf=DEFAULT_LF, prepare=None, streams=None,
              overlap=True, round_call=None):
        tids, losses, n_valid, cols, owner = view
        names_now = tuple(n for n, _, _ in labels)
        if (labels is not self._labels_obj or streams is not self._streams_obj or
                names_now != self._names_t):
            self._labels_obj, self._streams_obj, self._names_t = labels, streams, names_now
            self._label_key = (tuple((n, k) for n, k, _ in labels) +
                               (tuple(streams) if streams is not None else (),))
            self._names = [n for n, _, _ in labels]
        key = (self._label_key, eng.history_generation)
        names = self._names
        obs_now = [cols[n] for n in names]
        lens = [len(o[0]) for o in obs_now]
        same_owner = self.owner is not None and self.owner() is owner
        fresh = (not same_owner or self.key != key or len(tids) < self.n_trials or
                 (self.n_trials and tids[self.n_trials - 1] != self.last_tid) or
                 any(a < c for a, c in zip(lens, self.prev_counts)))
        self.key, self.owner = None, None
        if fresh:
            specs, cat_p, self.trs = spec_table(labels, streams)
            self.tr_kind = np.array([0 if t is None else (1 if t is np.log else 2) for t in self.trs])
            self.tr_floor = np.array([getattr(t, 'floor', -np.inf) for t in self.trs])
            eng.history_reset(specs, cat_p)
            self.prev_counts = [0] * len(labels)
            self.pos_parts = [[] for _ in labels]
            self.val_parts = [[] for _ in labels]
            self.tie_labels = frozenset()
        t0 = time.perf_counter()
        counts = lens
        n_new = [a - c for a, c in zip(lens, self.prev_counts)]
        ni_l = [o[0][c:] for o, c, m in zip(obs_now, self.prev_counts, n_new) if m]
        nv_l = [o[1][c:] for o, c, m in zip(obs_now, self.prev_counts, n_new) if m]
        if ni_l:
            ni = np.concatenate(ni_l)
            raw = np.asarray(np.concatenate(nv_l), dtype=float)
            lab = np.repeat(np.arange(len(labels)), n_new)
            kind = self.tr_kind[lab]
            vals = raw.copy()
            lg = kind > 0
            if lg.any():
                vals[lg] = np.log(np.maximum(raw[lg], self.tr_floor[lab[lg]]))
            nan = np.isnan(vals)
            if nan.any():
                raise NonFiniteObservation('label %r: NaN observation value'
                                           % (labels[int(lab[np.argmax(nan)])][0],))
            pos = np.searchsorted(tids, ni)
            pc = np.minimum(pos, len(tids) - 1)
            trial = np.where(tids[pc] == ni, pc, -1).astype(np.int32)
            o = 0
            for i, m in enumerate(n_new):
                if m:
                    self.pos_parts[i].append(trial[o:o + m])
                    self.val_parts[i].append(vals[o:o + m])
                    o += m
        if ni_l:
            eng.history_append(np.asarray(n_new, dtype=np.int64), trial, vals)
        self.prev_counts = counts
        self.key = (key[0], eng.history_generation)
        self.owner = weakref.ref(owner)
        self.n_trials = len(tids)
        self.last_tid = tids[-1] if len(tids) else None
        _phase('append', t0)
        out = build_reference_order(eng, losses, n_valid, gamma, prior_weight, lf,
                                    self._obs_of(len(labels)), self.tie_labels,
                                    prepare=prepare, overlap=overlap, round_call=round_call)
        self.tie_labels = out[1]
        return out[0], (out[2] if round_call is not None else None)

    def _obs_of(self, n_labels):
        def obs_of(l):
            for parts in (self.pos_parts, self.val_parts):
                if len(parts[l]) > 1:
                    parts[l][:] = [np.concatenate(parts[l])]
            if not self.pos_parts[l]:
                return np.zeros(0, np.int32), np.zeros(0)
            return self.pos_parts[l][0], self.val_parts[l][0]
        obs_of.n_labels = n_labels
        return obs_of

    prev_counts = ()
    _labels_obj = _streams_obj = _names_t = None
    pos_parts = val_parts = ()
    tie_labels = frozenset()
    n_trials = 0
    last_tid = None
    trs = ()


def device_inputs(labels, tids, losses, obs):
    from .engine import SPEC_DTYPE
    tids = np.asarray(tids, dtype=np.int64)
    specs = np.zeros(len(labels), dtype=SPEC_DTYPE)
    cat_p, p_len = [], 0
    off = [0]
    trial_parts, val_parts = [], []
    for i, (name, kind, args) in enumerate(labels):
        sp, tr, p = label_spec(kind, args)
        for k, v in sp.items():
            specs[i][k] = v
        if p is not None:
            specs[i]['p_off'] = p_len
            cat_p.append(p)
            p_len += len(p)
        oi, ov = obs[name]
        oi = np.asarray(oi, dtype=np.int64)
        ov = np.asarray(ov, dtype=float)
        if tr is not None and len(ov):
            ov = tr(ov)
# ... 52 lines not shown
```

include/hyperopt_tpe.h:

```cpp
#ifndef HYPEROPT_TPE_H
#define HYPEROPT_TPE_H

#include <stdint.h>

#ifdef __cplusplus
extern "C" {
#endif

#define TPE_ABI_VERSION 4

#define TPE_OK 0
#define TPE_ERR_VALUE (-1)
#define TPE_ERR_TYPE (-2)
#define TPE_ERR_ARG (-3)
#define TPE_ERR_HIP (-4)
#define TPE_ERR_SAMPLE (-5)

#define TPE_F64 0
#define TPE_F32 1

#define TPE_GMM1 0
#define TPE_LGMM1 1
#define TPE_CATEGORICAL 2

#define TPE_HAS_LOW 1
#define TPE_HAS_HIGH 2
#define TPE_HAS_Q 4
#define TPE_HAS_STREAM 8

typedef struct tpe_ctx tpe_ctx;

typedef struct {
    int32_t kind;
    int32_t flags;
    double low;
    double high;
    double q;
    int64_t below_off;
    int64_t above_off;
    int32_t n_below;
    int32_t n_above;
} tpe_label_desc;

#define TPE_OBS_IDENTITY 0
#define TPE_OBS_LOG 1
#define TPE_OBS_LOG_FLOOR 2

typedef struct {
    int32_t kind;
    int32_t flags;
    double low;
    double high;
    double q;
    double prior_mu;
    double prior_sigma;
    int32_t upper;
    int32_t randint;
    int64_t p_off;
    int32_t stream;
    int32_t reserved;
} tpe_label_spec;

typedef struct {
    double value;
    double score;
    double lpdf_below;
    double lpdf_above;
    int64_t index;
    int32_t label;
    int32_t status;
} tpe_label_result;

#define TPE_STATUS_VALUE_ONLY 1

int tpe_abi_version(void);

const char *tpe_source_hash(void);

int tpe_ctx_create(int device, int precision, tpe_ctx **out);

int tpe_ctx_create_multi(const int *devices, int32_t n_devices, int precision, tpe_ctx **out);

int32_t tpe_ctx_devices(const tpe_ctx *ctx, int32_t *devices, int32_t cap);

int32_t tpe_label_device(const tpe_ctx *ctx, int32_t label);

void tpe_ctx_destroy(tpe_ctx *ctx);
const char *tpe_last_error(const tpe_ctx *ctx);


int tpe_gmm1_lpdf(tpe_ctx *ctx, const double *samples, int64_t n,
                  const double *weights, const double *mus, const double *sigmas,
                  int32_t k, int32_t flags, double low, double high, double q,
                  double *out);

int tpe_lgmm1_lpdf(tpe_ctx *ctx, const double *samples, int64_t n,
                   const double *weights, const double *mus, const double *sigmas,
                   int32_t k, int32_t flags, double low, double high, double q,
                   double *out);

int tpe_categorical_lpdf(tpe_ctx *ctx, const int64_t *samples, int64_t n,
                         const double *p, int32_t upper, double *out);

int tpe_broadcast_best(tpe_ctx *ctx, const double *below, const double *above,
                       int64_t n, int64_t *best);

int tpe_gmm1_sample(tpe_ctx *ctx, const double *weights, const double *mus,
                    const double *sigmas, int32_t k, int32_t flags, double low,
                    double high, double q, uint64_t seed, uint32_t stream,
                    uint32_t round, int64_t offset, int64_t n, double *out);

int tpe_lgmm1_sample(tpe_ctx *ctx, const double *weights, const double *mus,
                     const double *sigmas, int32_t k, int32_t flags, double low,
                     double high, double q, uint64_t seed, uint32_t stream,
                     uint32_t round, int64_t offset, int64_t n, double *out);

int tpe_categorical_sample(tpe_ctx *ctx, const double *p, int32_t upper,
                           uint64_t seed, uint32_t stream, uint32_t round,
                           int64_t offset, int64_t n, int64_t *out);


int tpe_set_posterior(tpe_ctx *ctx, const tpe_label_desc *labels, int32_t n_labels,
                      const double *weights, const double *mus, const double *sigmas,
                      int64_t n_components);

int tpe_build_posterior(tpe_ctx *ctx, const tpe_label_spec *specs, int32_t n_labels,
                        const double *cat_p, int64_t n_cat_p,
                        const double *losses, int64_t n_trials,
                        const int64_t *obs_off, const int32_t *obs_trial,
                        const double *obs_val, double gamma, double prior_weight,
                        int32_t lf, int32_t *n_below_out);

int tpe_history_reset(tpe_ctx *ctx, const tpe_label_spec *specs, int32_t n_labels,
                      const double *cat_p, int64_t n_cat_p);
int tpe_history_append(tpe_ctx *ctx, const int64_t *n_new, const int32_t *obs_trial,
                       const double *obs_val);
int tpe_build_posterior_resident(tpe_ctx *ctx, const double *losses, int64_t n_trials,
                                 int64_t n_valid, double gamma, double prior_weight,
                                 int32_t lf, int32_t *n_below_out);

int tpe_build_posterior_resident_ordered(tpe_ctx *ctx, const double *losses, int64_t n_trials,
                                         int64_t n_valid, double gamma, double prior_weight,
                                         int32_t lf, const uint8_t *below, const int64_t *order_off,
                                         const int32_t *order, int32_t *n_below_out, int32_t *ties);

int tpe_rebuild_labels(tpe_ctx *ctx, const double *losses, int64_t n_trials, int64_t n_valid,
                       double gamma, double prior_weight, int32_t lf, const int64_t *order_off,
                       const int32_t *order, const int32_t *labels, int32_t n_only,
                       int32_t *n_below_out, int32_t *ties);

int tpe_get_mixture(tpe_ctx *ctx, int32_t label, int32_t side, double *weights,
                    double *mus, double *sigmas, int32_t cap, int32_t *n);

int32_t tpe_resident_labels(const tpe_ctx *ctx);

int tpe_last_build_ms(const tpe_ctx *ctx, float *ms);

int tpe_build_report(tpe_ctx *ctx, int32_t *n_below, int32_t *ties);

int tpe_suggest(tpe_ctx *ctx, uint64_t seed, uint32_t round, int64_t n_candidates,
                int64_t cand_offset, tpe_label_result *out);

int tpe_suggest_batch(tpe_ctx *ctx, uint64_t seed, const uint32_t *rounds,
                      int32_t n_rounds, int64_t n_candidates, int64_t cand_offset,
                      tpe_label_result *out);

int tpe_suggest_batch_device(tpe_ctx *ctx, uint64_t seed, const uint32_t *rounds,
                             int32_t n_rounds, int64_t n_candidates, int64_t cand_offset,
                             tpe_label_result *d_out, tpe_label_result *out);

int tpe_merge_results_device(tpe_ctx *ctx, const tpe_label_result *d_parts, int32_t n_parts,
                             int32_t n, tpe_label_result *d_out);

int tpe_export_posterior(tpe_ctx *ctx, void *d_out, int64_t cap, int64_t *bytes);
int tpe_import_posterior(tpe_ctx *ctx, const void *d_blobs, int64_t blob_bytes, const int64_t *part_off,
                         int32_t n_parts, const int32_t *part_labels, const int32_t *label_ids);

#define TPE_JOINT_STREAM 0x7FFFFFFF

typedef struct {
    int32_t kind;
    int32_t flags;
    double low, high;
    int32_t stream;
} tpe_joint_dim;

int tpe_joint_set_posterior(tpe_ctx *ctx, const tpe_joint_dim *dims, int32_t n_dims,
                            int32_t n_below, const double *wb, const double *mub, const double *sigb,
                            int32_t n_above, const double *wa, const double *mua, const double *siga);
int tpe_joint_draw(tpe_ctx *ctx, uint64_t seed, uint32_t round, int64_t n, int64_t cand_offset,
                   double *values, int32_t *comp);
int tpe_joint_score(tpe_ctx *ctx, const double *values, int64_t n, double *ll, double *lg);
int tpe_joint_suggest(tpe_ctx *ctx, uint64_t seed, uint32_t round, int64_t n_candidates,
                      double *values, int64_t *index, double *ll, double *lg);

int tpe_score(tpe_ctx *ctx, int32_t label, const double *cand, int64_t n,
              double *lpdf_below, double *lpdf_above, tpe_label_result *out);

int tpe_merge_results(const tpe_label_result *parts, int32_t n_parts, int32_t n,
                      tpe_label_result *out);

int tpe_last_timing(const tpe_ctx *ctx, float *score_ms, float *round_ms);

int64_t tpe_last_evals(const tpe_ctx *ctx);

int tpe_last_mode_stats(const tpe_ctx *ctx, float *ms, int64_t *evals);

int tpe_last_screen(const tpe_ctx *ctx, int64_t *screened, int64_t *rescored,
                    float *screen_ms);

int tpe_last_screen_terms(const tpe_ctx *ctx, int64_t *terms);

int tpe_last_rescore_terms(const tpe_ctx *ctx, int64_t *terms);

int tpe_last_drawn(const tpe_ctx *ctx, int64_t *quantized, int64_t *categorical);

int64_t tpe_device_bytes(void);

int32_t tpe_last_screen_mode(const tpe_ctx *ctx);

int tpe_last_hot(const tpe_ctx *ctx, int64_t *listed, int32_t *fallback);

int tpe_last_prepare(tpe_ctx *ctx, float *ms);

int tpe_hot_probe(tpe_ctx *ctx, int32_t label, const double *cand, int64_t n,
                  double *upper, double *lower, double *mass);

int tpe_screen_probe(tpe_ctx *ctx, int32_t label, const double *cand, int64_t n,
                     double *score32, double *err_bound);

#define TPE_OPT_SCREEN 1
#define TPE_OPT_SPLITK 2
#define TPE_OPT_DEDUP 3
#define TPE_OPT_CHUNKS 4
#define TPE_OPT_WHOLE_N 5
#define TPE_OPT_WHOLE_ROUNDS 6
#define TPE_OPT_TIMING 7
#define TPE_OPT_WINDOW 8
#define TPE_OPT_WIN_T 9
#define TPE_OPT_WIN_GROUPS 10
#define TPE_OPT_EXPAND 11
#define TPE_OPT_HOT 12
#define TPE_OPT_EARLY 13
#define TPE_OPT_HOT_DIV 14
#define TPE_OPT_ZERO_WIN 15
#define TPE_OPT_VALUE_ONLY 16
#define TPE_OPT_RESCORE_CAP 17
#define TPE_OPT_MODE_MASK 18
#define TPE_OPT_AUX_FAMILIES 19
#define TPE_OPT_BX_SPLIT 21
#define TPE_OPT_BX_T 22
#define TPE_OPT_PK_SLICED 23
#define TPE_OPT_DEFER_REPORT 24
#define TPE_OPT_LABEL_SHARDS 25
int tpe_set_option(tpe_ctx *ctx, int32_t option, int64_t value);

int tpe_prepare(tpe_ctx *ctx, int64_t n_candidates, int32_t n_rounds);

int tpe_arm_prepare(tpe_ctx *ctx, int64_t n_candidates, int32_t n_rounds);

#ifdef __cplusplus
}
#endif

#endif
```

Measured before the change: 46.05 billion.

## Split suggest round into begin/finish to overlap dense scoring with label rebuild

Adds suggest_begin/suggest_finish so the dense GMM/LGMM scoring of a round can be launched before the host finishes computing tie-breaking orders and rebuilding only categorical or quantized labels. The quantized and categorical pass is then run in the finish phase after the subset rebuild lands. This aims to hide the host-side ordering and rebuild latency behind the dense kernel. In exchange it adds state tracking, discard paths that run the round when a full rebuild is needed, and untimed builds while a round is in flight.

```diff
diff --git a/hyperopt_amd/_lib.py b/hyperopt_amd/_lib.py
--- a/hyperopt_amd/_lib.py
+++ b/hyperopt_amd/_lib.py
@@ -11,6 +11,7 @@
 TPE_ERR_VALUE = -1
 TPE_ERR_TYPE = -2
 TPE_ERR_ARG = -3
+TPE_ROUND_NOT_STARTED = 1
 TPE_STATUS_VALUE_ONLY = 1
 TPE_ERR_HIP = -4
 TPE_ERR_SAMPLE = -5
@@ -117,6 +118,9 @@
     'tpe_set_posterior': (ctypes.c_int, [_P, _P, _I32, _P, _P, _P, _I64]),
     'tpe_suggest': (ctypes.c_int, [_P, _U64, _U32, _I64, _I64, _P]),
     'tpe_suggest_batch': (ctypes.c_int, [_P, _U64, _P, _I32, _I64, _I64, _P]),
+    'tpe_suggest_begin': (ctypes.c_int, [_P, _U64, _P, _I32, _I64, _I64]),
+    'tpe_suggest_finish': (ctypes.c_int, [_P, _P]),
+    'tpe_round_state': (ctypes.c_int, [_P, _P, _P]),
     'tpe_score': (ctypes.c_int, [_P, _I32, _P, _I64, _P, _P, _P]),
     'tpe_merge_results': (ctypes.c_int, [_P, _I32, _I32, _P]),
     'tpe_suggest_batch_device': (ctypes.c_int, [_P, _U64, _P, _I32, _I64, _I64, _P, _P]),
diff --git a/hyperopt_amd/csrc/tpe_build.hip b/hyperopt_amd/csrc/tpe_build.hip
--- a/hyperopt_amd/csrc/tpe_build.hip
+++ b/hyperopt_amd/csrc/tpe_build.hip
@@ -1480,7 +1480,7 @@
     std::memcpy(B.last_ties.data(), B.h_rep.data() + rep_dl + 16, (n_labels + 1) * sizeof(int32_t));
     B.last_n_below = t.n_below;
     if (ties_out) std::memcpy(ties_out, B.last_ties.data(), (n_labels + 1) * sizeof(int32_t));
-    if (t.deferred) ctx->build_ms = -1.f;
+    if (t.deferred || t.untimed) ctx->build_ms = -1.f;
     else HIPCHK(ctx, hipEventElapsedTime(&ctx->build_ms, ctx->ev0, ctx->ev1));
     if (errh & 1) return ctx->fail(TPE_ERR_ARG, "observation trial position out of range");
     if (errh & 2) return ctx->fail(TPE_ERR_ARG, "more below observations than the below set (duplicate trial in a label?)");
@@ -1693,7 +1693,8 @@
         HIPCHK(ctx, hipGetLastError());
     }
 
-    HIPCHK(ctx, hipEventRecord(ctx->ev0, st));
+    const bool untimed = ctx->begun.active;
+    if (!untimed) HIPCHK(ctx, hipEventRecord(ctx->ev0, st));
     if (T > 0 && !below_h && !subset) {
         const int rc = launch_split(ctx, st, B.losses.p, T, n_below, B.below.p, B.ties.p + n_labels);
         if (rc) return rc;
@@ -1713,7 +1714,7 @@
                        B.scratch.p, B.scratch.p + 2 * total, B.scratch.p + 3 * total, B.scratch.p + total,
                        ctx->build_err.p, only_d);
     HIPCHK(ctx, hipGetLastError());
-    HIPCHK(ctx, hipEventRecord(ctx->ev1, st));
+    if (!untimed) HIPCHK(ctx, hipEventRecord(ctx->ev1, st));
     const int64_t rep_dl = (int64_t)n_labels * (int64_t)sizeof(DLabel);
     const int64_t rep_bytes = rep_dl + 16 + (int64_t)(n_labels + 1) * (int64_t)sizeof(int32_t);
     HIPCHK(ctx, B.d_rep.reserve(rep_bytes));
@@ -1759,6 +1760,7 @@
     t.beside = beside;
     t.qc_queued = qc_queued;
     t.subset = subset;
+    t.untimed = untimed;
     t.n_trials = n_trials;
     t.n_valid = n_valid;
     t.arm_c = arm_c;
@@ -1781,6 +1783,13 @@
 
 int tpe_rt::settle_build(tpe_ctx* ctx) {
     if (!ctx) return TPE_OK;
+    const int rc = tpe_rt::discard_round(ctx);
+    if (rc) return rc;
+    return tpe_rt::apply_pending(ctx);
+}
+
+int tpe_rt::apply_pending(tpe_ctx* ctx) {
+    if (!ctx) return TPE_OK;
     auto& B = ctx->build;
     if (!B.pending) return TPE_OK;
     std::unique_ptr<BuildTail> t = std::move(B.pending);
@@ -1826,7 +1835,15 @@
                                 const int32_t* order, const int32_t* labels, int32_t n_only,
                                 int32_t* n_below_out, int32_t* ties) {
     if (!ctx) return TPE_ERR_ARG;
-    TPE_SETTLE(ctx);
+    bool keep = ctx->begun.active && labels && n_only > 0;
+    for (int32_t i = 0; keep && i < n_only; ++i) {
+        keep = labels[i] >= 0 && labels[i] < (int32_t)ctx->build.specs_h.size();
+        if (!keep) break;
+        const tpe_label_spec& s = ctx->build.specs_h[labels[i]];
+        keep = s.kind == TPE_CATEGORICAL || (s.flags & TPE_HAS_Q) != 0;
+    }
+    if (keep) TPE_SETTLE_KEEP(ctx);
+    else TPE_SETTLE(ctx);
     if (!labels || n_only <= 0) return ctx->fail(TPE_ERR_ARG, "tpe_rebuild_labels: no labels");
     return build_resident(ctx, losses, n_trials, n_valid, gamma, prior_weight, lf, n_below_out, nullptr,
                           order_off, order, ties, labels, n_only);
diff --git a/hyperopt_amd/csrc/tpe_ctx.h b/hyperopt_amd/csrc/tpe_ctx.h
--- a/hyperopt_amd/csrc/tpe_ctx.h
+++ b/hyperopt_amd/csrc/tpe_ctx.h
@@ -262,6 +262,7 @@
     std::vector<int32_t> grp[kNumModes];
     std::vector<int64_t> mix;
     bool beside = false, qc_queued = false, subset = false, deferred = false;
+    bool untimed = false;
     int64_t n_trials = 0, n_valid = 0, arm_c = 0;
     int32_t arm_r = 0;
     bool prescan = false;
@@ -269,6 +270,15 @@
     uint64_t loss_hash = 0;
 };
 int settle_build(tpe_ctx* ctx);
+int apply_pending(tpe_ctx* ctx);
+int discard_round(tpe_ctx* ctx);
+
+struct BegunRound {
+    bool active = false;
+    uint64_t seed = 0;
+    std::vector<uint32_t> rounds;
+    int64_t n = 0, cand_offset = 0;
+};
 
 struct BuildBufs {
     std::vector<tpe_label_spec> specs_h;
@@ -509,6 +519,8 @@
     int64_t built_n_trials = 0;
     int32_t built_n_below = 0;
     float build_ms = 0.f;
+    tpe_rt::BegunRound begun;
+    int64_t begun_discards = 0;
 
     std::vector<tpe_ctx*> peers;
     std::shared_ptr<void> workers;
@@ -574,6 +586,11 @@
         const int settle_rc_ = tpe_rt::settle_build(ctx); \
         if (settle_rc_) return settle_rc_;                \
     } while (0)
+#define TPE_SETTLE_KEEP(ctx)                               \
+    do {                                                   \
+        const int settle_rc_ = tpe_rt::apply_pending(ctx); \
+        if (settle_rc_) return settle_rc_;                 \
+    } while (0)
 
 #define TPE_DEV __attribute__((visibility("hidden")))
 extern "C" {
@@ -585,6 +602,9 @@
 TPE_DEV int tpe1_suggest_batch(tpe_ctx* ctx, uint64_t seed, const uint32_t* rounds,
                                int32_t n_rounds, int64_t n_candidates, int64_t cand_offset,
                                tpe_label_result* out);
+TPE_DEV int tpe1_suggest_begin(tpe_ctx* ctx, uint64_t seed, const uint32_t* rounds, int32_t n_rounds,
+                               int64_t n_candidates, int64_t cand_offset);
+TPE_DEV int tpe1_suggest_finish(tpe_ctx* ctx, tpe_label_result* out);
 TPE_DEV int tpe1_set_option(tpe_ctx* ctx, int32_t option, int64_t value);
 TPE_DEV int tpe1_prepare(tpe_ctx* ctx, int64_t n_candidates, int32_t n_rounds);
 TPE_DEV int tpe1_arm_prepare(tpe_ctx* ctx, int64_t n_candidates, int32_t n_rounds);
diff --git a/hyperopt_amd/csrc/tpe_engine.hip b/hyperopt_amd/csrc/tpe_engine.hip
--- a/hyperopt_amd/csrc/tpe_engine.hip
+++ b/hyperopt_amd/csrc/tpe_engine.hip
@@ -4014,15 +4014,38 @@
     return ctx->hip(hipGetLastError(), "split-K launch");
 }
 
+enum { kRoundWhole = 0, kRoundBegin = 1, kRoundFinish = 2 };
+
+bool begin_eligible(const tpe_ctx* ctx, int64_t n) {
+    const tpe_rt::Posterior& P = *ctx->P;
+    int64_t nd = 0, ns = 0;
+    for (int m = 0; m < kNumModes; ++m) {
+        if (!((ctx->mode_mask >> m) & 1)) continue;
+        (m == DENSE_GMM || m == DENSE_LGMM ? nd : ns) += (int64_t)P.h_group[m].size();
+    }
+    return ctx->peers.empty() && !ctx->qx && !ctx->dev_out && ctx->hint_n == 0 && ctx->precision == TPE_F64 &&
+           ctx->screen && ctx->expand && n >= kTile && n >= kWinMinN && P.bx_ready && P.bx_ok && nd > 0 &&
+           (ns == 0 || (ctx->aux_families && ctx->aux)) && !ctx->hot_redo && !ctx->pk_redo;
+}
+
 int run_round(tpe_ctx* ctx, uint64_t seed, const uint32_t* rounds_h, int32_t n_rounds, int64_t n,
               int64_t cand_offset, const double* cand_in_dev, double* olb, double* ola,
-              tpe_label_result* out, int32_t only_label) {
+              tpe_label_result* out, int32_t only_label, int phase = kRoundWhole) {
+    if (phase != kRoundFinish) {
+        const int rc = tpe_rt::discard_round(ctx);
+        if (rc) return rc;
+    }
     if (ctx->P->n_labels == 0) return ctx->fail(TPE_ERR_ARG, "no posterior set (tpe_set_posterior)");
     if (n < 0 || n_rounds <= 0) return ctx->fail(TPE_ERR_ARG, "bad candidate/round count");
     if (cand_offset < 0 || cand_offset + n > (int64_t)UINT32_MAX)
         return ctx->fail(TPE_ERR_ARG, "candidate indices must stay below 2^32");
-    if (!(ctx->build.pending && only_label < 0 && cand_in_dev == nullptr && n > 0 && ctx->aux_families &&
-          ctx->aux && !ctx->qx))
+    if (phase == kRoundBegin) {
+        TPE_SETTLE(ctx);
+        if (!begin_eligible(ctx, n)) return TPE_ROUND_NOT_STARTED;
+    }
+    const bool fin = phase == kRoundFinish;
+    if (!fin && !(ctx->build.pending && only_label < 0 && cand_in_dev == nullptr && n > 0 && ctx->aux_families &&
+                  ctx->aux && !ctx->qx))
         TPE_SETTLE(ctx);
     Slots S{0, 0, n_rounds};
     int32_t tiles;
@@ -4040,15 +4063,15 @@
         gz = (uint32_t)n_rounds;
     }
     const int32_t L = ctx->P->n_labels;
-    ctx->rep.clear();
-    HIPCHK(ctx, ctx->partials.reserve((size_t)n_rounds * L * std::max(tiles, 1)));
-    HIPCHK(ctx, ctx->results.reserve((size_t)n_rounds * L));
-    HIPCHK(ctx, ctx->rounds.reserve(n_rounds));
-    HIPCHK(ctx, ctx->errflag.reserve(1));
-    HIPCHK(ctx, hipMemcpyAsync(ctx->rounds.p, rounds_h, n_rounds * sizeof(uint32_t),
-                               hipMemcpyHostToDevice, ctx->stream));
-    HIPCHK(ctx, ctx->xdrawn.reserve(2));
-    {
+    if (!fin) {
+        ctx->rep.clear();
+        HIPCHK(ctx, ctx->partials.reserve((size_t)n_rounds * L * std::max(tiles, 1)));
+        HIPCHK(ctx, ctx->results.reserve((size_t)n_rounds * L));
+        HIPCHK(ctx, ctx->rounds.reserve(n_rounds));
+        HIPCHK(ctx, ctx->errflag.reserve(1));
+        HIPCHK(ctx, hipMemcpyAsync(ctx->rounds.p, rounds_h, n_rounds * sizeof(uint32_t),
+                                   hipMemcpyHostToDevice, ctx->stream));
+        HIPCHK(ctx, ctx->xdrawn.reserve(2));
         FillSet f{};
         add_fill(f, ctx->errflag.p, sizeof(int32_t), 0);
         add_fill(f, ctx->xdrawn.p, 2 * sizeof(unsigned long long), 0);
@@ -4065,7 +4088,7 @@
     for (int m = 0; m < kNumModes; ++m) {
         g.dev[m] = ctx->P->groups.p + ctx->P->group_off[m];
         g.count[m] = (fam >> m) & 1 ? (int32_t)ctx->P->h_group[m].size() : 0;
-        if (!((fam >> m) & 1)) continue;
+        if (!((fam >> m) & 1) || fin) continue;
         ctx->mode_ran[m] = false;
         ctx->mode_ms[m] = 0.f;
         ctx->mode_evals[m] = 0;
@@ -4088,7 +4111,7 @@
         S.cpack ? (uint32_t)((rounds_whole + S.rpb - 1) / S.rpb) : gx;
     RoundArgs a{n, cand_offset, seed, n_rounds, tiles, cand_in_dev, olb, ola, S, gx, gz,
                 n_whole * rounds_whole, gx_whole};
-    if (dense_on) {
+    if (dense_on && !fin) {
         ctx->screen_total = ctx->screen_rescored = 0;
         ctx->hot_ran = false;
         ctx->hot_listed = 0;
@@ -4097,16 +4120,18 @@
         ctx->screen_exec = 0;
         ctx->screen_rescore_terms = 0;
     }
-    if (fam & (1 << CAT)) ctx->cat_early = false;
-    ctx->dense_one = false;
-    ctx->pk_plan_pending = false;
-    ctx->zw_pending = false;
-    ctx->evw_used = 0;
-    ctx->screen_pending = false;
-    ctx->screen_exec_pending = false;
+    if (!fin) {
+        if (fam & (1 << CAT)) ctx->cat_early = false;
+        ctx->dense_one = false;
+        ctx->pk_plan_pending = false;
+        ctx->zw_pending = false;
+        ctx->evw_used = 0;
+        ctx->screen_pending = false;
+        ctx->screen_exec_pending = false;
+    }
     const bool sample = cand_in_dev == nullptr;
     int64_t evals_q[2] = {0, 0};
-    if (ctx->timing) HIPCHK(ctx, hipEventRecord(ctx->ev0, ctx->stream));
+    if (ctx->timing && !fin) HIPCHK(ctx, hipEventRecord(ctx->ev0, ctx->stream));
     const bool splitk = sample && ctx->splitk && n > 0 && S.cpack != 0 &&
                         a.total_slots <= kSplitKMaxSlots;
     if (splitk) {
@@ -4134,10 +4159,24 @@
         const bool side = ctx->aux_families && ctx->aux && !ctx->qx && a.tiles > 0 &&
                           g.count[CAT] + g.count[QUANT_GMM] + g.count[QUANT_LGMM] > 0;
         int rc = TPE_OK;
-        bool dense_done = false;
+        bool dense_done = fin;
+        if (phase == kRoundBegin) {
+            if (side) HIPCHK(ctx, hipEventRecord(ctx->ev_cat[0], ctx->stream));
+            rc = launch_dense<double>(ctx, g, a);
+            if (rc) return rc;
+            HIPCHK(ctx, hipGetLastError());
+            ctx->begun.active = true;
+            ctx->begun.seed = seed;
+            ctx->begun.rounds.assign(rounds_h, rounds_h + n_rounds);
+            ctx->begun.n = n;
+            ctx->begun.cand_offset = cand_offset;
+            return TPE_OK;
+        }
         if (side) {
-            HIPCHK(ctx, hipEventRecord(ctx->ev_cat[0], ctx->stream));
-            if (ctx->build.pending) {
+            if (!fin) HIPCHK(ctx, hipEventRecord(ctx->ev_cat[0], ctx->stream));
+            if (fin) {
+                TPE_SETTLE_KEEP(ctx);
+            } else if (ctx->build.pending) {
                 rc = ctx->precision == TPE_F32 ? launch_dense<float>(ctx, g, a) : launch_dense<double>(ctx, g, a);
                 if (rc) return rc;
                 dense_done = true;
@@ -4151,7 +4190,7 @@
             const hipError_t e = hipEventRecord(ctx->ev_cat[1], ctx->aux);
             if (rc == TPE_OK && e != hipSuccess) rc = ctx->hip(e, "second-stream join");
         } else {
-            TPE_SETTLE(ctx);
+            TPE_SETTLE_KEEP(ctx);
             rc = launch_quantized(ctx, g, a, evals_q);
         }
         if (rc == TPE_OK && !dense_done)
@@ -4172,7 +4211,7 @@
         launch_round<double, CAT, false>(ctx, g, a);
     }
     HIPCHK(ctx, hipGetLastError());
-    TPE_SETTLE(ctx);
+    TPE_SETTLE_KEEP(ctx);
     if (ctx->timing) HIPCHK(ctx, hipEventRecord(ctx->ev1, ctx->stream));
     if (tiles == 1) {
         const int64_t nr = (int64_t)n_rounds * L;
@@ -4330,6 +4369,15 @@
     if (errh & 4) return ctx->fail(TPE_ERR_VALUE, "categorical sample out of range");
     if (errh & 8) return ctx->fail(TPE_ERR_VALUE, "quantized sample beyond 2^52 grid steps");
     return TPE_OK;
+}
+
+int finish_round(tpe_ctx* ctx, tpe_label_result* out) {
+    if (!ctx->begun.active) return TPE_ROUND_NOT_STARTED;
+    tpe_rt::BegunRound b = std::move(ctx->begun);
+    ctx->begun = tpe_rt::BegunRound{};
+    HIPCHK(ctx, hipSetDevice(ctx->device));
+    return run_round(ctx, b.seed, b.rounds.data(), (int32_t)b.rounds.size(), b.n, b.cand_offset, nullptr, nullptr,
+                     nullptr, out, -1, kRoundFinish);
 }
 
 __global__ __launch_bounds__(64) void k_samp_fold(const DLabel* __restrict__ labels, SampRec* __restrict__ samp) {
@@ -4525,9 +4573,23 @@
 
 }
 
+int tpe_rt::discard_round(tpe_ctx* ctx) {
+    if (!ctx || !ctx->begun.active) return TPE_OK;
+    ++ctx->begun_discards;
+    const int rc = finish_round(ctx, nullptr);
+    return rc == TPE_ERR_SAMPLE || rc == TPE_ERR_VALUE ? TPE_OK : rc;
+}
+
 extern "C" {
 
 int tpe_abi_version(void) { return TPE_ABI_VERSION; }
+
+int tpe_round_state(const tpe_ctx* ctx, int32_t* begun, int64_t* discards) {
+    if (!ctx) return TPE_ERR_ARG;
+    if (begun) *begun = ctx->begun.active ? 1 : 0;
+    if (discards) *discards = ctx->begun_discards;
+    return TPE_OK;
+}
 
 #ifndef TPE_SOURCE_HASH
 #define TPE_SOURCE_HASH "unstamped000000"
@@ -4682,6 +4744,19 @@
                      nullptr, out, -1);
 }
 
+TPE_DEV int tpe1_suggest_begin(tpe_ctx* ctx, uint64_t seed, const uint32_t* rounds, int32_t n_rounds,
+                               int64_t n_candidates, int64_t cand_offset) {
+    if (!ctx || !rounds) return TPE_ERR_ARG;
+    HIPCHK(ctx, hipSetDevice(ctx->device));
+    return run_round(ctx, seed, rounds, n_rounds, n_candidates, cand_offset, nullptr, nullptr, nullptr, nullptr,
+                     -1, kRoundBegin);
+}
+
+TPE_DEV int tpe1_suggest_finish(tpe_ctx* ctx, tpe_label_result* out) {
+    if (!ctx || !out) return TPE_ERR_ARG;
+    return finish_round(ctx, out);
+}
+
 TPE_DEV int tpe1_score(tpe_ctx* ctx, int32_t label, const double* cand, int64_t n, double* lpdf_below,
                        double* lpdf_above, tpe_label_result* out) {
     if (!ctx || (!cand && n > 0)) return TPE_ERR_ARG;
@@ -4953,7 +5028,8 @@
 
 TPE_DEV int tpe1_set_option(tpe_ctx* ctx, int32_t option, int64_t value) {
     if (!ctx) return TPE_ERR_ARG;
-    TPE_SETTLE(ctx);
+    if (option == TPE_OPT_DEFER_REPORT) TPE_SETTLE_KEEP(ctx);
+    else TPE_SETTLE(ctx);
     switch (option) {
         case TPE_OPT_SCREEN: ctx->screen = value != 0; break;
         case TPE_OPT_SPLITK: ctx->splitk = value != 0; break;
diff --git a/hyperopt_amd/csrc/tpe_multi.hip b/hyperopt_amd/csrc/tpe_multi.hip
--- a/hyperopt_amd/csrc/tpe_multi.hip
+++ b/hyperopt_amd/csrc/tpe_multi.hip
@@ -652,4 +652,17 @@
     return sharded_round(ctx, seed, rounds, n_rounds, n_candidates, cand_offset, out);
 }
 
-}
+int tpe_suggest_begin(tpe_ctx* ctx, uint64_t seed, const uint32_t* rounds, int32_t n_rounds,
+                      int64_t n_candidates, int64_t cand_offset) {
+    if (!ctx || !rounds) return TPE_ERR_ARG;
+    if (!ctx->peers.empty()) return TPE_ROUND_NOT_STARTED;
+    return tpe1_suggest_begin(ctx, seed, rounds, n_rounds, n_candidates, cand_offset);
+}
+
+int tpe_suggest_finish(tpe_ctx* ctx, tpe_label_result* out) {
+    if (!ctx || !out) return TPE_ERR_ARG;
+    if (!ctx->peers.empty()) return TPE_ROUND_NOT_STARTED;
+    return tpe1_suggest_finish(ctx, out);
+}
+
+}
diff --git a/hyperopt_amd/engine.py b/hyperopt_amd/engine.py
--- a/hyperopt_amd/engine.py
+++ b/hyperopt_amd/engine.py
@@ -1,3 +1,4 @@
+import contextlib
 import ctypes
 import threading
 
@@ -77,6 +78,54 @@
             raise ValueError('devices must not be empty')
         return tuple(int(d) for d in device)
     return (int(device),)
+
+
+def _dense_of(specs):
+    return frozenset(np.flatnonzero(
+        (specs['kind'] != L.TPE_CATEGORICAL) & ((specs['flags'] & L.TPE_HAS_Q) == 0)).tolist())
+
+
+class PendingRound(object):
+
+    def __init__(self, eng, started, whole):
+        self.eng, self.started, self._whole, self._res = eng, started, whole, None
+        self._single = False
+
+    def result(self):
+        if self._res is None:
+            res = self.eng.suggest_finish() if self.started else None
+            self.started = False
+            if res is None:
+                res = self._whole()
+            elif self._single:
+                res = res[0]
+            self._res = res
+        return self._res
+
+    def discard(self):
+        if self.started and self._res is None:
+            self.eng.suggest_finish()
+        self.started = False
+        self._whole = None
+
+    def __getitem__(self, key):
+        return _PendingItem(self, key)
+
+
+class _PendingItem(object):
+    def __init__(self, parent, key):
+        self.parent, self.key = parent, key
+
+    started = property(lambda self: self.parent.started)
+
+    def result(self):
+        return self.parent.result()[self.key]
+
+    def discard(self):
+        self.parent.discard()
+
+    def __getitem__(self, key):
+        return _PendingItem(self, key)
 
 
 class Engine(object):
@@ -100,6 +149,9 @@
         self.device = devs[0]
         self.n_labels = 0
         self.history_generation = 0
+        self._split = False
+        self._begun_rounds = 0
+        self.dense_labels = frozenset()
 
     def close(self):
         if getattr(self, 'h', None):
@@ -149,6 +201,7 @@
             _ptr(obs_off), _ptr(obs_trial), _ptr(obs_val), float(gamma), float(prior_weight),
             int(lf), ctypes.byref(nb)))
         self.n_labels = self.hist_labels = len(specs)
+        self.dense_labels = _dense_of(specs)
         return nb.value
 
     def history_reset(self, specs, cat_p):
@@ -158,6 +211,7 @@
         self._check(self.lib.tpe_history_reset(self.h, _ptr(specs), len(specs), _ptr(cat_p),
                                                len(cat_p)))
         self.hist_labels = len(specs)
+        self.dense_labels = _dense_of(specs)
 
     def history_append(self, n_new, obs_trial, obs_val):
         n_new = np.ascontiguousarray(n_new, dtype=np.int64)
@@ -247,7 +301,46 @@
         self.n_labels = int(self.lib.tpe_resident_labels(self.h))
         return self.n_labels
 
+    def suggest_begin(self, seed, rounds, n_candidates, cand_offset=0):
+        rounds = np.ascontiguousarray(np.asarray(rounds, dtype=np.uint32)).reshape(-1)
+        rc = self.lib.tpe_suggest_begin(self.h, int(seed) & 0xFFFFFFFFFFFFFFFF, _ptr(rounds), len(rounds),
+                                        int(n_candidates), int(cand_offset))
+        if rc == L.TPE_ROUND_NOT_STARTED:
+            return False
+        self._check(rc)
+        self._begun_rounds = len(rounds)
+        return True
+
+    def suggest_finish(self):
+        nr = self._begun_rounds
+        out = np.empty(max(nr, 1) * self._labels(), dtype=RESULT_DTYPE)
+        rc = self.lib.tpe_suggest_finish(self.h, _ptr(out))
+        self._begun_rounds = 0
+        if rc == L.TPE_ROUND_NOT_STARTED:
+            return None
+        self._check(rc)
+        return out.reshape(nr, self.n_labels)
+
+    def round_state(self):
+        b, d = ctypes.c_int32(), ctypes.c_int64()
+        self._check(self.lib.tpe_round_state(self.h, ctypes.byref(b), ctypes.byref(d)))
+        return bool(b.value), d.value
+
+    @contextlib.contextmanager
+    def split_rounds(self):
+        prev, self._split = self._split, True
+        try:
+            yield self
+        finally:
+            self._split = prev
+
     def suggest(self, seed, n_candidates, round=0, cand_offset=0):
+        if self._split:
+            self._split = False
+            p = PendingRound(self, self.suggest_begin(seed, [int(round) & 0xFFFFFFFF], n_candidates, cand_offset),
+                             lambda: self.suggest(seed, n_candidates, round, cand_offset))
+            p._single = True
+            return p
         out = np.empty(self._labels(), dtype=RESULT_DTYPE)
         self._check(self.lib.tpe_suggest(self.h, int(seed) & 0xFFFFFFFFFFFFFFFF,
                                          int(round) & 0xFFFFFFFF, int(n_candidates),
@@ -256,6 +349,10 @@
 
     def suggest_batch(self, seed, rounds, n_candidates, cand_offset=0):
         rounds = np.ascontiguousarray(np.asarray(rounds, dtype=np.uint32))
+        if self._split:
+            self._split = False
+            return PendingRound(self, self.suggest_begin(seed, rounds, n_candidates, cand_offset),
+                                lambda: self.suggest_batch(seed, rounds, n_candidates, cand_offset))
         out = np.empty(len(rounds) * self._labels(), dtype=RESULT_DTYPE)
         self._check(self.lib.tpe_suggest_batch(self.h, int(seed) & 0xFFFFFFFFFFFFFFFF,
                                                _ptr(rounds), len(rounds), int(n_candidates),
diff --git a/hyperopt_amd/posterior.py b/hyperopt_amd/posterior.py
--- a/hyperopt_amd/posterior.py
+++ b/hyperopt_amd/posterior.py
@@ -388,6 +388,7 @@
 
 SUBSET_REBUILD = True
 DEFER_REPORT = True
+SPLIT_ROUND = True
 
 
 def build_reference_order(eng, losses, n_valid, gamma, prior_weight, lf, obs_of, known=(), prepare=None,
@@ -407,6 +408,7 @@
     early = holder['early']
     n_below = n_below_of(n_valid, gamma)
     known = set(known)
+    can_split = False
     t0 = time.perf_counter()
     if prepare and (overlap or not known):
         if known and EARLY_ORDERS and early is None:
@@ -418,6 +420,7 @@
         eng.prepare(*prepare)
         t0 = _phase('prepare_enqueue', t0)
         have = set()
+        can_split = SPLIT_ROUND and round_call is not None
     elif known:
         below, off, order = reference_orders(losses, n_below, obs_of, known)
         t0 = _phase('argsorts', t0)
@@ -437,7 +440,19 @@
         raise AssertionError('below mixture depends on a tie order (lf < gamma_cap?)')
     need = have | set(np.flatnonzero(ties[:-1] & 2).tolist())
     res = None
+    pend = None
+    rebuilt = False
     deferred = False
+    if (can_split and not ties[-1] and (early is not None or need != have) and
+            (SPLIT_ROUND == 'always' or early is None or not early.done()) and
+            len(getattr(eng, 'devices', ())) == 1 and hasattr(eng, 'split_rounds') and
+            not ((need | known) & set(getattr(eng, 'dense_labels', range(obs_of.n_labels))))):
+        with eng.split_rounds():
+            r = round_call()
+        if hasattr(r, 'result') and hasattr(r, 'discard'):
+            pend = r
+        else:
+            res = r
     if early is not None:
         orders = early.result()
         if need != have and need <= known:
@@ -455,17 +470,27 @@
             nb, ties = eng.rebuild_labels(losses, n_valid, gamma, prior_weight, lf, off, order, need,
                                           defer=deferred)
         else:
+            if pend is not None:
+                pend.discard()
+                pend = None
             nb, ties = eng.build_posterior_ordered(losses, n_valid, gamma, prior_weight, lf, below, off,
                                                    order)
+        rebuilt = True
         t0 = _phase('rebuild', t0)
         if np.any(ties[:-1]):
             need |= set(np.flatnonzero(ties[:-1] & 2).tolist())
             below, off, order = reference_orders(losses, n_below, obs_of, need)
+            if pend is not None:
+                pend.discard()
+                pend = None
             nb, ties = eng.build_posterior_ordered(losses, n_valid, gamma, prior_weight, lf, below, off,
                                                    order)
             assert not np.any(ties[:-1])
     if round_call is not None:
-        res = round_call()
+        if pend is not None:
+            res = pend.result()
+        elif res is None or rebuilt:
+            res = round_call()
         if deferred:
             nb, ties = eng.build_report()
             if np.any(ties[:-1]):
diff --git a/include/hyperopt_tpe.h b/include/hyperopt_tpe.h
--- a/include/hyperopt_tpe.h
+++ b/include/hyperopt_tpe.h
@@ -15,6 +15,7 @@
 #define TPE_ERR_ARG (-3)
 #define TPE_ERR_HIP (-4)
 #define TPE_ERR_SAMPLE (-5)
+#define TPE_ROUND_NOT_STARTED 1
 
 #define TPE_F64 0
 #define TPE_F32 1
@@ -164,6 +165,11 @@
 int tpe_suggest_batch(tpe_ctx *ctx, uint64_t seed, const uint32_t *rounds,
                       int32_t n_rounds, int64_t n_candidates, int64_t cand_offset,
                       tpe_label_result *out);
+
+int tpe_suggest_begin(tpe_ctx *ctx, uint64_t seed, const uint32_t *rounds, int32_t n_rounds,
+                      int64_t n_candidates, int64_t cand_offset);
+int tpe_suggest_finish(tpe_ctx *ctx, tpe_label_result *out);
+int tpe_round_state(const tpe_ctx *ctx, int32_t *begun, int64_t *discards);
 
 int tpe_suggest_batch_device(tpe_ctx *ctx, uint64_t seed, const uint32_t *rounds,
                              int32_t n_rounds, int64_t n_candidates, int64_t cand_offset,
```

After: 42.47 billion. 0.922x the previous value.
